# Shiakaron/Iterative-solvers-summer-2020

Hardware: AMD Instinct MI355X
Metric: Newton-steps/sec + JVP SpMV HBM GB/s (% peak), 4096^2 grid, 1/2/4/8 GPU (higher is better)
Workload: dtype f64

## Files before the change

include/nkhip.h:

```cpp
#ifndef NKHIP_H
#define NKHIP_H

#include <stdint.h>

#ifdef __cplusplus
extern "C" {
#endif

#define NK_OK 0
#define NK_NO_CONVERGENCE 1
#define NK_NONFINITE 2
#define NK_ZERO_STEP 3
#define NK_BAD_RHS 4
#define NK_EINVAL (-1)
#define NK_EHIP (-2)
#define NK_ECOMM (-3)
#define NK_ENOMEM (-4)

#define NKHIP_ABI_VERSION 3

#define NK_JVP_FD 0
#define NK_JVP_ANALYTIC 1

typedef struct nk_opts {
  double f_tol, f_rtol, x_tol, x_rtol;
  double rdiff;
  int64_t maxiter;
  int32_t inner_m;
  int32_t outer_k;
  int32_t line_search;
  int32_t jvp_mode;
  int32_t verbose;
  int32_t profile;
} nk_opts;

typedef struct nk_stats {
  int64_t nit;
  int64_t nfev;
  int64_t njvp;
  int64_t n_arnoldi;
  double fnorm_inf;
  double fnorm_2;
  int32_t status;
  int32_t pad_;
  int64_t n_backtrack;
  double step_min;
  int64_t n_device_steps;
} nk_stats;

typedef struct nk_kprof {
  char name[32];
  int64_t launches;
  double total_ms;
  double alg_bytes;
  int64_t timed;
  double timed_bytes;
} nk_kprof;

typedef struct nk_comm nk_comm;
typedef struct nk_sh nk_sh;

const char* nk_version(void);
int nk_abi_version(void);
int nk_opts_default(nk_opts* o);
const char* nk_status_string(int code);


int nk_lap5_apply(const double* v_dev, double* y_dev, int64_t ny, int64_t nx, double e, void* stream);

int nk_sh13_apply(const double* v_dev, double* y_dev, int64_t ny, int64_t nx, double h, double r,
                  void* stream);

int nk_sh_residual(const double* u_dev, const double* uo_dev, double* F_dev, int64_t ny, int64_t nx,
                   double h, double r, double k, double g, void* stream);

int nk_sh_jvp(const double* u_dev, const double* v_dev, double* y_dev, int64_t ny, int64_t nx,
              double h, double r, double k, double g, void* stream);

int nk_sh_fdjvp(const double* x0_dev, const double* G0_dev, const double* z_dev, double* y_dev,
                int64_t ny, int64_t nx, double h, double r, double k, double g, double zs,
                double sc, void* stream);

int nk_sh_arnoldi_fused(const double* const* V_dev, const double* coef, int32_t nv,
                        const double* w_dev, double tau, const double* x0_dev, const double* G0_dev,
                        const double* z_dev, int64_t ny, int64_t nx, double h, double r, double k,
                        double g, double zs, double sc, double* v_out_dev, double* w_out_dev,
                        double* dots, void* stream);

int64_t nk_edge_elems(int64_t ny, int64_t nx);
int nk_edge_gather(const double* v_dev, double* E_dev, int64_t ny, int64_t nx, void* stream);
int nk_sh_arnoldi_fused_edges(const double* const* V_dev, const double* const* E_dev,
                              const double* coef, int32_t nv, const double* w_dev, double tau,
                              const double* x0_dev, const double* G0_dev, const double* z_dev,
                              int64_t ny, int64_t nx, double h, double r, double k, double g,
                              double zs, double sc, double* v_out_dev, double* w_out_dev,
                              double* Ev_out_dev, double* Ew_out_dev, double* dots, void* stream);
int64_t nk_arnoldi_mbox_launches(void);

int nk_dot(const double* x_dev, const double* y_dev, int64_t n, double* out, void* stream);
int nk_nrm2(const double* x_dev, int64_t n, double* out, void* stream);
int nk_maxnorm(const double* x_dev, int64_t n, double* out, void* stream);
int nk_axpy(double a, const double* x_dev, double* y_dev, int64_t n, void* stream);
int nk_scal(double a, double* x_dev, int64_t n, void* stream);
int nk_mdot(const double* const* V_dev, int32_t m, const double* w_dev, int64_t n, double* out,
            void* stream);
int nk_maxpy(const double* const* V_dev, const double* coef, int32_t m, double* y_dev, int64_t n,
             void* stream);

int nk_stream_copy(const double* src_dev, double* dst_dev, int64_t n, void* stream);

int nk_debug_bounds(int64_t* violations, int32_t* first_line, int32_t reset);
int nk_debug_mailbox(int64_t* counts, int32_t reset);
int nk_debug_close(const double* const* P_dev, const double* cN, const double* cA,
                   const double* cB, int32_t m, int64_t n, double* A_dev, double* B_dev,
                   double* norm2, void* stream);
int nk_debug_ctl_step(int32_t form, int32_t t, const int32_t* ints, const double* scal,
                      const double* sig, const double* h, const double* cs, const double* sn,
                      const double* gram, const double* red, void* state_out, void* mirror_out,
                      double* prm_out, uint32_t* status_out);
typedef struct nk_stencil_pass {
  int64_t mode;
  int64_t ny, nx;
  int64_t r0, r1;
  const double* a;
  const double* a_halo;
  const double* b;
  const double* b_halo;
  const double* p0;
  double* out0;
  double* out1;
  double* out2;
  double alpha, sc, e, theta;
  double h, r, k, g;
  const double* znorm2;
  double omega;
  const double* spec;
  double spec_thr, spec_ftol, spec_rdiff, spec_zn, spec_zs;
  const double* Ea;
  const double* Eb;
  double* E0;
  double* E2;
  double* PS0[2];
  double* PS2[2];
  int64_t ps_ld;
  int64_t rev;
} nk_stencil_pass;
int nk_debug_stencil(const nk_stencil_pass* p, double* red, int64_t* nblk, void* stream);

int nk_comm_unique_id_bytes(void);
int nk_comm_get_unique_id(void* out);
int nk_comm_create_rccl(nk_comm** out, const void* unique_id, int32_t rank, int32_t nranks);
int nk_comm_create_loopback(nk_comm** out, int32_t nranks);
int nk_comm_peer_handle_bytes(void);
int nk_comm_create_peer(nk_comm** out, int32_t rank, int32_t nranks, int64_t max_nx,
                        void* handle_out);
int nk_comm_peer_connect(nk_comm* c, const void* handles);
int nk_comm_destroy(nk_comm* c);
int nk_comm_abort(nk_comm* c);
int nk_comm_selftest(nk_comm* c, int64_t nx, void* stream);
int nk_comm_selftest_push(nk_comm* c, int64_t nx, void* stream);

int nk_sh_create(nk_sh** out, int64_t ny_local, int64_t nx, int64_t ny_global, double h, double r,
                 double k, double g, const nk_opts* opts, nk_comm* comm, void* stream);
int nk_sh_destroy(nk_sh* s);
int nk_sh_step(nk_sh* s, const double* u_prev_dev, double* u_next_dev, nk_stats* stats);
int nk_sh_set_opts(nk_sh* s, const nk_opts* opts);
int nk_sh_kernel_profile(nk_sh* s, nk_kprof* out, int32_t max);
int nk_sh_reset_profile(nk_sh* s);
int nk_sh_step_log(nk_sh* s, double* steps, int32_t max);
int64_t nk_sh_workspace_bytes(nk_sh* s);

typedef int (*nk_residual_fn)(void* ctx, const double* x_dev, double* f_dev, int64_t n);
int64_t nk_solve_workspace_bytes(int64_t n, const nk_opts* opts);
int nk_solve(nk_residual_fn F, void* ctx, const double* x0_dev, double* x_dev, int64_t n,
             const nk_opts* opts, nk_stats* stats, void* stream, void* workspace,
             int64_t workspace_bytes);

typedef struct nk_drop_params {
  int32_t nx, ny;
  double endl, endr, endb, endt;
  double epsilon;
  int32_t n_exp, m_exp;
  double Bo, alpha2;
  double alpha, gamma, C;
  int32_t smoothing_iters;
  int32_t pad_;
  double a;
} nk_drop_params;
typedef struct nk_drop nk_drop;

int nk_drop_params_default(nk_drop_params* p);
int nk_drop_create(nk_drop** out, const nk_drop_params* p, const nk_opts* opts, void* stream);
int nk_drop_destroy(nk_drop* d);
int nk_drop_lds_fits(int32_t nx, int32_t ny);
int nk_drop_set_state(nk_drop* d, const double* U_dev, const double* Q_dev);
int nk_drop_get_state(nk_drop* d, double* U_dev, double* Q_dev);
int nk_drop_step(nk_drop* d, double dt, double dtmesh, int32_t pmaloops, nk_stats* stats,
                 double* dt_used, double* scale);
int nk_drop_set_scale(nk_drop* d, double scale);
int nk_drop_prepare(nk_drop* d);
int nk_drop_field(nk_drop* d, int32_t which, double* out_dev);
int nk_drop_residual(nk_drop* d, const double* u_dev, double dt, double* R_dev);
int nk_drop_solve(nk_drop* d, double dt, double* U_dev, nk_stats* stats);
int nk_drop_pma(nk_drop* d, double dtmesh, int32_t loops);
int nk_drop_init_coalescing(nk_drop* d, int32_t vsteps, const double* info, int32_t ndrops,
                            double dtmesh, int32_t loops);

typedef struct nk_shlin nk_shlin;
int nk_shlin_create(nk_shlin** out, int64_t ny, int64_t nx, double h, double r, double g, double k,
                    double rtol, int64_t maxiter, void* stream);
int nk_shlin_destroy(nk_shlin* s);
int nk_shlin_step(nk_shlin* s, const double* U_dev, const double* Uo_dev, double* Unew_dev,
                  int64_t* iters, double* relres);

typedef struct nk_mems_params {
  int32_t n;
  int32_t m;
  int32_t smoothing_iters;
  int32_t p;
  double alpha, gamma;
  double epsilon, beta, lambd;
  double endl, endr;
  double k;
} nk_mems_params;
typedef struct nk_mems nk_mems;

int nk_mems_params_default(nk_mems_params* p);
int nk_mems_create(nk_mems** out, const nk_mems_params* p, const nk_opts* opts, void* stream);
int nk_mems_destroy(nk_mems* m);
int nk_mems_set_state(nk_mems* m, const double* U_dev, const double* Q_dev);
int nk_mems_get_state(nk_mems* m, double* U_dev, double* Q_dev);
int nk_mems_step(nk_mems* m, nk_stats* stats, double* dt_used, double* time);
int nk_mems_prepare(nk_mems* m, double* dt);
int nk_mems_field(nk_mems* m, int32_t which, double* out_dev);
int nk_mems_residual(nk_mems* m, const double* u_dev, double* R_dev);

#ifdef __cplusplus
}
#endif
#endif
```

iterative-solvers-summer-2020_amd/csrc/capi.cpp:

```cpp
#include <hip/hip_runtime.h>

#include <cmath>
#include <cstdlib>
#include <cstdio>
#include <cstring>
#include <mutex>
#include <memory>
#include <new>
#include <vector>

#include "../../include/nkhip.h"
#include "comm.h"
#include "nk_kernels.h"
#include "nk_solver.h"
#include "droplet_problem.h"
#include "mems_problem.h"
#include "sh_problem.h"
#include "shlin.h"

using namespace nk;

namespace {

hipStream_t S(void* s) { return static_cast<hipStream_t>(s); }
// ... 121 lines not shown
  A.alpha = sc * zs;
  A.sc = sc;
  A.p0 = G0;
  A.out0 = y;
  A.c = sh_coef(h, r, k, g);
  return hip_rc(stencil_launch(SMode::FDJVP, A, S(stream), nullptr));
}

namespace {
int attach_mbox(ArnoldiArgs& A) {
  const int mode = arnoldi_mbox_mode();
  if (mode == 0) return NK_OK;
  static std::mutex mu;
  static double* buf = nullptr;
  static int64_t cap = 0;
  static uint64_t tag = 0;
  static std::vector<double*> retired;
  std::lock_guard<std::mutex> lk(mu);
  const int64_t need = arnoldi_mbox_elems(A.ny, A.nx);
  if (cap < need) {
    if (buf) retired.push_back(buf);
    buf = nullptr;
    cap = 0;
    if (hipMalloc(reinterpret_cast<void**>(&buf), sizeof(double) * need) != hipSuccess)
      return NK_ENOMEM;
    if (hipMemset(buf, 0, sizeof(double) * need) != hipSuccess) return NK_EHIP;
    cap = need;
  }
  A.mb = buf;
  A.mb_cap = cap;
  A.mb_tag = ++tag;
  A.mb_recompute = mode == 2;
  return NK_OK;
}

int arnoldi_fused_call(const double* const* V, const double* const* E, const double* coef,
                       int32_t nv, const double* w, double tau, const double* x0, const double* G0,
                       const double* z, int64_t ny, int64_t nx, double h, double r, double k,
                       double g, double zs, double sc, double* v_out, double* w_out,
                       double* Ev_out, double* Ew_out, double* dots, void* stream) {
  if (!V || !coef || !w || !x0 || !v_out || !w_out || !(sc != 0.0)) return NK_EINVAL;
  if (!arnoldi_supported(nv, ny, nx)) return NK_EINVAL;
  ArnoldiArgs A;
  if (E) {
    for (int i = 0; i <= nv; ++i) {
      if (!E[i]) return NK_EINVAL;
      A.E[i] = E[i];
    }
  }
  A.Eout_v = Ev_out;
  A.Eout_w = Ew_out;
  A.ny = ny;
  A.nx = nx;
  A.nv = nv;
  for (int i = 0; i < nv; ++i) {
    if (!V[i]) return NK_EINVAL;
    A.V[i] = V[i];
    A.c[i] = coef[i];
  }
  A.w = w;
  A.tau = tau;
  A.x0 = x0;
  A.g0 = G0;
  A.z = z;
  A.alpha = sc * zs;
  A.sc = sc;
  A.k = sh_coef(h, r, k, g);
  A.out_v = v_out;
  A.out_w = w_out;
  if (int rc = attach_mbox(A)) return rc;
  const int nval = 2 * nv + 3;
  if (!dots) {
    static std::mutex mu;
    std::lock_guard<std::mutex> lk(mu);
    static double* buf = nullptr;
    static int64_t cap = 0;
    const int64_t need = int64_t(nval) * 65536;
    if (cap < need) {
      if (buf) hipFree(buf);
      buf = nullptr;
      cap = 0;
      if (hipMalloc(reinterpret_cast<void**>(&buf), sizeof(double) * need) != hipSuccess)
        return NK_ENOMEM;
      cap = need;
    }
    A.partial = buf;
    A.partial_cap = cap;
    int64_t nw = 0;
    return hip_rc(arnoldi_launch(A, S(stream), &nw));
  }
  return reduce_call(int64_t(65536) * 2048, nval, nval, nval, dots, S(stream),
                     [&](double* part, int64_t* nb) {
                       A.partial = part;
                       A.partial_cap = int64_t(nval) * (65536 + 1);
                       return arnoldi_launch(A, S(stream), nb);
                     });
}
}

int64_t nk_arnoldi_mbox_launches(void) { return arnoldi_mbox_launches(); }

int nk_sh_arnoldi_fused(const double* const* V, const double* coef, int32_t nv, const double* w,
                        double tau, const double* x0, const double* G0, const double* z,
                        int64_t ny, int64_t nx, double h, double r, double k, double g, double zs,
                        double sc, double* v_out, double* w_out, double* dots, void* stream) {
  return arnoldi_fused_call(V, nullptr, coef, nv, w, tau, x0, G0, z, ny, nx, h, r, k, g, zs, sc,
                            v_out, w_out, nullptr, nullptr, dots, stream);
}

int nk_sh_arnoldi_fused_edges(const double* const* V, const double* const* E, const double* coef,
                              int32_t nv, const double* w, double tau, const double* x0,
                              const double* G0, const double* z, int64_t ny, int64_t nx, double h,
                              double r, double k, double g, double zs, double sc, double* v_out,
                              double* w_out, double* Ev_out, double* Ew_out, double* dots,
                              void* stream) {
  if (!E) return NK_EINVAL;
  return arnoldi_fused_call(V, E, coef, nv, w, tau, x0, G0, z, ny, nx, h, r, k, g, zs, sc, v_out,
                            w_out, Ev_out, Ew_out, dots, stream);
}

int64_t nk_edge_elems(int64_t ny, int64_t nx) {
  return (ny > 0 && nx > 0) ? edge_elems(ny, nx) : NK_EINVAL;
}

int nk_edge_gather(const double* v, double* E, int64_t ny, int64_t nx, void* stream) {
  if (!v || !E || ny < 1 || nx < 4 || nx % 2) return NK_EINVAL;
  return hip_rc(edge_gather_launch(v, E, ny, nx, S(stream)));
}

int nk_dot(const double* x, const double* y, int64_t n, double* out, void* stream) {
  if (!x || !y || !out || n < 0) return NK_EINVAL;
  VecList P;
  P.p[0] = y;
  return reduce_call(n, 3, 3, 1, out, S(stream), [&](double* part, int64_t* nb) {
    return mdot_launch(x, nullptr, P, 1, n, part, S(stream), nb);
  });
}

int nk_nrm2(const double* x, int64_t n, double* out, void* stream) {
  if (!x || !out || n < 0) return NK_EINVAL;
  double s2 = 0.0;
  VecList P;
  P.p[0] = x;
  const int rc = reduce_call(n, 3, 3, 1, &s2, S(stream), [&](double* part, int64_t* nb) {
    return mdot_launch(x, nullptr, P, 1, n, part, S(stream), nb);
  });
  *out = std::sqrt(s2);
  return rc;
}

int nk_maxnorm(const double* x, int64_t n, double* out, void* stream) {
  if (!x || !out || n <= 0) return NK_EINVAL;
  double* tmp = nullptr;
  hipError_t e = hipMallocAsync(reinterpret_cast<void**>(&tmp), sizeof(double) * n, S(stream));
  if (e != hipSuccess) return hip_rc(e);
  VecList none;
  double r2[2];
  const int rc = reduce_call(n, 2, 1, 2, r2, S(stream), [&](double* part, int64_t* nb) {
    return combo_launch(tmp, x, 1.0, none, 0, n, part, S(stream), nb);
  });
  hipFreeAsync(tmp, S(stream));
  hipStreamSynchronize(S(stream));
  *out = r2[1];
  return rc;
}

int nk_axpy(double a, const double* x, double* y, int64_t n, void* stream) {
  if (!x || !y || n < 0) return NK_EINVAL;
  return hip_rc(axpby_launch(a, x, 1.0, y, y, n, S(stream)));
}

int nk_scal(double a, double* x, int64_t n, void* stream) {
  if (!x || n < 0) return NK_EINVAL;
  return hip_rc(axpby_launch(a, x, 0.0, nullptr, x, n, S(stream)));
}

int nk_mdot(const double* const* V, int32_t m, const double* w, int64_t n, double* out,
            void* stream) {
  if (!V || !w || !out || m < 0 || m > kMaxVec || n < 0) return NK_EINVAL;
  if (m == 0) return NK_OK;
  VecList P;
  for (int i = 0; i < m; ++i) P.p[i] = V[i];
  const int nv = 2 * m + 1;
  double res[2 * kMaxVec + 1];
  const int rc = reduce_call(n, nv, nv, nv, res, S(stream), [&](double* part, int64_t* nb) {
    return mdot_launch(w, nullptr, P, m, n, part, S(stream), nb);
  });
  for (int i = 0; i < m; ++i) out[i] = res[i];
  return rc;
}

int nk_maxpy(const double* const* V, const double* coef, int32_t m, double* y, int64_t n,
             void* stream) {
  if (!V || !coef || !y || m < 0 || m > kMaxVec || n < 0) return NK_EINVAL;
  VecList P;
  for (int i = 0; i < m; ++i) {
    P.p[i] = V[i];
    P.c[i] = coef[i];
  }
  int64_t nb = 0;
  return hip_rc(combo_launch(y, y, 1.0, P, m, n, nullptr, S(stream), &nb));
}

int nk_stream_copy(const double* src, double* dst, int64_t n, void* stream) {
  if (!src || !dst || n < 0) return NK_EINVAL;
  return hip_rc(stream_copy_launch(src, dst, n, S(stream)));
}

int nk_debug_bounds(int64_t* violations, int32_t* first_line, int32_t reset) {
  const int rc = arnoldi_check_counters(violations, first_line, reset != 0);
  return rc == 0 ? NK_OK : (rc == -1 ? NK_EINVAL : NK_EHIP);
}

int nk_debug_mailbox(int64_t* counts, int32_t reset) {
  if (!counts) return NK_EINVAL;
  const int rc = arnoldi_mailbox_counters(counts, reset != 0);
  return rc == 0 ? NK_OK : (rc == -1 ? NK_EINVAL : NK_EHIP);
}

int nk_debug_close(const double* const* P, const double* cN, const double* cA, const double* cB,
                   int32_t m, int64_t n, double* A, double* B, double* norm2, void* stream) {
  if (!P || !cN || !cA || !cB || !A || !B || A == B || !norm2 || m < 1 || m > kMaxVec || n < 1)
    return NK_EINVAL;
  CloseList L;
  for (int i = 0; i < m; ++i) {
    for (int k = 0; k < i; ++k)
      if (P[k] == P[i]) return NK_EINVAL;
    if (!P[i]) return NK_EINVAL;
    L.p[i] = P[i];
    L.cN[i] = cN[i];
    L.cA[i] = cA[i];
    L.cB[i] = cB[i];
  }
  return reduce_call(n, 1, 1, 1, norm2, S(stream), [&](double* part, int64_t* nb) {
    return close_launch(A, B, L, m, n, part, S(stream), nb);
  });
}

int nk_debug_ctl_step(int32_t form, int32_t t, const int32_t* ints, const double* scal,
                      const double* sig, const double* h, const double* cs, const double* sn,
                      const double* gram, const double* red, void* state_out, void* mirror_out,
                      double* prm_out, uint32_t* status_out) {
  if (!state_out) return int(sizeof(ArnCtlState));
  if ((form != 0 && form != 1) || t < 1 || t + 1 > kArnMaxNV || !ints || !scal || !sig || !h ||
      !cs || !sn || !gram || !red || !mirror_out || !prm_out || !status_out)
    return NK_EINVAL;
  const int nval = 2 * (t + 1) + 1;
  ArnCtlState *hS = nullptr, *dS = nullptr;
  uint32_t* status = nullptr;
  double *prm = nullptr, *dred = nullptr;
  hipError_t e = hipHostMalloc(reinterpret_cast<void**>(&hS), sizeof(ArnCtlState), 0);
  if (e == hipSuccess)
    e = hipHostMalloc(reinterpret_cast<void**>(&status), sizeof(uint32_t) * (kMaxVec + 2), 0);
  if (e == hipSuccess) e = hipMalloc(reinterpret_cast<void**>(&dS), sizeof(ArnCtlState));
  if (e == hipSuccess) e = hipMalloc(reinterpret_cast<void**>(&prm), sizeof(double) * kCtlPrm);
  if (e == hipSuccess) e = hipMalloc(reinterpret_cast<void**>(&dred), sizeof(double) * 2 * nval);
  if (e == hipSuccess) {
    std::memset(hS, 0, sizeof(ArnCtlState));
    std::memset(status, 0, sizeof(uint32_t) * (kMaxVec + 2));
    ArnCtlState& S = *hS;
    S.j = ints[0];
    S.hn_pending = ints[1];
    S.m = ints[2];
    S.nv_max = ints[3];
    S.halt = ints[4];
    S.steps = ints[5];
    S.wnorm[t - 1] = scal[0];
    S.gv[t - 1] = scal[1];
    S.sig_est[t] = scal[2];
    S.ptol = scal[3];
    S.omega = scal[4];
    S.lag_ratio2 = scal[5];
    for (int i = 0; i <= t; ++i) S.sig[i] = sig[i];
    for (int i = 0; i < t; ++i) {
      S.h[i] = h[i];
      S.cs[i] = cs[i];
      S.sn[i] = sn[i];
      for (int k = 0; k < i; ++k) S.gram[i][k] = gram[i * t + k];
    }
    e = hipMemcpy(dS, hS, sizeof(ArnCtlState), hipMemcpyHostToDevice);
  }
  if (e == hipSuccess) e = hipMemset(prm, 0, sizeof(double) * kCtlPrm);
  if (e == hipSuccess) e = hipMemcpy(dred, red, sizeof(double) * nval, hipMemcpyHostToDevice);
  if (e == hipSuccess)
    e = form == 0 ? arn_ctl_launch(dS, hS, dred, nullptr, prm, status, t, nullptr)
                  : arn_reduce_ctl_launch(dred, 1, nval, dred + nval, nullptr, dS, hS, prm, status,
                                          t, nullptr);
  if (e == hipSuccess) e = hipDeviceSynchronize();
  if (e == hipSuccess) e = hipMemcpy(state_out, dS, sizeof(ArnCtlState), hipMemcpyDeviceToHost);
  if (e == hipSuccess)
    e = hipMemcpy(prm_out, prm, sizeof(double) * kCtlPrm, hipMemcpyDeviceToHost);
  if (e == hipSuccess) {
    std::memcpy(mirror_out, hS, sizeof(ArnCtlState));
    *status_out = status[t];
  }
  if (hS) (void)hipHostFree(hS);
  if (status) (void)hipHostFree(status);
  (void)hipFree(dS);
  (void)hipFree(prm);
  (void)hipFree(dred);
  return hip_rc(e);
}

int nk_debug_stencil(const nk_stencil_pass* p, double* red, int64_t* nblk_out, void* stream) {
  if (!p || p->mode < 0 || p->mode > 7 || p->ny <= 0 || p->nx <= 0 || !p->a || !p->out0)
    return NK_EINVAL;
  const SMode m = static_cast<SMode>(int(p->mode));
  const bool two = m == SMode::RESID || m == SMode::TRIAL || m == SMode::FDJVP || m == SMode::LINOP;
  const bool has_p0 = m == SMode::TRIAL || m == SMode::FDJVP || m == SMode::AJVP || m == SMode::LINOP;
  const bool reduces = m == SMode::TRIAL || m == SMode::LINOP;
  if ((two && !p->b) || (has_p0 && !p->p0) || (m == SMode::TRIAL && !p->out1) ||
      (m == SMode::LINOP && !p->out2) || (reduces && !red))
    return NK_EINVAL;
  if (m == SMode::FDJVP && !p->znorm2 && !p->spec && !(p->sc != 0.0)) return NK_EINVAL;
  const bool ranged = p->r1 >= 0;
  if (ranged && (p->ny < 4 || p->r0 < 0 || p->r0 >= p->r1 || p->r1 > p->ny || p->r0 == 1 ||
                 p->r1 == p->ny - 1))
    return NK_EINVAL;
  const bool push0 = p->PS0[0] || p->PS0[1], push2 = p->PS2[0] || p->PS2[1];
  if ((push0 && (!p->PS0[0] || !p->PS0[1])) || (push2 && (!p->PS2[0] || !p->PS2[1])) ||
      (push2 && !(m == SMode::TRIAL && p->out2)) ||
      ((push0 || push2) && (p->ny < 4 || p->ps_ld < p->nx || p->ps_ld % 2)))
    return NK_EINVAL;
  for (const void* q : {(const void*)p->Ea, (const void*)p->Eb, (const void*)p->E0,
                        (const void*)p->E2, (const void*)p->PS0[0], (const void*)p->PS0[1],
                        (const void*)p->PS2[0], (const void*)p->PS2[1]})
    if (reinterpret_cast<uintptr_t>(q) & 15u) return NK_EINVAL;
  if (p->E2 && m != SMode::TRIAL) return NK_EINVAL;
  if (p->rev < -1 || p->rev > 1) return NK_EINVAL;

  StencilArgs A;
  A.ny = p->ny;
  A.nx = p->nx;
  auto field = [&](const double* base, const double* halo) {
    return halo ? Field{base, halo, halo + 2 * p->nx} : periodic(base);
  };
  A.a = field(p->a, p->a_halo);
  if (p->b) A.b = (p->b == p->a && p->b_halo == p->a_halo) ? A.a : field(p->b, p->b_halo);
  A.alpha = p->alpha;
  A.p0 = p->p0;
  A.out0 = p->out0;
  A.out1 = p->out1;
  A.out2 = p->out2;
  A.e = p->e;
  A.c = sh_coef(p->h, p->r, p->k, p->g);
  A.sc = p->sc;
  A.znorm2 = p->znorm2;
  A.omega = p->omega;
  A.spec = p->spec;
  A.spec_thr = p->spec_thr;
  A.spec_ftol = p->spec_ftol;
  A.spec_rdiff = p->spec_rdiff;
  A.spec_zn = p->spec_zn;
  A.spec_zs = p->spec_zs;
  A.theta = p->theta;
  A.Ea = p->Ea;
  A.Eb = p->Eb;
  A.E0 = p->E0;
  A.E2 = p->E2;
  A.e_ny = p->ny;
  A.e_row0 = 0;
  for (int i = 0; i < 2; ++i) {
    A.PS0[i] = p->PS0[i];
    A.PS2[i] = p->PS2[i];
  }
  A.ps_ld = p->ps_ld;
  A.rev_force = int(p->rev);
  const StencilArgs L = ranged ? stencil_rows(A, p->r0, p->r1) : A;

  hipStream_t s = S(stream);
  double* buf = nullptr;
  const int64_t slots = stencil_partial_slots(p->ny, p->nx);
  hipError_t e = hipSuccess;
  StencilArgs R = L;
  if (reduces) {
    e = hipMallocAsync(reinterpret_cast<void**>(&buf), sizeof(double) * (slots + 3), s);
    if (e == hipSuccess) e = hipMemsetAsync(buf, 0xff, sizeof(double) * (slots + 3), s);
    if (e != hipSuccess) {
      if (buf) hipFreeAsync(buf, s);
      return hip_rc(e);
    }
    R.partial = buf;
  }
  int64_t nblk = 0;
  e = stencil_launch(m, R, s, &nblk);
  double host[3] = {0.0, 0.0, 0.0};
  const int nv = m == SMode::TRIAL ? 3 : 1;
  if (reduces && e == hipSuccess && 3 * nblk > slots) e = hipErrorInvalidValue;
  if (reduces && e == hipSuccess) e = reduce_final_launch(buf, nblk, 1, nv, buf + slots, nullptr, s);
  if (reduces && e == hipSuccess)
    e = hipMemcpyAsync(host, buf + slots, sizeof(double) * nv, hipMemcpyDeviceToHost, s);
  if (buf) hipFreeAsync(buf, s);
  if (e == hipSuccess) e = hipStreamSynchronize(s);
  if (e != hipSuccess) return hip_rc(e);
  for (int i = 0; reduces && i < nv; ++i) red[i] = host[i];
  if (nblk_out) *nblk_out = nblk;
  return NK_OK;
}

int nk_comm_unique_id_bytes(void) { return comm_unique_id_bytes(); }
int nk_comm_get_unique_id(void* out) { return out ? comm_get_unique_id(out) : NK_EINVAL; }
int nk_comm_create_rccl(nk_comm** out, const void* uid, int32_t rank, int32_t nranks) {
  return comm_create_rccl(out, uid, rank, nranks);
}
int nk_comm_create_loopback(nk_comm** out, int32_t nranks) {
  return comm_create_loopback(out, nranks);
}
int nk_comm_peer_handle_bytes(void) { return comm_peer_handle_bytes(); }
int nk_comm_create_peer(nk_comm** out, int32_t rank, int32_t nranks, int64_t max_nx,
                        void* handle_out) {
  return comm_create_peer(out, rank, nranks, max_nx, handle_out);
}
int nk_comm_peer_connect(nk_comm* c, const void* handles) { return comm_peer_connect(c, handles); }
int nk_comm_destroy(nk_comm* c) {
  delete c;
  return NK_OK;
}
int nk_comm_abort(nk_comm* c) {
  if (!c) return NK_EINVAL;
  c->abort();
  return NK_OK;
}

int nk_comm_selftest(nk_comm* c, int64_t nx, void* stream) {
  if (!c || nx < 1) return NK_EINVAL;
  const hipStream_t s = S(stream);
  const int P = c->size(), r = c->rank();
  constexpr int kV = 8, kSum = 5;
  const int64_t nslab = 4 * nx, nhalo = 4 * nx;
  std::vector<double> h(kV + nslab + nhalo);
  for (int i = 0; i < kV; ++i) h[i] = (i < kSum) ? r + 1.0 + i : r + double(i);
  auto code = [&](int q, int64_t row, int64_t j) { return 1e6 * q + double(row * nx + j); };
  for (int64_t row = 0; row < 4; ++row)
    for (int64_t j = 0; j < nx; ++j) h[kV + row * nx + j] = code(r, row, j);
  double* d = nullptr;
  if (hipMalloc(reinterpret_cast<void**>(&d), h.size() * sizeof(double)) != hipSuccess)
    return NK_EHIP;
  int rc = hipMemcpyAsync(d, h.data(), (kV + nslab) * sizeof(double), hipMemcpyHostToDevice, s) ==
                   hipSuccess
               ? NK_OK
               : NK_EHIP;
  if (!rc) rc = c->allreduce(d, kSum, kV, s);
  if (!rc) rc = c->halo(d + kV, d + kV + nslab, d + kV + nslab + 2 * nx, 4, nx, s);
  if (!rc && (hipMemcpyAsync(h.data(), d, h.size() * sizeof(double), hipMemcpyDeviceToHost, s) !=
                  hipSuccess ||
              hipStreamSynchronize(s) != hipSuccess))
    rc = NK_EHIP;
  (void)hipFree(d);
  if (rc) return rc;
  if (c->failed()) return NK_ECOMM;
  for (int i = 0; i < kV; ++i) {
    const double want = (i < kSum) ? P * (P + 1) / 2.0 + double(P) * i : (P - 1.0) + i;
    if (h[i] != want) return NK_ECOMM;
  }
  const int prev = (r - 1 + P) % P, next = (r + 1) % P;
  const double* lo = h.data() + kV + nslab;
  const double* hi = lo + 2 * nx;
  for (int64_t row = 0; row < 2; ++row)
    for (int64_t j = 0; j < nx; ++j)
      if (lo[row * nx + j] != code(prev, 2 + row, j) || hi[row * nx + j] != code(next, row, j))
        return NK_ECOMM;
  return NK_OK;
}

namespace {
__global__ void slot_read_kernel(const double* src, double* dst, int64_t n) {
  const int64_t i = int64_t(blockIdx.x) * blockDim.x + threadIdx.x;
  if (i < n) dst[i] = src[i];
}
}

int nk_comm_selftest_push(nk_comm* c, int64_t nx, void* stream) {
  if (!c || nx < 1) return NK_EINVAL;
  const hipStream_t s = S(stream);
  nk_halo_slots sl;
  static const char owner = 0;
  const bool claimed = c->claim_slots(&owner, &sl);
  struct Release {
    nk_comm* c;
    bool on;
    ~Release() {
      if (on) c->release_slots(&owner);
    }
  } rel{c, claimed};
  const bool have = claimed && sl.ld >= nx && sl.count >= 1;
  const int P = c->size(), r = c->rank();
  const int64_t ny = 4;
  const int64_t slots[2] = {0, sl.count - 1};
  const char* be = std::getenv("NKHIP_PEER_SELFTEST_BREAK_PUSH");
  const bool broken = be && *be && std::atoi(be) == r;
  auto code = [&](int q, int64_t slot, int64_t row, int64_t j) {
    return 1e9 * (q + 1) + 1e6 * slot + double(row * nx + j);
  };
  const int64_t nslot = have ? 4 * sl.ld : 0;
  std::vector<double> h(2 * ny * nx + 2 * nslot + 2);
  h[2 * ny * nx + 2 * nslot] = have ? 0.0 : 1.0;
  double* d = nullptr;
  if (hipMalloc(reinterpret_cast<void**>(&d), h.size() * sizeof(double)) != hipSuccess)
    return NK_EHIP;
  double* vsrc = d;
  double* rd = d + 2 * ny * nx;
  double* ar = rd + 2 * nslot;
  for (int k = 0; k < 2; ++k)
    for (int64_t row = 0; row < ny; ++row)
      for (int64_t j = 0; j < nx; ++j)
        h[(k * ny + row) * nx + j] = code(r, slots[k], row, j) + (broken ? 0.5 : 0.0);
  int rc = NK_OK;
  auto ok = [&](hipError_t e) {
    if (!rc && e != hipSuccess) rc = NK_EHIP;
  };
  for (int k = 0; k < 2 && have; ++k)
    ok(hipMemsetAsync(sl.mine + slots[k] * 4 * sl.ld, 0xff, sizeof(double) * nslot, s));
  ok(hipMemcpyAsync(d, h.data(), sizeof(double) * (2 * ny * nx + 2 * nslot + 2),
                    hipMemcpyHostToDevice, s));
  if (!rc) rc = c->allreduce(ar, 0, 2, s);
  double any_without = 1.0;
  if (!rc && (hipMemcpyAsync(&any_without, ar, sizeof(double), hipMemcpyDeviceToHost, s) !=
                  hipSuccess ||
              hipStreamSynchronize(s) != hipSuccess))
    rc = NK_EHIP;
  if (!rc && any_without != 0.0) rc = NK_EINVAL;
  for (int k = 0; k < 2 && !rc; ++k)
    ok(push_rows_launch(vsrc + k * ny * nx, sl.prev + slots[k] * 4 * sl.ld,
                        sl.next + slots[k] * 4 * sl.ld, ny, nx, sl.ld, s));
  if (!rc) rc = c->allreduce(ar, 1, 2, s);
  for (int k = 0; k < 2 && !rc; ++k) {
    hipLaunchKernelGGL(slot_read_kernel, dim3(unsigned((nslot + 255) / 256)), dim3(256), 0, s,
                       sl.mine + slots[k] * 4 * sl.ld, rd + k * nslot, nslot);
    ok(hipGetLastError());
  }
  if (!rc && (hipMemcpyAsync(h.data(), rd, sizeof(double) * 2 * nslot, hipMemcpyDeviceToHost, s) !=
                  hipSuccess ||
              hipStreamSynchronize(s) != hipSuccess))
    rc = NK_EHIP;
  (void)hipFree(d);
  if (rc) return rc;
  if (c->failed()) return NK_ECOMM;
  const int prev = (r - 1 + P) % P, next = (r + 1) % P;
  for (int k = 0; k < 2; ++k) {
    const double* m = h.data() + k * nslot;
    for (int64_t row = 0; row < 4; ++row)
      for (int64_t j = 0; j < nx; ++j) {
        const double want = row < 2 ? code(prev, slots[k], ny - 2 + row, j)
                                    : code(next, slots[k], row - 2, j);
        if (m[row * sl.ld + j] != want) return NK_ECOMM;
      }
  }
  return NK_OK;
}

int nk_sh_create(nk_sh** out, int64_t ny_local, int64_t nx, int64_t ny_global, double h, double r,
                 double k, double g, const nk_opts* opts, nk_comm* comm, void* stream) {
  if (!out || ny_local <= 0 || nx <= 0 || ny_global < ny_local || !(h > 0) || !(k != 0))
    return NK_EINVAL;
  if (comm && comm->size() > 1 && ny_local < 2) return NK_EINVAL;
  if ((!comm || comm->size() == 1) && ny_global != ny_local) return NK_EINVAL;
  std::unique_ptr<nk_sh> sh(new (std::nothrow) nk_sh());
  if (!sh) return NK_ENOMEM;
  sh->opts = opts ? *opts : default_opts();
  sh->ny = ny_local;
  sh->nx = nx;
  sh->E = std::make_unique<Engine>(ny_local * nx, comm, S(stream), sh->opts.profile > 0,
                                   stencil_partial_slots(ny_local, nx));
  sh->E->sample = sh->opts.profile > 1 ? sh->opts.profile : 1;
  sh->P = std::make_unique<SHProblem>(*sh->E, ny_local, nx, ny_global, sh_coef(h, r, k, g),
                                      sh->opts.jvp_mode);
  if (sh->P->status()) return sh->P->status();
  sh->NK = std::make_unique<NewtonKrylov>(*sh->E, *sh->P, sh->opts);
  if (sh->NK->status()) return sh->NK->status();
  const int rc = sh->E->sync();
  if (rc) return rc;
  *out = sh.release();
  return NK_OK;
}

int nk_sh_destroy(nk_sh* s) {
  delete s;
  return NK_OK;
}

int nk_sh_set_opts(nk_sh* s, const nk_opts* opts) {
  if (!s || !opts) return NK_EINVAL;
  if (opts->inner_m != s->opts.inner_m || opts->outer_k != s->opts.outer_k) return NK_EINVAL;
  s->opts = *opts;
  s->E->profile = opts->profile > 0;
  s->E->sample = opts->profile > 1 ? opts->profile : 1;
  s->P->set_jvp_mode(opts->jvp_mode);
  s->NK->set_opts(*opts);
  return NK_OK;
}

int nk_sh_step(nk_sh* s, const double* u_prev, double* u_next, nk_stats* stats) {
  if (!s || !u_prev || !u_next) return NK_EINVAL;
  int rc = s->P->prepare(u_prev);
  if (!rc) rc = s->NK->solve(u_prev, u_next, stats);
  if (rc < 0 && s->E->comm) s->E->comm->abort();
  return rc;
}

int nk_sh_kernel_profile(nk_sh* s, nk_kprof* out, int32_t max) {
  if (!s) return NK_EINVAL;
  for (int k = 0; k < K_NKINDS && k < max; ++k) {
    std::memset(out[k].name, 0, sizeof(out[k].name));
    std::strncpy(out[k].name, kind_name(k), sizeof(out[k].name) - 1);
    out[k].launches = s->E->stat(k).launches;
    out[k].total_ms = s->E->stat(k).ms;
    out[k].alg_bytes = s->E->stat(k).bytes;
    out[k].timed = s->E->stat(k).timed;
    out[k].timed_bytes = s->E->stat(k).tbytes;
  }
  return K_NKINDS;
}

int nk_sh_reset_profile(nk_sh* s) {
  if (!s) return NK_EINVAL;
  s->E->reset_stats();
  return NK_OK;
}

int nk_sh_step_log(nk_sh* s, double* steps, int32_t max) {
  if (!s || max < 0 || (max > 0 && !steps)) return NK_EINVAL;
  const std::vector<double>& log = s->NK->step_log();
  for (int32_t i = 0; i < max && size_t(i) < log.size(); ++i) steps[i] = log[i];
  return int(log.size());
}

int64_t nk_sh_workspace_bytes(nk_sh* s) { return s ? s->E->bytes_allocated() : -1; }

int64_t nk_solve_workspace_bytes(int64_t n, const nk_opts* opts) {
  if (n <= 0) return NK_EINVAL;
  const nk_opts o = opts ? *opts : default_opts();
  return int64_t(sizeof(double)) * Engine::pad(n) * (NewtonKrylov::vectors_needed(o) + 2);
}

int nk_solve(nk_residual_fn F, void* ctx, const double* x0, double* x, int64_t n,
             const nk_opts* opts, nk_stats* stats, void* stream, void* workspace,
             int64_t workspace_bytes) {
  if (!F || !x0 || !x || n <= 0) return NK_EINVAL;
  const nk_opts o = opts ? *opts : default_opts();
  if (o.jvp_mode != NK_JVP_FD) return NK_EINVAL;
  Engine E(n, nullptr, S(stream), o.profile != 0);
  const int nvec = NewtonKrylov::vectors_needed(o);
  const int64_t npad = Engine::pad(n);
  const int64_t need = nk_solve_workspace_bytes(n, &o);
  double* ws = static_cast<double*>(workspace);
  const bool own = (ws == nullptr);
  if (!own && (workspace_bytes < need || (reinterpret_cast<uintptr_t>(ws) & 255u)))
    return NK_EINVAL;
  if (own && hipMalloc(reinterpret_cast<void**>(&ws), need) != hipSuccess) return NK_ENOMEM;
  CallbackProblem P(E, F, ctx, ws + npad * nvec, ws + npad * (nvec + 1));
  int rc;
  {
    NewtonKrylov NK(E, P, o, ws, int64_t(sizeof(double)) * npad * nvec);
    rc = NK.status();
    if (!rc) rc = NK.solve(x0, x, stats);
  }
  hipStreamSynchronize(S(stream));
  if (own) hipFree(ws);
  return rc;
}

int nk_drop_params_default(nk_drop_params* p) {
  if (!p) return NK_EINVAL;
  *p = nk_drop_params{};
  p->nx = 91;
  p->ny = 61;
  p->endl = -3;
  p->endr = 6;
  p->endb = -3;
  p->endt = 3;
  p->epsilon = 1e-2;
  p->n_exp = 6;
  p->m_exp = 3;
  p->Bo = 0.01;
  p->alpha2 = 0.0;
  p->alpha = 0.01;
  p->gamma = 0.1;
  p->C = 0.15;
  p->smoothing_iters = 4;
  p->a = 100.0;
  return NK_OK;
}

int nk_drop_create(nk_drop** out, const nk_drop_params* p, const nk_opts* opts, void* stream) {
  if (!out || !p || p->nx < 7 || p->ny < 7) return NK_EINVAL;
  if (p->n_exp < 0 || p->m_exp < 0) return NK_EINVAL;
  DropParams P{};
  P.nx = p->nx;
  P.ny = p->ny;
  P.endl = p->endl;
  P.endr = p->endr;
  P.endb = p->endb;
  P.endt = p->endt;
  P.dksi = (p->endr - p->endl) / (p->nx - 1);
  P.deta = (p->endt - p->endb) / (p->ny - 1);
  P.epsilon = p->epsilon;
  P.n_exp = p->n_exp;
  P.m_exp = p->m_exp;
  P.Bo = p->Bo;
  P.alpha2 = p->alpha2;
// ... 178 lines not shown
```

iterative-solvers-summer-2020_amd/csrc/lgmres.cpp:

```cpp
#include <algorithm>
#include <atomic>
#include <cstddef>
#include <cfloat>
#include <cmath>
#include <cstdlib>
#include <cstring>

#include "nk_solver.h"
#include "peer_dev.h"

namespace nk {

namespace {
constexpr double kEps = DBL_EPSILON;
constexpr double kLagMinRatio2 = 1e-12;

bool devctl_enabled(bool multi) {
  const char* v = std::getenv("NKHIP_DEVCTL");
  if (v && v[0] == '0') return false;
  if (v && v[0] == '1') return true;
  return multi;
}

bool lag_enabled() {
  static const bool on = [] {
    const char* v = std::getenv("NKHIP_LAGNORM");
    return !(v && v[0] == '0');
  }();
  return on;
}

int close_mode_env() {
  const char* v = std::getenv("NKHIP_CLOSE");
  if (v && v[0] == '0') return 0;
  if (v && v[0] == '2') return 2;
  return 1;
}
}

int NewtonKrylov::issue_step(int j, const double* z, double zs, double znorm, bool dev_scale,
                             bool have_w) {
  const int64_t n = E_.n;
  zp_[j] = z;
  hS_->zs[j] = zs;
  double* w = V_[j + 1];
  int rc;
  if (have_w) {
    rc = NK_OK;
    st_->njvp += 1;
  } else if (dev_scale) {
    rc = P_.jvp_dev(X_, G0_, z, E_.dres(Engine::kSlotCombo), omega_, w);
    st_->njvp += 1;
  } else if (znorm == 0.0) {
    rc = E_.launch(K_COPY, 8.0 * n,
                   [&] { return hipMemsetAsync(w, 0, sizeof(double) * n, E_.s); });
    if (!rc) rc = P_.publish_edges(w);
  } else {
    rc = P_.jvp(X_, G0_, z, zs, omega_ / znorm, w);
    st_->njvp += 1;
  }
  if (rc) return rc;
  st_->n_arnoldi += 1;
  VecList P;
  for (int i = 0; i <= j; ++i) P.p[i] = V_[i];
  int64_t nblk = 0;
  const double* g = (j > 0) ? V_[j] : nullptr;
  rc = E_.launch(K_MDOT, 8.0 * n * (j + 2),
                 [&] { return mdot_launch(w, g, P, j + 1, n, E_.partial(), E_.s, &nblk); });
  if (rc) return rc;
  const int np = j + 1;
  return E_.reduce_async(nblk, 2 * np + 1, 2 * np + 1, Engine::slot_mdot(j));
}

int NewtonKrylov::lgmres(double tol, double* dnorm, double* dmax, double** dvec) {
  *dnorm = 0.0;
  *dmax = 0.0;
  *dvec = nullptr;
  const double b_norm = fx_norm_;
  if (!std::isfinite(b_norm)) return NK_BAD_RHS;
  if (b_norm == 0.0) return NK_OK;
  const double atol = std::max(0.0, tol * b_norm);
  const double r_norm = b_norm;
  if (r_norm <= std::max(atol, tol * b_norm)) return NK_OK;
  const double ptol = std::min(1.0, std::max(atol, tol * b_norm) / r_norm);

  const int n_o = ocount_;
  const int m = o_.inner_m + n_o;
  const int64_t n = E_.n;
  const int K = int(outer_.size());
  const bool lag = lag_enabled() && P_.may_speculate();
  const bool devctl = lag && devctl_enabled(E_.comm != nullptr || P_.prefers_devctl());
  V_[0] = Fx_;
  ArnCtlState& S = *hS_;
  S.m = m;
  S.halt = 0;
  S.steps = 0;
  S.ptol = ptol;
  S.omega = omega_;
  S.lag_ratio2 = kLagMinRatio2;
  double* const sig = S.sig;
  double* const rn = S.rn;
  double* const sig_est = S.sig_est;
  double* const wnorm = S.wnorm;
  double* const zs_ = S.zs;
  double* const h = S.h;
  sig[0] = 1.0 / b_norm;
  rn[0] = b_norm;
  double hcur[kMaxVec + 2];
  double red[2 * kMaxVec + 2];
  for (int i = 0; i < kMaxVec + 2; ++i) S.gv[i] = 0.0;
  S.gv[0] = 1.0;

  auto input = [&](int j, const double** z, double* zs, double* zn) {
    if (j < n_o) {
      const int slot = (ohead_ + j) % K;
      *z = outer_[slot];
      *zs = osig_[slot];
      *zn = osig_[slot] * orn_[slot];
    } else {
      *z = V_[j > n_o ? j : 0];
      const int q = j > n_o ? j : 0;
      *zs = sig[q];
      *zn = sig[q] * rn[q];
    }
  };
  auto rotated = [&](int i, double hn, double* hc) {
    for (int k = 0; k <= i; ++k) hc[k] = h[k];
    hc[i + 1] = hn;
    for (int k = 0; k < i; ++k) {
      const double t = S.cs[k] * hc[k] + S.sn[k] * hc[k + 1];
      hc[k + 1] = -S.sn[k] * hc[k] + S.cs[k] * hc[k + 1];
      hc[k] = t;
    }
  };
  auto would_stop = [&](int i, double hn) -> bool {
    double hc[kMaxVec + 2], c, s;
    rotated(i, hn, hc);
    detail::givens(hc[i], hc[i + 1], &c, &s);
    return std::fabs(-s * S.gv[i]) < ptol || !(hn > kEps * wnorm[i]);
  };
  auto finish = [&](int i, double hn) -> bool {
    rotated(i, hn, hcur);
    const double alpha = 1.0 / hn;
    sig[i + 1] = std::isfinite(alpha) ? alpha : 1.0;
    rn[i + 1] = hn;
    const bool breakdown = !(hn > kEps * wnorm[i]);
    detail::givens(hcur[i], hcur[i + 1], &S.cs[i], &S.sn[i]);
    hcur[i] = S.cs[i] * hcur[i] + S.sn[i] * hcur[i + 1];
    for (int k = 0; k <= i; ++k) S.R[k][i] = hcur[k];
    S.gv[i + 1] = -S.sn[i] * S.gv[i];
    S.gv[i] = S.cs[i] * S.gv[i];
    return std::fabs(S.gv[i + 1]) < ptol || breakdown;
  };

  int rc;
  {
    const double* z;
    double zs, zn;
    input(0, &z, &zs, &zn);
    const bool have = spec_.valid && n_o > 0 && z == spec_.z && zs == spec_.zs &&
                      zn == spec_.zn && V_[1] == spec_.w && X_ == spec_.x && G0_ == spec_.g;
    spec_.valid = false;
    rc = issue_step(0, z, zs, zn, false, have);
  }
  sig_est[0] = 0.0;
  if (!rc) rc = E_.sync();
  if (rc) return rc;
  int j = 0, last = 0;
  int close_mode = lag ? close_mode_env() : 0;
  bool closed = false;
  bool hn_pending = false;
  for (;;) {
    const int np = j + 1;
    std::memcpy(red, E_.hres(Engine::slot_mdot(j)), sizeof(double) * (2 * np + 1));
    double tau = 1.0;
    if (hn_pending) {
      hn_pending = false;
      if (finish(j - 1, std::sqrt(red[np + j]))) {
        st_->njvp -= 1;
        st_->n_arnoldi -= 1;
        last = j - 1;
        break;
      }
      if (sig_est[j] > 0.0) {
        tau = sig[j] / sig_est[j];
        zs_[j] = sig[j];
      }
    }
    const double ww = tau * tau * red[2 * np];
    if (!std::isfinite(ww)) return NK_NONFINITE;
    wnorm[j] = std::sqrt(ww);
    for (int i = 0; i < j; ++i) S.gram[j][i] = sig[j] * sig[i] * red[np + i];
    double hh = 0.0;
    for (int i = 0; i <= j; ++i) {
      double acc = tau * sig[i] * red[i];
      for (int k = 0; k < i; ++k) acc -= S.gram[i][k] * h[k];
      h[i] = acc;
      hh += acc * acc;
    }
    VecList U;
    for (int i = 0; i <= j; ++i) {
      U.p[i] = V_[i];
      U.c[i] = -h[i] * sig[i];
    }
    double* w = V_[j + 1];
    const bool more = j + 1 < m;
    const bool next_is_v = more && (j + 1 > n_o);
    const double est = ww - hh;
    int64_t nblk = 0;
    bool predicted = false;
    if (close_mode && P_.has_fused(j + 1) && j + 2 < int(V_.size())) {
      const double hn_est = std::sqrt(est);
      if (close_mode == 2) {
        predicted = true;
        close_mode = 1;
      } else if (hn_est > kEps * wnorm[j]) {
        predicted = !more || (est > kLagMinRatio2 * ww && would_stop(j, hn_est));
      }
    }
    if (predicted) {
      double hc[kMaxVec + 2], a[kMaxVec + 1], b[kMaxVec + 1];
      rotated(j, 0.0, hc);
      if (j > 0 && !detail::lstsq_upper_direct(S.R, j)) {
        close_mode = 0;
        predicted = false;
      }
      for (int i = j - 1; predicted && i >= 0; --i) {
        double accA = S.gv[i], accB = hc[i];
        for (int k = i + 1; k < j; ++k) {
          accA -= S.R[i][k] * a[k];
          accB -= S.R[i][k] * b[k];
        }
        a[i] = accA / S.R[i][i];
        b[i] = accB / S.R[i][i];
      }
      CloseList C;
      int nc = 0;
      auto entry = [&](const double* p) -> int {
        for (int q = 0; q < nc; ++q)
          if (C.p[q] == p) return q;
        if (nc == kMaxVec) return -1;
        C.p[nc] = p;
        C.cN[nc] = C.cA[nc] = C.cB[nc] = 0.0;
        return nc++;
      };
      if (predicted) {
        C.cN[entry(w)] = tau;
        for (int i = 0; i <= j; ++i) C.cN[entry(V_[i])] = U.c[i];
        for (int i = 0; i <= j; ++i) {
          const int q = entry(zp_[i]);
          if (q < 0) {
            predicted = false;
            break;
          }
          if (i < j) {
            C.cA[q] += b_norm * a[i] * zs_[i];
            C.cB[q] -= b[i] * zs_[i];
          } else {
            C.cB[q] += zs_[j];
          }
        }
      }
      if (predicted) {
        rc = E_.launch(K_COMBO, 8.0 * n * (nc + 2), [&] {
          return close_launch(Sv_, V_[j + 2], C, nc, n, E_.partial(), E_.s, &nblk);
        });
        if (rc) return rc;
        double v2 = 0.0;
        rc = E_.reduce(nblk, 1, 1, &v2);
        if (rc) return rc;
        const double hn = std::sqrt(v2);
        if (!more || would_stop(j, hn)) {
          finish(j, hn);
          last = j;
          closed = true;
          break;
        }
      }
    }
    const bool lag_step =
        more && lag && !predicted && (!next_is_v || est > kLagMinRatio2 * ww);
    if (lag_step && P_.has_fused(j + 1)) {
      const double* z = nullptr;
      double zs, zn;
      if (next_is_v) {
        const double e = std::sqrt(est);
        zs = 1.0 / e;
        zn = zs * e;
      } else {
        input(j + 1, &z, &zs, &zn);
      }
      if (zn != 0.0) {
        const double* Vp[kMaxVec];
        double cc[kMaxVec];
        for (int i = 0; i <= j; ++i) {
          Vp[i] = V_[i];
          cc[i] = U.c[i];
        }
        int64_t nw = 0;
        double* vout = Sv_;
        rc = P_.fused_step(Vp, cc, j + 1, w, tau, X_, G0_, z, zs, omega_ / zn, vout, V_[j + 2],
                           &nw, nullptr);
        if (rc) return rc;
        Sv_ = V_[j + 1];
        V_[j + 1] = vout;
        zp_[j + 1] = next_is_v ? vout : z;
        zs_[j + 1] = zs;
        sig_est[j + 1] = next_is_v ? zs : 0.0;
        st_->njvp += 1;
        st_->n_arnoldi += 1;
        const int np1 = j + 2;
        rc = E_.reduce_async(nw, 2 * np1 + 1, 2 * np1 + 1, Engine::slot_mdot(j + 1));
        if (rc) return rc;
        hn_pending = true;
        ++j;
        if (devctl && next_is_v) {
          S.j = j;
          S.hn_pending = 1;
          rc = device_steps();
          j = S.j;
          hn_pending = S.hn_pending != 0;
        } else {
          rc = E_.wait_results(Engine::slot_mdot(j), 2 * np1 + 1);
        }
        if (rc) return rc;
        continue;
      }
    }
    if (lag_step) {
      const EdgeOut eo = P_.edge_out(w);
      rc = E_.launch(K_COMBO, 8.0 * n * (j + 3), [&] {
        return combo_launch(w, w, tau, U, j + 1, n, nullptr, E_.s, &nblk, eo);
      });
      if (!rc) rc = P_.publish_edges(w, eo.E != nullptr);
      if (rc) return rc;
      const double* z;
      double zs, zn;
      if (next_is_v) {
        const double e = std::sqrt(est);
        z = w;
        zs = 1.0 / e;
        zn = zs * e;
        sig_est[j + 1] = zs;
      } else {
        input(j + 1, &z, &zs, &zn);
        sig_est[j + 1] = 0.0;
      }
      rc = issue_step(j + 1, z, zs, zn, false);
      if (rc) return rc;
      hn_pending = true;
      ++j;
      if (devctl && next_is_v && P_.has_jvp_prm() && zn != 0.0) {
        S.j = j;
        S.hn_pending = 1;
        rc = device_steps();
        j = S.j;
        hn_pending = S.hn_pending != 0;
        if (rc) return rc;
        continue;
      }
      rc = E_.sync();
      if (rc) return rc;
      continue;
    }
    const EdgeOut eo = P_.edge_out(w);
    rc = E_.launch(K_COMBO, 8.0 * n * (j + 3), [&] {
      return combo_launch(w, w, tau, U, j + 1, n, E_.partial(), E_.s, &nblk, eo);
    });
    if (!rc) rc = P_.publish_edges(w, eo.E != nullptr);
    if (!rc) rc = E_.reduce_async(nblk, 1, 1, Engine::kSlotCombo);
    if (rc) return rc;
    const bool spec = next_is_v && P_.has_dev_scale() && P_.may_speculate();
    if (spec) {
      rc = issue_step(j + 1, w, 0.0, 0.0, true);
      if (rc) return rc;
    }
    rc = E_.sync();
    if (rc) return rc;
    const bool stop = finish(j, std::sqrt(E_.hres(Engine::kSlotCombo)[0]));
    if (spec) zs_[j + 1] = sig[j + 1];
    if (stop || !more) {
      if (spec) {
        st_->njvp -= 1;
        st_->n_arnoldi -= 1;
      }
      last = j;
      break;
    }
    if (!spec) {
      const double* z;
      double zs, zn;
      input(j + 1, &z, &zs, &zn);
      rc = issue_step(j + 1, z, zs, zn, false);
      if (!rc) rc = E_.sync();
      if (rc) return rc;
    }
    sig_est[j + 1] = 0.0;
    ++j;
  }
  j = last;
  if (!std::isfinite(S.R[j][j])) return NK_OK;
  double y[kMaxVec + 1];
  detail::lstsq_upper(S.R, j + 1, S.gv, y);
  for (int i = 0; i <= j; ++i) {
    y[i] *= b_norm;
    if (!std::isfinite(y[i])) return NK_OK;
  }
  const int slot = (o_.outer_k > 0 && ocount_ < o_.outer_k) ? (ohead_ + ocount_) % K : ohead_;
  VecList Z;
  int nz = j + 1;
  if (closed && detail::lstsq_upper_direct(S.R, j + 1)) {
    nz = 2;
    Z.p[0] = Sv_;
    Z.c[0] = 1.0;
    Z.p[1] = V_[j + 2];
    Z.c[1] = y[j];
  } else {
    for (int i = 0; i <= j; ++i) {
      Z.p[i] = zp_[i];
      Z.c[i] = y[i] * zs_[i];
    }
  }
  int64_t nblk = 0;
  double* d = outer_[slot];
  const EdgeOut eo = P_.edge_out(d);
  rc = E_.launch(K_COMBO, 8.0 * n * (nz + 1), [&] {
    return combo_launch(d, nullptr, 0.0, Z, nz, n, E_.partial(), E_.s, &nblk, eo);
  });
  if (!rc) rc = P_.publish_edges(d, eo.E != nullptr);
  if (rc) return rc;
  double r2[2];
  rc = E_.reduce(nblk, 1, 2, r2);
  if (rc) return rc;
  const double nx = std::sqrt(r2[0]);
  if (nx > 0 && o_.outer_k > 0) {
    osig_[slot] = 1.0 / nx;
    orn_[slot] = nx;
    if (ocount_ < o_.outer_k)
      ++ocount_;
    else
      ohead_ = (ohead_ + 1) % K;
  }
  *dnorm = nx;
  *dmax = r2[1];
  *dvec = d;
  return NK_OK;
}

int NewtonKrylov::device_steps() {
  ArnCtlState& S = *hS_;
  const int t0 = S.j;
  int nvmax = t0;
  while (nvmax + 1 < S.m && nvmax + 1 <= kArnMaxNV &&
         (P_.has_fused(nvmax + 1) || P_.has_jvp_prm()))
    ++nvmax;
  if (nvmax < t0 + 1) return E_.wait_results(Engine::slot_mdot(t0), 2 * (t0 + 1) + 1);
  S.nv_max = nvmax;
  S.halt = 0;
  S.steps = 0;
  S.arrive = 0;
  S.done = 0;
  volatile uint32_t* st = status_;
  for (int t = t0; t < S.m && t < kMaxVec + 2; ++t) st[t] = 0;
  std::atomic_thread_fence(std::memory_order_release);

  const bool one = E_.comm == nullptr;
  struct Rot {
    double* spare;
    double* v;
    bool fused;
    bool unfused;
    bool ctl;
    bool red;
  };
  Rot rot[kMaxVec + 2];
  double cc[kMaxVec] = {};
  const uint64_t wait_ticks = device_wait_ticks();
  auto control = [&](int t, bool copy, int upload_rows = -1) {
    const int slot = Engine::slot_mdot(t);
    return E_.launch(K_CTL, 0.0, [&] {
      return arn_ctl_launch(dS_, hS_, E_.dres(slot), copy ? E_.hres_mut(slot) : nullptr, prm_,
                            status_, t, E_.s, upload_rows);
    });
  };
  auto issue = [&](int t) -> int {
    rot[t] = Rot{Sv_, V_[t + 1], false, false, true, false};
    const int nval = 2 * (t + 2) + 1;
    const int slot = Engine::slot_mdot(t + 1);
    if (!P_.has_fused(t + 1)) {
      const int64_t n = E_.n;
      double* w = V_[t + 1];
      VecList U;
      for (int i = 0; i <= t; ++i) U.p[i] = V_[i];
      int rc = E_.launch(K_COMBO, 8.0 * n * (t + 3),
                         [&] { return combo_prm_launch(w, w, prm_, U, t + 1, n, E_.s); });
      if (!rc) rc = P_.jvp_prm(X_, G0_, w, prm_, V_[t + 2]);
      if (rc) return rc;
      zp_[t + 1] = w;
      rot[t].unfused = true;
      VecList Pm;
      for (int i = 0; i <= t + 1; ++i) Pm.p[i] = V_[i];
      int64_t nb = 0;
      rc = E_.launch(K_MDOT, 8.0 * n * (t + 4), [&] {
        return mdot_launch(V_[t + 2], w, Pm, t + 2, n, E_.partial(), E_.s, &nb);
      });
      if (rc) return rc;
      if (one)
        return E_.launch(K_CTL, 8.0 * nb * nval, [&] {
          return arn_reduce_ctl_launch(E_.partial(), nb, nval, E_.dres_mut(slot),
                                       E_.hres_mut(slot), dS_, hS_, prm_, status_, t + 1, E_.s);
        });
      rot[t].red = true;
      rc = E_.reduce_async(nb, nval, nval, slot, false);
      return rc ? rc : control(t + 1, true);
    }
    const double* Vp[kMaxVec];
    for (int i = 0; i <= t; ++i) Vp[i] = V_[i];
    double* vout = Sv_;
    int64_t nw = 0;
    PeerArgs pa;
    const bool have_pa = !one && peer_fuse_enabled() && E_.comm->take_allreduce(&pa, nval);
    ArnTail tl;
    const char* te = std::getenv("NKHIP_ARN_TAIL");
    const bool tail_env = te && (te[0] == '1' || te[0] == '2');
    const bool want_tail = tail_env && (one || (have_pa && ((te && te[0] == '2') ||
                                                            !E_.comm->group_shares_device())));
    if (want_tail) {
      tl.S = dS_;
      tl.H = hS_;
      tl.result = E_.dres_mut(slot);
      tl.result_host = E_.hres_mut(slot);
      tl.prm = prm_;
      tl.status = status_;
      tl.t = t + 1;
      tl.nval = nval;
      tl.peer = !one;
      const uint64_t ticks = wait_ticks;
      tl.wait_ticks = ticks;
      if (have_pa) tl.pa = pa;
      if (const char* e = std::getenv("NKHIP_ARN_TAIL_TIMEOUT_S")) {
        const double sec = std::atof(e);
        if (sec > 0) {
          const uint64_t t = uint64_t(double(ticks) * sec / device_wait_seconds());
          tl.wait_ticks = std::min(tl.wait_ticks, t);
          if (have_pa) tl.pa.wait_ticks = std::min(tl.pa.wait_ticks, t);
        }
      }
    }
    bool tail_used = false;
    int rc = P_.fused_step(Vp, cc, t + 1, V_[t + 1], 1.0, X_, G0_, nullptr, 1.0, 1.0, vout,
                           V_[t + 2], &nw, prm_, want_tail ? &tl : nullptr, &tail_used);
    if (rc) return rc;
    Sv_ = V_[t + 1];
    V_[t + 1] = vout;
    zp_[t + 1] = vout;
    rot[t].fused = true;
    if (tail_used) {
      rot[t].ctl = false;
      return NK_OK;
    }
    if (one)
      return E_.launch(K_CTL, 8.0 * nw * nval, [&] {
        return arn_reduce_ctl_launch(E_.partial(), nw, nval, E_.dres_mut(slot),
                                     E_.hres_mut(slot), dS_, hS_, prm_, status_, t + 1, E_.s);
      });
    if (have_pa)
      return E_.launch(K_CTL, 8.0 * nw * nval, [&] {
        return arn_reduce_allreduce_ctl_launch(E_.partial(), nw, nval, E_.dres_mut(slot),
                                               E_.hres_mut(slot), pa, dS_, hS_, prm_, status_,
                                               t + 1, E_.s);
      });
    rot[t].red = true;
    rc = E_.reduce_async(nw, nval, nval, slot, false);
    return rc ? rc : control(t + 1, true);
  };
  int rc = control(t0, false, t0);
  int next = t0;
  if (!rc) rc = issue(next++);
  int t = t0;
  while (!rc) {
    const uint32_t v = E_.wait_flag(status_ + t);
    if (v != 1) {
      if (v != 2) rc = (E_.comm && E_.comm->failed()) ? NK_ECOMM : NK_EHIP;
      break;
    }
    st_->njvp += 1;
    st_->n_arnoldi += 1;
    st_->n_device_steps += 1;
    ++t;
    if (next == t && next + 1 <= nvmax) rc = issue(next++);
  }
  int voided = 0, voided_unfused = 0, voided_ctl = 0, voided_red = 0;
  for (int u = next - 1; u >= t; --u) {
    voided_ctl += rot[u].ctl ? 1 : 0;
    voided_red += rot[u].red ? 1 : 0;
    if (rot[u].unfused) {
      ++voided_unfused;
      continue;
    }
    if (!rot[u].fused) continue;
    Sv_ = rot[u].spare;
    V_[u + 1] = rot[u].v;
    ++voided;
  }
  P_.void_fused_steps(voided);
  E_.void_last(K_CTL, voided_ctl);
  E_.void_last(K_COMBO, voided_unfused);
  E_.void_last(K_USERF, voided_unfused);
  E_.void_last(K_MDOT, voided_unfused);
  E_.void_last(K_REDUCE, voided_red);
  if (rc) return rc;
  if (voided > 0 && (rc = E_.sync()) != NK_OK) return rc;
  if (S.j != t || S.halt != 1 + t) return NK_EHIP;
  S.halt = 0;
  return NK_OK;
}

}
```

iterative-solvers-summer-2020_amd/csrc/nk_kernels.h:

```cpp
#pragma once

#include <hip/hip_runtime.h>

#include <cstdint>

#include "peer_dev.h"

struct nk_comm;

namespace nk {

bool peer_fuse_enabled();
bool slab_x_enabled(const nk_comm* c);
uint64_t device_wait_ticks();
double device_wait_seconds();

struct Field {
  const double* base;
  const double* lo;
  const double* hi;
};

inline Field periodic(const double* p) { return Field{p, nullptr, nullptr}; }

struct SHCoef {
  double c0, c1, c2, c3;
  double k, g;
  double ik;
};
SHCoef sh_coef(double h, double r, double k, double g);

enum class SMode : int {
  LAP5 = 0,
  SH13 = 1,
  RESID = 2,
  BOLD = 3,
  TRIAL = 4,
  FDJVP = 5,
  AJVP = 6,
  LINOP = 7,
};

struct StencilArgs {
  int64_t ny = 0, nx = 0;
  Field a{}, b{};
  double alpha = 0.0;
  const double* p0 = nullptr;
  double* out0 = nullptr;
  double* out1 = nullptr;
  double* out2 = nullptr;
  double e = 0.0;
  SHCoef c{};
  double sc = 1.0;
  double* partial = nullptr;
  const double* znorm2 = nullptr;
  double omega = 0.0;
  const double* spec = nullptr;
  double spec_thr = 0.0, spec_ftol = 0.0, spec_rdiff = 0.0, spec_zn = 1.0, spec_zs = 1.0;
  double theta = 0.0;
  double* E0 = nullptr;
  double* E2 = nullptr;
  const double* Ea = nullptr;
  const double* Eb = nullptr;
  int64_t e_ny = 0, e_row0 = 0;
  double* PS0[2] = {};
  double* PS2[2] = {};
  int64_t ps_ld = 0;
  bool rev = false;
  int rev_force = -1;
  bool nt_p0 = false;
};

bool traversal_reverse();

StencilArgs stencil_rows(const StencilArgs& A, int64_t r0, int64_t r1);
hipError_t stencil_launch(SMode m, const StencilArgs& a, hipStream_t s, int64_t* nblk);
int64_t stencil_partial_slots(int64_t ny, int64_t nx);
double stencil_bytes_per_point(SMode m, bool has_xt);

constexpr int kMaxVec = 64;
struct VecList {
  const double* p[kMaxVec];
  double c[kMaxVec];
};

constexpr int kKrylovBlock = 256;
constexpr int kKrylovPerThread = 8;
constexpr int64_t kKrylovChunk = int64_t(kKrylovBlock) * kKrylovPerThread;

inline int64_t krylov_blocks(int64_t n) { return (n + kKrylovChunk - 1) / kKrylovChunk; }
int64_t krylov_grid(int64_t n, int* cpb, int64_t target_blocks);

hipError_t mdot_launch(const double* a, const double* g, const VecList& P, int np, int64_t n,
                       double* partial, hipStream_t s, int64_t* nblk);
struct EdgeOut {
  double* E = nullptr;
  int64_t nx = 0, ny = 0;
};
hipError_t combo_launch(double* out, const double* in, double cin, const VecList& P, int np,
                        int64_t n, double* partial, hipStream_t s, int64_t* nblk,
                        const EdgeOut& eo = EdgeOut{});
hipError_t combo_prm_launch(double* out, const double* in, const double* prm, const VecList& P,
                            int np, int64_t n, hipStream_t s);
struct CloseList {
  const double* p[kMaxVec];
  double cN[kMaxVec], cA[kMaxVec], cB[kMaxVec];
};
hipError_t close_launch(double* outA, double* outB, const CloseList& P, int np, int64_t n,
                        double* partial, hipStream_t s, int64_t* nblk);
hipError_t reduce_final_launch(const double* partial, int64_t nblk, int nsum, int nv,
                               double* result, double* result_host, hipStream_t s);
hipError_t fddiff_launch(double* w, const double* f0, double sc, int64_t n, hipStream_t s);
hipError_t cg_update_launch(double* x, double* r, const double* p, const double* q, double alpha,
                            int64_t n, double* partial, hipStream_t s, int64_t* nblk);
hipError_t shlin_diag_launch(const double* U, const double* Uo, double k, double g, double* d,
                             int64_t n, hipStream_t s);
hipError_t stream_copy_launch(const double* src, double* dst, int64_t n, hipStream_t s);
hipError_t axpby_launch(double a, const double* x, double b, const double* y, double* out,
                        int64_t n, hipStream_t s);

constexpr int kArnMaxNV = 35;
constexpr int kEdgeW = 256;
__host__ __device__ inline int64_t edge_groups(int64_t nx) { return (nx + kEdgeW - 1) / kEdgeW; }
__host__ __device__ inline int64_t edge_elems(int64_t ny, int64_t nx) { return edge_groups(nx) * ny * 4; }
hipError_t edge_gather_launch(const double* v, double* E, int64_t ny, int64_t nx, hipStream_t s);
struct SlabX {
  char* me = nullptr;
  char* prev = nullptr;
  char* next = nullptr;
  int P = 0;
  int64_t max_nx = 0;
  uint64_t tag = 0;
  int* err = nullptr;
  uint64_t wait_ticks = 0;
};
struct ArnCtlState;
struct ArnTail {
  ArnCtlState* S = nullptr;
  ArnCtlState* H = nullptr;
  double* result = nullptr;
  double* result_host = nullptr;
  double* prm = nullptr;
  uint32_t* status = nullptr;
  int t = 0;
  int nval = 0;
  bool peer = false;
  uint64_t wait_ticks = 0;
  PeerArgs pa{};
};
struct ArnoldiArgs {
  int64_t ny = 0, nx = 0;
  int nv = 0;
  int strips = 0, nbands = 0, RY = 0;
  const double* V[kArnMaxNV] = {};
  double c[kArnMaxNV] = {};
  const double* w = nullptr;
  double tau = 1.0;
  const double* x0 = nullptr;
  const double* g0 = nullptr;
  const double* z = nullptr;
  double alpha = 0.0;
  double sc = 1.0;
  SHCoef k{};
  double* out_v = nullptr;
  double* out_w = nullptr;
  const double* E[kArnMaxNV + 1] = {};
  double* Eout_v = nullptr;
  double* Eout_w = nullptr;
  const double* yh = nullptr;
  int64_t yh_ld = 0;
  SlabX x{};
  const double* HS[kArnMaxNV + 2] = {};
  int64_t hs_ld = 0;
  double* PS[4] = {};
  double* partial = nullptr;
  int64_t partial_cap = 0;
  int64_t r_begin = 0, r_end = -1;
  int64_t pstride = 0, pcol0 = 0;
  bool plan_only = false;
  int reserve_cus = 0;
  const double* ctl = nullptr;
  double* mb = nullptr;
  int64_t mb_cap = 0;
  uint64_t mb_tag = 0;
  bool mb_recompute = false;
  int alt = -1;
  ArnTail tail{};
};
inline int64_t arnoldi_mbox_elems(int64_t ny, int64_t nx) {
  return (2 * ny + 64) * (nx / 128 + 2) * 8;
}
int arnoldi_mbox_mode();
int64_t arnoldi_mbox_launches();
bool arnoldi_supported(int nv, int64_t ny, int64_t nx);
bool arnoldi_wide(int nv);
hipError_t arnoldi_launch(const ArnoldiArgs& A, hipStream_t s, int64_t* nwaves);
hipError_t arnoldi_edge_launch(const ArnoldiArgs& A, double* y4, hipStream_t s);
hipError_t arnoldi_edge_halo_launch(const ArnoldiArgs& A, const PeerArgs& pa, double* yh,
                                    hipStream_t s);
int arnoldi_check_counters(int64_t* violations, int32_t* first_line, bool reset);
int arnoldi_mailbox_counters(int64_t out[4], bool reset);
hipError_t push_rows_launch(const double* v, double* prev_slot, double* next_slot, int64_t ny,
                            int64_t nx, int64_t ld, hipStream_t s);

struct ArnCtlState {
  int32_t j;
  int32_t hn_pending;
  int32_t m;
  int32_t nv_max;
  int32_t halt;
  int32_t steps;
  uint32_t arrive;
  uint32_t done;
  double ptol, omega, lag_ratio2, pad2_;
  double sig[kMaxVec + 2];
  double rn[kMaxVec + 2];
  double sig_est[kMaxVec + 2];
  double wnorm[kMaxVec + 2];
  double zs[kMaxVec + 2];
  double cs[kMaxVec + 1], sn[kMaxVec + 1];
  double gv[kMaxVec + 2];
  double h[kMaxVec + 2];
  double R[kMaxVec + 1][kMaxVec + 1];
  double gram[kMaxVec + 1][kMaxVec + 1];
};
constexpr int kCtlPrm = kArnMaxNV + 4;
hipError_t arn_ctl_launch(ArnCtlState* S, ArnCtlState* H, const double* red, double* red_host,
                          double* prm, uint32_t* status, int t, hipStream_t s,
                          int upload_rows = -1);
hipError_t arn_reduce_ctl_launch(const double* partial, int64_t nblk, int nval, double* result,
                                 double* result_host, ArnCtlState* S, ArnCtlState* H, double* prm,
                                 uint32_t* status, int t, hipStream_t s);
hipError_t arn_reduce_allreduce_ctl_launch(const double* partial, int64_t nblk, int nval,
                                           double* result, double* result_host, const PeerArgs& pa,
                                           ArnCtlState* S, ArnCtlState* H, double* prm,
                                           uint32_t* status, int t, hipStream_t s);

}
```

iterative-solvers-summer-2020_amd/csrc/nk_solver.cpp:

```cpp
#include "nk_solver.h"

#include <algorithm>
#include <atomic>
#include <cfloat>
#include <cmath>
#include <cstdio>
#include <cstdlib>
#include <cstring>
#include <mutex>

namespace nk {

namespace {
constexpr double kEps = DBL_EPSILON;
constexpr int kReduceSlots = Engine::kSlots;
}

const char* kind_name(int kind) {
  static const char* names[K_NKINDS] = {"sh_fdjvp", "sh_ajvp", "sh_trial", "sh_bold",
                                         "krylov_mdot", "krylov_combo", "reduce_final", "copy",
                                         "halo", "user_F", "axpby", "arnoldi_fused",
                                         "arnoldi_edge", "edge_gather", "arnoldi_slab_edges",
                                         "arnoldi_ctl", "halo_push"};
  return (kind >= 0 && kind < K_NKINDS) ? names[kind] : "?";
// ... 171 lines not shown
}

int64_t Engine::pool_index(const double* v) const {
  if (!pool_ || !v || v < pool_) return -1;
  const int64_t off = v - pool_;
  if (off % npad != 0 || off / npad >= pool_count_) return -1;
  return off / npad;
}

void Engine::mark_edges(const double* v) {
  const int64_t q = pool_index(v);
  if (q < 0 || !epool_) return;
  if (ekept_.size() < size_t(pool_count_)) ekept_.assign(pool_count_, 0);
  ekept_[q] = 1;
}

bool Engine::edges_kept(const double* v) const {
  const int64_t q = pool_index(v);
  return q >= 0 && size_t(q) < ekept_.size() && ekept_[q] != 0;
}

double* Engine::edges(const double* v) const {
  if (!epool_ || !v || v < pool_) return nullptr;
  const int64_t off = v - pool_;
  if (off % npad != 0 || off / npad >= pool_count_) return nullptr;
  return epool_ + edge_n_ * (off / npad);
}

int Engine::gather_edges(const double* v) {
  double* e = edges(v);
  if (!e) return NK_OK;
  mark_edges(v);
  return launch(K_EDGE, 8.0 * edge_n_ * 2,
                [&] { return edge_gather_launch(v, e, edge_ny_, edge_nx_, s); });
}

EdgeOut Engine::edge_out(const double* v) {
  EdgeOut eo;
  eo.E = edges(v);
  if (!eo.E) return eo;
  mark_edges(v);
  eo.nx = edge_nx_;
  eo.ny = edge_ny_;
  return eo;
}

hipEvent_t Engine::ev() {
  if (!free_ev_.empty()) {
    hipEvent_t e = free_ev_.back();
    free_ev_.pop_back();
    return e;
  }
  hipEvent_t e = nullptr;
  hipEventCreate(&e);
  return e;
}

void Engine::harvest() {
  for (auto& p : pend_) {
    float ms = 0.f;
    hipEventElapsedTime(&ms, p.a, p.b);
    stats_[p.kind].timed += 1;
    stats_[p.kind].ms += ms;
    stats_[p.kind].tbytes += p.bytes;
    free_ev_.push_back(p.a);
    free_ev_.push_back(p.b);
  }
  pend_.clear();
}

void Engine::void_last(int kind, int count) {
  if (kind < 0 || kind >= K_NKINDS) return;
  for (int c = 0; c < count && c < kRecent && stats_[kind].launches > 0; ++c) {
    const int64_t idx = stats_[kind].launches - 1;
    stats_[kind].launches = idx;
    stats_[kind].bytes -= recent_bytes_[kind][idx % kRecent];
    for (size_t i = 0; i < pend_.size(); ++i) {
      if (pend_[i].kind == kind && pend_[i].idx == idx) {
        free_ev_.push_back(pend_[i].a);
        free_ev_.push_back(pend_[i].b);
        pend_.erase(pend_.begin() + i);
        break;
      }
    }
  }
}

void Engine::reset_stats() {
  for (auto& k : stats_) k = KStat{};
  for (auto& t : tick_) t = 0;
}

int Engine::sync() {
  if (hipStreamSynchronize(s) != hipSuccess) return NK_EHIP;
  harvest();
  return (comm && comm->failed()) ? NK_ECOMM : NK_OK;
}

int Engine::copy(double* dst, const double* src, int64_t cnt) {
  if (dst == src) return NK_OK;
  return launch(K_COPY, 16.0 * cnt, [&] {
    if (cnt >= (int64_t(1) << 16)) return axpby_launch(1.0, src, 0.0, nullptr, dst, cnt, s);
    return hipMemcpyAsync(dst, src, sizeof(double) * cnt, hipMemcpyDeviceToDevice, s);
  });
}

namespace {
constexpr uint64_t kUnset = 0x7FF0DEADBEEF0001ull;
bool poll_enabled() {
  static const bool on = [] {
    const char* e = std::getenv("NKHIP_POLL");
    return !(e && e[0] == '0');
  }();
  return on;
}
}

int Engine::wait_results(int slot, int nv) {
  if ((comm && !comm->allreduce_writes_host()) || !poll_enabled()) return sync();
  volatile uint64_t* h = reinterpret_cast<volatile uint64_t*>(hres_ + slot);
  for (int k = 0; k < nv; ++k) {
    for (int64_t spins = 0; h[k] == kUnset; ++spins) {
      if (spins > (int64_t(1) << 26)) return sync();
      __builtin_ia32_pause();
    }
  }
  std::atomic_thread_fence(std::memory_order_acquire);
  return NK_OK;
}

uint32_t Engine::wait_flag(const uint32_t* flag) {
  const volatile uint32_t* f = flag;
  for (int64_t spins = 0; *f == 0; ++spins) {
    if (spins > (int64_t(1) << 26)) {
      if (sync() != NK_OK) return 0;
      break;
    }
    __builtin_ia32_pause();
  }
  const uint32_t v = *f;
  std::atomic_thread_fence(std::memory_order_acquire);
  return v;
}

int Engine::reduce_async(int64_t nblk, int nsum, int nv, int slot, bool host_copy) {
  if (slot < 0 || slot + nv > kReduceSlots) return NK_EINVAL;
  const bool multi = comm != nullptr;
  if (!multi || (host_copy && comm->allreduce_writes_host())) {
    uint64_t* h = reinterpret_cast<uint64_t*>(hres_ + slot);
    for (int k = 0; k < nv; ++k) h[k] = kUnset;
    std::atomic_thread_fence(std::memory_order_release);
  }
  int rc = launch(K_REDUCE, 8.0 * nblk * nv, [&] {
    return reduce_final_launch(partial_, nblk, nsum, nv, dres_ + slot,
                               multi ? nullptr : hres_ + slot, s);
  });
  if (rc || !multi) return rc;
  if (!host_copy) return comm->allreduce(dres_ + slot, nsum, nv, s);
  return comm->allreduce_host(dres_ + slot, hres_ + slot, nsum, nv, s);
}

int Engine::reduce(int64_t nblk, int nsum, int nv, double* out) {
  int rc = reduce_async(nblk, nsum, nv, kSlotSync);
  if (!rc) rc = sync();
  if (rc) return rc;
  std::memcpy(out, hres_ + kSlotSync, sizeof(double) * nv);
  return NK_OK;
}

namespace detail {

void givens(double a, double b, double* c, double* s) {
  if (b == 0.0) {
    *c = 1.0;
    *s = 0.0;
    return;
  }
  const double r = std::hypot(a, b);
  *c = a / r;
  *s = b / r;
}

bool lstsq_upper_direct(const double (*R)[kMaxVec + 1], int n) {
  double dmax = 0.0, dmin = INFINITY;
  for (int i = 0; i < n; ++i) {
    dmax = std::max(dmax, std::fabs(R[i][i]));
    dmin = std::min(dmin, std::fabs(R[i][i]));
  }
  return n > 0 && dmin > kEps * n * dmax;
}

void lstsq_upper(const double (*R)[kMaxVec + 1], int n, const double* g, double* y) {
  if (lstsq_upper_direct(R, n)) {
    for (int i = n - 1; i >= 0; --i) {
      double acc = g[i];
      for (int k = i + 1; k < n; ++k) acc -= R[i][k] * y[k];
      y[i] = acc / R[i][i];
    }
    return;
  }
  std::vector<double> A(n * n), Vm(n * n, 0.0);
  for (int i = 0; i < n; ++i)
    for (int k = 0; k < n; ++k) A[i * n + k] = (k >= i) ? R[i][k] : 0.0;
  for (int i = 0; i < n; ++i) Vm[i * n + i] = 1.0;
  for (int sweep = 0; sweep < 60; ++sweep) {
    double off = 0.0;
    for (int p = 0; p < n - 1; ++p)
      for (int q = p + 1; q < n; ++q) {
        double a = 0, b = 0, c = 0;
        for (int i = 0; i < n; ++i) {
          a += A[i * n + p] * A[i * n + p];
          b += A[i * n + q] * A[i * n + q];
          c += A[i * n + p] * A[i * n + q];
        }
        if (c == 0.0) continue;
        off = std::max(off, std::fabs(c) / std::sqrt(a * b + 1e-300));
        const double zeta = (b - a) / (2.0 * c);
        const double t = std::copysign(1.0, zeta) / (std::fabs(zeta) + std::sqrt(1.0 + zeta * zeta));
        const double cs = 1.0 / std::sqrt(1.0 + t * t), sn = cs * t;
        for (int i = 0; i < n; ++i) {
          const double ap = A[i * n + p], aq = A[i * n + q];
          A[i * n + p] = cs * ap - sn * aq;
          A[i * n + q] = sn * ap + cs * aq;
          const double vp = Vm[i * n + p], vq = Vm[i * n + q];
          Vm[i * n + p] = cs * vp - sn * vq;
          Vm[i * n + q] = sn * vp + cs * vq;
        }
      }
    if (off < 1e-15) break;
  }
  std::vector<double> sig(n);
  double smax = 0.0;
  for (int k = 0; k < n; ++k) {
    double acc = 0;
    for (int i = 0; i < n; ++i) acc += A[i * n + k] * A[i * n + k];
    sig[k] = std::sqrt(acc);
    smax = std::max(smax, sig[k]);
  }
  const double cut = kEps * n * smax;
  for (int i = 0; i < n; ++i) y[i] = 0.0;
  for (int k = 0; k < n; ++k) {
    if (!(sig[k] > cut)) continue;
    double ug = 0.0;
    for (int i = 0; i < n; ++i) ug += A[i * n + k] * g[i];
    ug /= sig[k] * sig[k];
    for (int i = 0; i < n; ++i) y[i] += Vm[i * n + k] * ug;
  }
}

}

NewtonKrylov::NewtonKrylov(Engine& E, Problem& P, const nk_opts& o, void* external,
                           int64_t external_bytes)
    : E_(E), P_(P), o_(o) {
  if (o.inner_m < 1 || o.outer_k < 0 || o.inner_m + o.outer_k + 1 > kMaxVec) {
    init_status_ = NK_EINVAL;
    return;
  }
  std::vector<double*> v;
  init_status_ = E_.alloc(vectors_needed(o), &v, external, external_bytes);
  if (init_status_) return;
  int q = 0;
  X_ = v[q++];
  Xt_ = v[q++];
  Fx_ = v[q++];
  Ft_ = v[q++];
  G0_ = v[q++];
  Gt_ = v[q++];
  Sv_ = v[q++];
  const int nv = o.inner_m + o.outer_k + 1;
  V_.assign(nv, nullptr);
  for (int i = 1; i < nv; ++i) V_[i] = v[q++];
  outer_.assign(std::max(o.outer_k, 1), nullptr);
  for (int i = 0; i < std::max(o.outer_k, 1); ++i) outer_[i] = v[q++];
  osig_.assign(outer_.size(), 0.0);
  orn_.assign(outer_.size(), 0.0);
  if (hipHostMalloc(reinterpret_cast<void**>(&hS_), sizeof(ArnCtlState), 0) != hipSuccess ||
      hipHostMalloc(reinterpret_cast<void**>(&status_), sizeof(uint32_t) * (kMaxVec + 2), 0) !=
          hipSuccess ||
      hipMalloc(reinterpret_cast<void**>(&dS_), sizeof(ArnCtlState)) != hipSuccess ||
      hipMalloc(reinterpret_cast<void**>(&prm_), sizeof(double) * kCtlPrm) != hipSuccess) {
    init_status_ = NK_ENOMEM;
    return;
  }
  std::memset(hS_, 0, sizeof(ArnCtlState));
}

NewtonKrylov::~NewtonKrylov() {
  if (E_.s) hipStreamSynchronize(E_.s);
  if (hS_) hipHostFree(hS_);
  if (status_) hipHostFree(status_);
  if (dS_) hipFree(dS_);
  if (prm_) hipFree(prm_);
}


int NewtonKrylov::line_search(double* s_out, double* fnorm_new, double* fmax, double* xmax) {
  double tmp_s = 0.0, tmp_phi = fx_norm_ * fx_norm_;
  double tmp_fmax = 0.0, tmp_xmax = 0.0, tmp_sum = tmp_phi;
  int rc = NK_OK;
  auto phi = [&](double s) -> double {
    if (s == tmp_s) return tmp_phi;
    double red[3];
    rc = P_.eval(X_, d_, -s, Xt_, Ft_, Gt_, red);
    st_->nfev += 1;
    const double p = std::isfinite(red[0]) ? red[0] : INFINITY;
    tmp_s = s;
    tmp_phi = p;
    tmp_sum = red[0];
    tmp_fmax = std::isfinite(red[0]) ? red[1] : NAN;
    tmp_xmax = red[2];
    return p;
  };
  double s = 1.0;
  bool found = true;
  if (o_.line_search) {
    const double phi0 = tmp_phi, derphi0 = -tmp_phi, c1 = 1e-4, amin = 1e-2;
    double alpha0 = 1.0;
    const double thr = phi0 + c1 * alpha0 * derphi0;
    const int K = int(outer_.size());
    spec_.valid = false;
    Problem::SpecJvp sp{};
    const bool arm = P_.can_spec_jvp() && ocount_ > 0 && K > 0 && V_.size() > 1;
    if (arm) {
      const int slot = ohead_ % K;
      sp = Problem::SpecJvp{outer_[slot], osig_[slot], osig_[slot] * orn_[slot], thr, f_tol_,
                            rdiff_, V_[1]};
      if (sp.zn != 0.0) P_.arm_spec(&sp);
    }
    double phi_a0 = phi(alpha0);
    P_.arm_spec(nullptr);
    if (rc) return rc;
    if (arm && sp.zn != 0.0) {
      const bool ran = std::isfinite(tmp_sum) && tmp_sum <= thr && !(tmp_fmax <= f_tol_);
      if (ran) {
        spec_.valid = true;
        spec_.z = sp.z;
        spec_.zs = sp.zs;
        spec_.zn = sp.zn;
        spec_.w = sp.w;
        spec_.x = Xt_;
        spec_.g = Gt_;
      } else {
        E_.void_last(K_FDJVP, 1);
      }
    }
    if (phi_a0 <= phi0 + c1 * alpha0 * derphi0) {
      s = alpha0;
    } else {
      double alpha1 = -(derphi0)*alpha0 * alpha0 / 2.0 / (phi_a0 - phi0 - derphi0 * alpha0);
      double phi_a1 = phi(alpha1);
      if (rc) return rc;
      if (phi_a1 <= phi0 + c1 * alpha1 * derphi0) {
        s = alpha1;
      } else {
        found = false;
        while (alpha1 > amin) {
          const double factor = alpha0 * alpha0 * alpha1 * alpha1 * (alpha1 - alpha0);
          double a = alpha0 * alpha0 * (phi_a1 - phi0 - derphi0 * alpha1) -
                     alpha1 * alpha1 * (phi_a0 - phi0 - derphi0 * alpha0);
          a = a / factor;
          double b = -alpha0 * alpha0 * alpha0 * (phi_a1 - phi0 - derphi0 * alpha1) +
                     alpha1 * alpha1 * alpha1 * (phi_a0 - phi0 - derphi0 * alpha0);
          b = b / factor;
          double alpha2 = (-b + std::sqrt(std::fabs(b * b - 3 * a * derphi0))) / (3.0 * a);
          const double phi_a2 = phi(alpha2);
          if (rc) return rc;
          if (phi_a2 <= phi0 + c1 * alpha2 * derphi0) {
            s = alpha2;
            found = true;
            break;
          }
          if ((alpha1 - alpha2) > alpha1 / 2.0 || (1 - alpha2 / alpha1) < 0.96) alpha2 = alpha1 / 2.0;
          alpha0 = alpha1;
          alpha1 = alpha2;
          phi_a0 = phi_a1;
          phi_a1 = phi_a2;
        }
        if (!found) s = 1.0;
      }
    }
    if (s != tmp_s) phi(s);
    if (rc) return rc;
  } else {
    phi(1.0);
    if (rc) return rc;
  }
  *s_out = s;
  *fnorm_new = std::sqrt(tmp_sum);
  *fmax = tmp_fmax;
  *xmax = tmp_xmax;
  return NK_OK;
}

int NewtonKrylov::solve(const double* x_in, double* x_out, nk_stats* st) {
  if (init_status_) return init_status_;
  nk_stats dummy;
  st_ = st ? st : &dummy;
  std::memset(st_, 0, sizeof(nk_stats));
  st_->step_min = 1.0;
  steps_.clear();
  ocount_ = 0;
  ohead_ = 0;
  const int64_t n = E_.n;
  const double f_tol = std::isnan(o_.f_tol) ? std::pow(kEps, 1.0 / 3.0) : o_.f_tol;
  f_tol_ = f_tol;
  spec_.valid = false;
  const double f_rtol = std::isnan(o_.f_rtol) ? INFINITY : o_.f_rtol;
  const double x_tol = std::isnan(o_.x_tol) ? INFINITY : o_.x_tol;
  const double x_rtol = std::isnan(o_.x_rtol) ? INFINITY : o_.x_rtol;
  rdiff_ = (o_.rdiff > 0) ? o_.rdiff : std::pow(kEps, 0.5);
  const int64_t maxiter = (o_.maxiter > 0) ? o_.maxiter : 100 * (P_.n_global() + 1);
  const bool talk = o_.verbose && (!E_.comm || E_.comm->rank() == 0);

  int rc = P_.set_x0(x_in);
  double red[3];
  if (!rc) rc = P_.eval(x_in, x_in, 0.0, X_, Fx_, G0_, red);
  if (rc) return rc;
  st_->nfev = 1;
  fx_norm_ = std::sqrt(red[0]);
  double fmax = std::isfinite(red[0]) ? red[1] : NAN;
  double xmax = red[2];
  omega_ = rdiff_ * std::max(1.0, xmax) / std::max(1.0, fmax);
  const double gamma = 0.9, eta_max = 0.9999, eta_treshold = 0.1;
  double eta = 1e-3;
  double dxmax = INFINITY;
  double f0_norm = NAN;
  bool converged = false;
  int64_t it = 0;
  for (it = 0; it < maxiter; ++it) {
    const double f_norm = fmax;
    if (std::isnan(f0_norm)) f0_norm = f_norm;
    if (f_norm == 0.0 || ((f_norm <= f_tol && f_norm / f_rtol <= f0_norm) &&
                          (dxmax <= x_tol && dxmax / x_rtol <= xmax))) {
      converged = true;
      break;
    }
    const double tol = std::min(eta, eta * fx_norm_);
    double dnorm = 0.0, dmx = 0.0;
    rc = lgmres(tol, &dnorm, &dmx, &d_);
    if (rc) break;
    if (!(dnorm != 0.0) || d_ == nullptr) {
      rc = NK_ZERO_STEP;
      break;
    }
    dxmax = dmx;
    rc = P_.set_dir(d_);
    if (rc) break;
    double s = 1.0, fnorm_new = 0.0;
    rc = line_search(&s, &fnorm_new, &fmax, &xmax);
    if (rc) break;
    if (s != 1.0) st_->n_backtrack += 1;
    st_->step_min = std::min(st_->step_min, s);
    steps_.push_back(s);
    std::swap(X_, Xt_);
    std::swap(Fx_, Ft_);
    std::swap(G0_, Gt_);
    rc = P_.set_x0(X_);
    if (rc) break;
    omega_ = rdiff_ * std::max(1.0, xmax) / std::max(1.0, fmax);
    const double eta_A = gamma * fnorm_new * fnorm_new / (fx_norm_ * fx_norm_);
    if (gamma * eta * eta < eta_treshold)
      eta = std::min(eta_max, eta_A);
    else
      eta = std::min(eta_max, std::max(eta_A, gamma * eta * eta));
    fx_norm_ = fnorm_new;
    if (talk) {
      std::printf("%lld:  |F(x)| = %g; step %g\n", static_cast<long long>(it), fmax, s);
      std::fflush(stdout);
    }
  }
  st_->nit = it;
  st_->fnorm_inf = fmax;
  st_->fnorm_2 = fx_norm_;
  if (rc) {
    st_->status = rc;
    return rc;
  }
  rc = E_.copy(x_out, X_, n);
  if (!rc) rc = E_.sync();
  if (rc) return rc;
  st_->status = converged ? NK_OK : NK_NO_CONVERGENCE;
  return st_->status;
}

}
```

iterative-solvers-summer-2020_amd/csrc/nk_solver.h:

```cpp
#pragma once

#include <hip/hip_runtime.h>

#include <cstdint>
#include <string>
#include <vector>

#include "../../include/nkhip.h"
#include "comm.h"
#include "nk_kernels.h"

namespace nk {

enum Kind : int {
  K_FDJVP = 0,
  K_AJVP,
  K_TRIAL,
  K_BOLD,
  K_MDOT,
  K_COMBO,
  K_REDUCE,
  K_COPY,
  K_HALO,
  K_USERF,
  K_AXPBY,
  K_ARNOLDI,
  K_ARN_EDGE,
  K_EDGE,
  K_ARN_SLAB,
  K_CTL,
  K_PUSH,
  K_NKINDS
};

const char* kind_name(int kind);
void log_launch(int kind, double bytes);

struct KStat {
  int64_t launches = 0;
  double bytes = 0.0;
  int64_t timed = 0;
  double ms = 0.0;
  double tbytes = 0.0;
};

class Engine {
 public:
  Engine(int64_t n, nk_comm* comm, hipStream_t s, bool profile, int64_t min_partial = 0);
  ~Engine();
  Engine(const Engine&) = delete;
  Engine& operator=(const Engine&) = delete;

  int alloc(int count, std::vector<double*>* out, void* external = nullptr,
            int64_t external_bytes = 0);
  bool pool_chunk_mapped() const { return vmm_base_ != nullptr; }
  void enable_edges(int64_t ny, int64_t nx) {
    edge_ny_ = ny;
    edge_nx_ = nx;
  }
  double* edges(const double* v) const;
  int64_t pool_index(const double* v) const;
  int pool_count() const { return pool_count_; }
  void mark_edges(const double* v);
  bool edges_kept(const double* v) const;
  int gather_edges(const double* v);
  EdgeOut edge_out(const double* v);
  static int64_t pad(int64_t n) {
    const int64_t p = (n + 255) / 256 * 256;
    if (p < (int64_t(1) << 16)) return p;
    return (p + 32767) / 32768 * 32768 + 16384;
  }

  template <class L>
  int launch(int kind, double bytes, L&& fn) {
    return launch_on(kind, bytes, s, static_cast<L&&>(fn));
  }
  template <class L>
  int launch_on(int kind, double bytes, hipStream_t st, L&& fn);
  int reduce(int64_t nblk, int nsum, int nv, double* out);
  int reduce_async(int64_t nblk, int nsum, int nv, int slot, bool host_copy = true);
  const double* dres(int slot) const { return dres_ + slot; }
  const double* hres(int slot) const { return hres_ + slot; }
  double* dres_mut(int slot) const { return dres_ + slot; }
  double* hres_mut(int slot) const { return hres_ + slot; }
  static constexpr int kSlots = 1024;
  static int slot_mdot(int j) { return (j & 3) * 136; }
  static constexpr int kSlotCombo = 560;
  static constexpr int kSlotSync = 600;
  int sync();
  int wait_results(int slot, int nv);
  uint32_t wait_flag(const uint32_t* flag);
  int copy(double* dst, const double* src, int64_t n);
  void void_last(int kind, int count);

  double* partial() const { return partial_; }
  int64_t partial_cap() const { return partial_cap_; }
  const KStat& stat(int k) const { return stats_[k]; }
  void reset_stats();
  int64_t bytes_allocated() const { return bytes_; }

  int64_t n;
  int64_t npad;
  nk_comm* comm;
  hipStream_t s;
  bool profile;
  int sample = 1;

 private:
  void harvest();
  hipEvent_t ev();
  double* pool_ = nullptr;
  bool own_pool_ = false;
  int pool_count_ = 0;
  std::vector<uint8_t> ekept_;
  double* epool_ = nullptr;
  int64_t edge_ny_ = 0, edge_nx_ = 0, edge_n_ = 0;
  double* partial_ = nullptr;
  int64_t partial_cap_ = 0;
  double* dres_ = nullptr;
  double* hres_ = nullptr;
  int64_t bytes_ = 0;
  void* vmm_base_ = nullptr;
  size_t vmm_size_ = 0, vmm_chunk_ = 0;
  std::vector<hipMemGenericAllocationHandle_t> vmm_h_;
  int vmm_alloc(size_t bytes, size_t chunk);
  void vmm_free();
  struct Pending {
    int kind;
    hipEvent_t a, b;
    double bytes;
    int64_t idx;
  };
  static constexpr int kRecent = 8;
  double recent_bytes_[K_NKINDS][kRecent] = {};
  std::vector<Pending> pend_;
  std::vector<hipEvent_t> free_ev_;
  KStat stats_[K_NKINDS];
  int64_t tick_[K_NKINDS] = {};
};

template <class L>
int Engine::launch_on(int kind, double bytes, hipStream_t st, L&& fn) {
  hipEvent_t a = nullptr, b = nullptr;
  const bool timed = profile && (tick_[kind]++ % sample == 0);
  if (timed) {
    a = ev();
    hipEventRecord(a, st);
  }
  const hipError_t e = fn();
  if (timed) {
    b = ev();
    hipEventRecord(b, st);
    pend_.push_back(Pending{kind, a, b, bytes, stats_[kind].launches});
  }
  recent_bytes_[kind][stats_[kind].launches % kRecent] = bytes;
  stats_[kind].launches += 1;
  stats_[kind].bytes += bytes;
  log_launch(kind, bytes);
  return e == hipSuccess ? NK_OK : NK_EHIP;
}

struct Problem {
  virtual ~Problem() = default;
  virtual int64_t n_global() const = 0;
  virtual int eval(const double* x, const double* p, double alpha, double* xt, double* F,
                   double* G, double red[3]) = 0;
  virtual int jvp(const double* x0, const double* G0, const double* z, double zs, double sc,
                  double* w) = 0;
  virtual bool has_dev_scale() const { return false; }
  virtual int jvp_dev(const double* , const double* , const double* ,
                      const double* , double , double* ) {
    return NK_EINVAL;
  }
  virtual bool may_speculate() const { return true; }
  virtual bool has_jvp_prm() const { return false; }
  virtual int jvp_prm(const double* , const double* , const double* ,
                      const double* , double* ) {
    return NK_EINVAL;
  }
  virtual bool prefers_devctl() const { return false; }
  virtual bool has_fused(int ) const { return false; }
  virtual int fused_step(const double* const* , const double* , int ,
                         const double* , double , const double* ,
                         const double* , const double* , double , double ,
                         double* , double* , int64_t* ,
                         const double* , const ArnTail*  = nullptr,
                         bool*  = nullptr) {
    return NK_EINVAL;
  }
  virtual int publish_edges(const double* , bool  = false) { return NK_OK; }
  virtual EdgeOut edge_out(const double* ) { return EdgeOut{}; }
  virtual void void_fused_steps(int ) {}
  virtual int set_x0(const double* ) { return NK_OK; }
  virtual int set_dir(const double* ) { return NK_OK; }
  struct SpecJvp {
    const double* z;
    double zs, zn;
    double thr, ftol, rdiff;
    double* w;
  };
  virtual bool can_spec_jvp() const { return false; }
  virtual void arm_spec(const SpecJvp* ) {}
};

class NewtonKrylov {
 public:
  NewtonKrylov(Engine& E, Problem& P, const nk_opts& o, void* external = nullptr,
               int64_t external_bytes = 0);
  ~NewtonKrylov();
  NewtonKrylov(const NewtonKrylov&) = delete;
  NewtonKrylov& operator=(const NewtonKrylov&) = delete;
  int status() const { return init_status_; }
  void set_opts(const nk_opts& o) { o_ = o; }
  int solve(const double* x_in, double* x_out, nk_stats* st);
  static int vectors_needed(const nk_opts& o) { return o.inner_m + 2 * o.outer_k + 8; }
  const std::vector<double>& step_log() const { return steps_; }

 private:
  int lgmres(double tol, double* dnorm, double* dmax, double** dvec);
  int issue_step(int j, const double* z, double zs, double znorm, bool dev_scale,
                 bool have_w = false);
  int device_steps();
  const double* zp_[kMaxVec + 1];
  ArnCtlState* hS_ = nullptr;
  ArnCtlState* dS_ = nullptr;
  double* prm_ = nullptr;
  uint32_t* status_ = nullptr;
  int line_search(double* s_out, double* fnorm_new, double* fmax, double* xmax);

  Engine& E_;
  Problem& P_;
  nk_opts o_;
  int init_status_ = NK_OK;
  double *X_ = nullptr, *Xt_ = nullptr, *Fx_ = nullptr, *Ft_ = nullptr, *G0_ = nullptr,
         *Gt_ = nullptr;
  double* Sv_ = nullptr;
  std::vector<double*> V_;
  std::vector<double*> outer_;
  std::vector<double> osig_, orn_;
  int ocount_ = 0, ohead_ = 0;
  double omega_ = 0.0;
  double* d_ = nullptr;
  nk_stats* st_ = nullptr;
  std::vector<double> steps_;
  double fx_norm_ = 0.0;
  double rdiff_ = 0.0;
  double f_tol_ = 0.0;
  struct {
    bool valid = false;
    const double* z = nullptr;
    double zs = 0.0, zn = 0.0;
    double* w = nullptr;
    const double* x = nullptr;
    const double* g = nullptr;
  } spec_;
};

nk_opts default_opts();

namespace detail {
void givens(double a, double b, double* c, double* s);
void lstsq_upper(const double (*R)[kMaxVec + 1], int n, const double* g, double* y);
bool lstsq_upper_direct(const double (*R)[kMaxVec + 1], int n);
}

}
```

iterative-solvers-summer-2020_amd/csrc/sh_problem.cpp:

```cpp
#include "sh_problem.h"

#include <algorithm>
#include <cmath>
#include <cstdlib>
#include <cstring>

#include "peer_dev.h"

namespace nk {

SHProblem::SHProblem(Engine& E, int64_t ny, int64_t nx, int64_t ny_global, SHCoef c, int jvp_mode)
    : E_(E), ny_(ny), nx_(nx), ny_g_(ny_global), c_(c), jvp_mode_(jvp_mode) {
  if (arnoldi_supported(1, ny, nx)) E_.enable_edges(ny, nx);
  if (arnoldi_supported(1, ny, nx) && !(E_.comm && E_.comm->shares_device())) {
    const int64_t n = arnoldi_mbox_elems(ny, nx);
    if (hipMalloc(reinterpret_cast<void**>(&mb_), sizeof(double) * n) == hipSuccess &&
        hipMemset(mb_, 0, sizeof(double) * n) == hipSuccess) {
      mb_cap_ = n;
    } else {
      if (mb_) hipFree(mb_);
      mb_ = nullptr;
      (void)hipGetLastError();
    }
  }
  if (hipMalloc(reinterpret_cast<void**>(&B_), sizeof(double) * Engine::pad(ny * nx)) !=
      hipSuccess) {
    B_ = nullptr;
    status_ = NK_ENOMEM;
    return;
  }
  if (dist()) {
    if (ny < 2) {
      status_ = NK_EINVAL;
      return;
    }
    double* h = nullptr;
    if (hipMalloc(reinterpret_cast<void**>(&h), sizeof(double) * 24 * nx) != hipSuccess) {
      status_ = NK_ENOMEM;
      return;
    }
    hx_ = h;
    hz_ = h + 4 * nx;
    hd_ = h + 8 * nx;
    hu_ = h + 12 * nx;
    y4_ = h + 16 * nx;
    yh_ = h + 20 * nx;
    if (!E_.comm->claim_slots(this, &slots_) || slots_.ld < nx) {
      if (slots_.mine) E_.comm->release_slots(this);
      slots_ = nk_halo_slots{};
    }
    double mm[3] = {-double(ny), double(ny), slots_.mine ? 0.0 : 1.0};
    if (hipMemcpyAsync(y4_, mm, sizeof(mm), hipMemcpyHostToDevice, E_.s) != hipSuccess ||
        E_.comm->allreduce(y4_, 0, 3, E_.s) != NK_OK ||
        hipMemcpyAsync(mm, y4_, sizeof(mm), hipMemcpyDeviceToHost, E_.s) != hipSuccess ||
        hipStreamSynchronize(E_.s) != hipSuccess) {
      status_ = NK_ECOMM;
      return;
    }
    ny_min_ = int64_t(-mm[0]);
    ny_max_ = int64_t(mm[1]);
    if (mm[2] > 0.0 && slots_.mine) {
      E_.comm->release_slots(this);
      slots_ = nk_halo_slots{};
    }
    if (hipStreamCreateWithFlags(&side_, hipStreamNonBlocking) != hipSuccess ||
        hipEventCreateWithFlags(&ev_in_, hipEventDisableTiming) != hipSuccess ||
        hipEventCreateWithFlags(&ev_out_, hipEventDisableTiming) != hipSuccess) {
      status_ = NK_EHIP;
      return;
    }
  }
}

SHProblem::~SHProblem() {
  if (slots_.mine) E_.comm->release_slots(this);
  if (side_) hipStreamSynchronize(side_);
  if (B_) hipFree(B_);
  if (hx_) hipFree(hx_);
  if (mb_) hipFree(mb_);
  if (ev_in_) hipEventDestroy(ev_in_);
  if (ev_out_) hipEventDestroy(ev_out_);
  if (side_) hipStreamDestroy(side_);
}

namespace {
Field sub_field(const Field& f, int64_t r0, int64_t r1, int64_t ny, int64_t nx) {
  if (!f.base) return f;
  Field s;
  s.base = f.base + r0 * nx;
  s.lo = (r0 >= 2) ? f.base + (r0 - 2) * nx : (f.lo ? f.lo : f.base + (ny - 2) * nx);
  s.hi = (r1 + 2 <= ny) ? f.base + r1 * nx : (f.lo ? f.hi : f.base);
  return s;
}
}

StencilArgs stencil_rows(const StencilArgs& A, int64_t r0, int64_t r1) {
  StencilArgs B = A;
  B.ny = r1 - r0;
  B.a = sub_field(A.a, r0, r1, A.ny, A.nx);
  B.b = sub_field(A.b, r0, r1, A.ny, A.nx);
  const int64_t off = r0 * A.nx;
  B.e_row0 = A.e_row0 + r0;
  if (A.p0) B.p0 = A.p0 + off;
  if (A.out0) B.out0 = A.out0 + off;
  if (A.out1) B.out1 = A.out1 + off;
  if (A.out2) B.out2 = A.out2 + off;
  return B;
}

int SHProblem::halo_stencil(int kind, SMode m, const StencilArgs& A, const double* z, double* zh) {
  const double bytes = stencil_bytes_per_point(m, false);
  if (!z)
    return E_.launch(kind, bytes * ny_ * nx_, [&] { return stencil_launch(m, A, E_.s, nullptr); });
  if (!dist() || ny_ < 8 || !side_) {
    int rc = halo(z, zh);
    if (rc) return rc;
    return E_.launch(kind, bytes * ny_ * nx_,
                     [&] { return stencil_launch(m, A, E_.s, nullptr); });
  }
  if (hipEventRecord(ev_in_, E_.s) != hipSuccess ||
      hipStreamWaitEvent(side_, ev_in_, 0) != hipSuccess)
    return NK_EHIP;
  const StencilArgs I = stencil_rows(A, 2, ny_ - 2);
  if (stencil_launch(m, I, side_, nullptr) != hipSuccess) return NK_EHIP;
  if (hipEventRecord(ev_out_, side_) != hipSuccess) return NK_EHIP;
  int rc = halo(z, zh);
  if (rc) return rc;
  const StencilArgs T = stencil_rows(A, 0, 2), Bm = stencil_rows(A, ny_ - 2, ny_);
  rc = E_.launch(kind, bytes * ny_ * nx_, [&] {
    hipError_t e = stencil_launch(m, T, E_.s, nullptr);
    if (e == hipSuccess) e = stencil_launch(m, Bm, E_.s, nullptr);
    if (e == hipSuccess) e = hipStreamWaitEvent(E_.s, ev_out_, 0);
    return e;
  });
  return rc;
}

Field SHProblem::field(const double* p, const double* halo) const {
  if (!dist()) return periodic(p);
  return Field{p, halo, halo + 2 * nx_};
}

int SHProblem::halo(const double* v, double* h) {
  if (!dist()) return NK_OK;
  return E_.launch(K_HALO, 2.0 * 4 * 8 * nx_,
                   [&] {
                     return E_.comm->halo(v, h, h + 2 * nx_, ny_, nx_, E_.s) == NK_OK
                                ? hipSuccess
                                : hipErrorUnknown;
                   }) == NK_OK
             ? NK_OK
             : NK_ECOMM;
}

int SHProblem::prepare(const double* u_prev) {
  int rc = halo(u_prev, hu_);
  if (rc) return rc;
  StencilArgs A;
  A.ny = ny_;
  A.nx = nx_;
  A.a = field(u_prev, hu_);
  A.c = c_;
  A.out0 = B_;
  return E_.launch(K_BOLD, stencil_bytes_per_point(SMode::BOLD, false) * ny_ * nx_,
                   [&] { return stencil_launch(SMode::BOLD, A, E_.s, nullptr); });
}

int SHProblem::set_x0(const double* x0) {
  hxp_ = slot_halo(x0);
  if (hxp_) return NK_OK;
  hxp_ = hx_;
  return halo(x0, hx_);
}
int SHProblem::set_dir(const double* d) {
  hdp_ = slot_halo(d);
  if (hdp_) return NK_OK;
  hdp_ = hd_;
  return halo(d, hd_);
}

void SHProblem::set_push(StencilArgs* A, const double* out0, const double* out2) {
  if (!push_mode() || !A->E0) return;
  double* p0 = slot(slots_.prev, out0);
  double* n0 = slot(slots_.next, out0);
  if (!p0 || !n0) return;
  A->PS0[0] = p0;
  A->PS0[1] = n0;
  A->ps_ld = slots_.ld;
  pushed(out0);
  if (out2) {
    double* p2 = slot(slots_.prev, out2);
    double* n2 = slot(slots_.next, out2);
    if (p2 && n2) {
      A->PS2[0] = p2;
      A->PS2[1] = n2;
      pushed(out2);
    }
  }
}

void SHProblem::pushed(const double* v) {
  const int64_t q = E_.pool_index(v);
  if (q < 0) return;
  if (push_ep_.size() < size_t(E_.pool_count())) push_ep_.assign(E_.pool_count(), ~uint64_t(0));
  push_ep_[q] = E_.comm->epoch();
}

const double* SHProblem::slot_halo(const double* v) const {
  if (!push_mode() || slots_.ld != nx_ || !has_fused(1)) return nullptr;
  const int64_t q = E_.pool_index(v);
  if (q < 0 || size_t(q) >= push_ep_.size() || push_ep_[q] == ~uint64_t(0) ||
      !(E_.comm->epoch() > push_ep_[q]))
    return nullptr;
  return slots_.mine + q * 4 * slots_.ld;
}

bool SHProblem::push_mode() const {
  if (!slots_.mine || E_.pool_count() > slots_.count || slab_x_enabled(E_.comm)) return false;
  const char* e = std::getenv("NKHIP_SLAB_PUSH");
  return !(e && e[0] == '0');
}

double* SHProblem::slot(double* base, const double* v) const {
  const int64_t q = E_.pool_index(v);
  return q < 0 ? nullptr : base + q * 4 * slots_.ld;
}

int SHProblem::push(const double* v) {
  if (!push_mode() || !has_fused(1)) return NK_OK;
  double* pp = slot(slots_.prev, v);
  double* pn = slot(slots_.next, v);
  if (!pp || !pn) return NK_OK;
  const int rc = E_.launch(K_PUSH, 2.0 * 4 * 8 * nx_, [&] {
    return push_rows_launch(v, pp, pn, ny_, nx_, slots_.ld, E_.s);
  });
  if (!rc) pushed(v);
  return rc;
}

int SHProblem::eval(const double* x, const double* p, double alpha, double* xt, double* F,
                    double* G, double red[3]) {
  StencilArgs A;
  A.ny = ny_;
  A.nx = nx_;
  A.a = field(x, hxp_ ? hxp_ : hx_);
  A.b = (p == x) ? A.a : field(p, hdp_ ? hdp_ : hd_);
  A.alpha = alpha;
  A.p0 = B_;
  A.out0 = F;
  A.out1 = G;
  A.out2 = xt;
  A.c = c_;
  A.partial = E_.partial();
  set_edges(&A, F);
  if (A.E0 && xt && (A.E2 = E_.edges(xt)) != nullptr) E_.mark_edges(xt);
  set_push(&A, F, xt);
  int64_t nblk = 0;
  int rc = E_.launch(K_TRIAL, stencil_bytes_per_point(SMode::TRIAL, xt != nullptr) * ny_ * nx_,
                     [&] { return stencil_launch(SMode::TRIAL, A, E_.s, &nblk); });
  if (rc) return rc;
  const SpecJvp sp = spec_;
  spec_ = SpecJvp{};
  if (!sp.z || !xt || dist()) return E_.reduce(nblk, 1, 3, red);
  rc = E_.reduce_async(nblk, 1, 3, Engine::kSlotSync);
  if (!rc) {
    StencilArgs J;
    J.ny = ny_;
    J.nx = nx_;
    J.c = c_;
    J.out0 = sp.w;
    set_edges(&J, sp.w);
    J.a = field(xt, hx_);
    J.b = field(sp.z, hz_);
    J.p0 = G;
    J.spec = E_.dres(Engine::kSlotSync);
    J.spec_thr = sp.thr;
    J.spec_ftol = sp.ftol;
    J.spec_rdiff = sp.rdiff;
    J.spec_zn = sp.zn;
    J.spec_zs = sp.zs;
    side_edges(&J, xt, sp.z);
    rc = halo_stencil(K_FDJVP, SMode::FDJVP, J, nullptr, hz_);
  }
  if (!rc) rc = E_.wait_results(Engine::kSlotSync, 3);
  if (rc) return rc;
  std::memcpy(red, E_.hres(Engine::kSlotSync), sizeof(double) * 3);
  return NK_OK;
}

bool SHProblem::can_spec_jvp() const {
  const char* e = std::getenv("NKHIP_SPEC_JVP");
  return !dist() && jvp_mode_ == NK_JVP_FD && !(e && e[0] == '0');
}

int SHProblem::jvp(const double* x0, const double* G0, const double* z, double zs, double sc,
                   double* w) {
  StencilArgs A;
  A.ny = ny_;
  A.nx = nx_;
  A.c = c_;
  A.out0 = w;
  set_edges(&A, w);
  set_push(&A, w, nullptr);
  const double* zsh = slot_halo(z);
  if (jvp_mode_ == NK_JVP_ANALYTIC) {
    A.a = field(z, zsh ? zsh : hz_);
    A.alpha = zs;
    A.p0 = x0;
    const int rc = halo_stencil(K_AJVP, SMode::AJVP, A, zsh ? nullptr : z, hz_);
    return rc;
  }
  A.a = field(x0, hxp_ ? hxp_ : hx_);
  A.b = field(z, zsh ? zsh : hz_);
  A.alpha = sc * zs;
  A.p0 = G0;
  A.sc = sc;
  side_edges(&A, x0, z);
  const int rc = halo_stencil(K_FDJVP, SMode::FDJVP, A, zsh ? nullptr : z, hz_);
  return rc;
}

int SHProblem::jvp_dev(const double* x0, const double* G0, const double* z, const double* znorm2,
                       double omega, double* w) {
  StencilArgs A;
  A.ny = ny_;
  A.nx = nx_;
  A.c = c_;
  A.out0 = w;
  set_edges(&A, w);
  set_push(&A, w, nullptr);
  A.znorm2 = znorm2;
  A.omega = omega;
  const double* zsh = slot_halo(z);
  if (jvp_mode_ == NK_JVP_ANALYTIC) {
    A.a = field(z, zsh ? zsh : hz_);
    A.p0 = x0;
    const int rc = halo_stencil(K_AJVP, SMode::AJVP, A, zsh ? nullptr : z, hz_);
    return rc;
  }
  A.a = field(x0, hxp_ ? hxp_ : hx_);
  A.b = field(z, zsh ? zsh : hz_);
  A.p0 = G0;
  side_edges(&A, x0, z);
  const int rc = halo_stencil(K_FDJVP, SMode::FDJVP, A, zsh ? nullptr : z, hz_);
  return rc;
}

bool SHProblem::has_fused(int nv) const {
  const char* e = std::getenv("NKHIP_FUSED");
  if (e && e[0] == '0') return false;
  if (jvp_mode_ != NK_JVP_FD) return false;
  if (!dist()) return arnoldi_supported(nv, ny_, nx_);
  return arnoldi_supported(nv, ny_min_, nx_) && arnoldi_supported(nv, ny_max_, nx_);
}

int SHProblem::fused_step(const double* const* V, const double* c, int nv, const double* w,
                          double tau, const double* x0, const double* G0, const double* z,
                          double zs, double sc, double* out_v, double* out_w, int64_t* nwaves,
                          const double* ctl, const ArnTail* tail, bool* tail_used) {
  ArnoldiArgs A;
  A.ctl = ctl;
  if (tail_used) *tail_used = false;
  auto with_tail = [&] {
    if (!tail) return;
    A.tail = *tail;
    if (tail_used) *tail_used = true;
  };
  A.ny = ny_;
  A.nx = nx_;
  A.nv = nv;
  for (int i = 0; i < nv; ++i) {
    A.V[i] = V[i];
    A.c[i] = c[i];
  }
  A.w = w;
  A.tau = tau;
  A.x0 = x0;
  A.g0 = G0;
  A.z = z;
  A.alpha = sc * zs;
  A.sc = sc;
  A.k = c_;
  A.out_v = out_v;
  A.out_w = out_w;
  A.partial = E_.partial();
  A.partial_cap = E_.partial_cap();
  bool all = true;
  for (int i = 0; i < nv; ++i) all = all && (A.E[i] = E_.edges(V[i])) != nullptr;
  all = all && (A.E[nv] = E_.edges(w)) != nullptr;
  const char* eoff = std::getenv("NKHIP_EDGES");
  if (!all || (eoff && eoff[0] == '0'))
    for (int i = 0; i <= nv; ++i) A.E[i] = nullptr;
  A.Eout_v = E_.edges(out_v);
  A.Eout_w = E_.edges(out_w);
  if (A.Eout_v) E_.mark_edges(out_v);
  if (A.Eout_w) E_.mark_edges(out_w);
  if (mb_) {
    const int mode = arnoldi_mbox_mode();
    if (mode != 0) {
      A.mb = mb_;
      A.mb_cap = mb_cap_;
      A.mb_tag = ++mb_tag_;
      A.mb_recompute = mode == 2;
    }
  }
  const double rowb = 8.0 * double(nx_) * (nv + 4 + (z ? 1 : 0));
  if (!dist()) {
    with_tail();
    return E_.launch(K_ARNOLDI, rowb * ny_, [&] { return arnoldi_launch(A, E_.s, nwaves); });
  }

  if (push_mode()) {
    bool ok = true;
    for (int i = 0; i < nv; ++i) ok = ok && (A.HS[i] = slot(slots_.mine, V[i])) != nullptr;
    ok = ok && (A.HS[nv] = slot(slots_.mine, w)) != nullptr;
    if (z) ok = ok && (A.HS[nv + 1] = slot(slots_.mine, z)) != nullptr;
    ok = ok && (A.PS[0] = slot(slots_.prev, out_v)) != nullptr &&
         (A.PS[1] = slot(slots_.next, out_v)) != nullptr &&
         (A.PS[2] = slot(slots_.prev, out_w)) != nullptr &&
         (A.PS[3] = slot(slots_.next, out_w)) != nullptr;
    if (ok) {
      A.hs_ld = slots_.ld;
      pushed(out_v);
      pushed(out_w);
      A.yh = y4_;
      A.yh_ld = nx_;
      last_split_ = false;
      edge_launched_ = false;
      with_tail();
      return E_.launch(K_ARNOLDI, rowb * ny_, [&] { return arnoldi_launch(A, E_.s, nwaves); });
    }
    for (int i = 0; i <= nv + 1; ++i) A.HS[i] = nullptr;
    for (auto& p : A.PS) p = nullptr;
  }
  const char* ov = std::getenv("NKHIP_SLAB_OVERLAP");
  const bool split = ny_ >= 12 && side_ && (ov && ov[0] == '1');
  last_split_ = split;
  ArnoldiArgs I = A, T = A, Bm = A;
  int64_t nwI = 0, nwT = 0, nwB = 0;
  if (split) {
    I.r_begin = 2;
    I.r_end = ny_ - 2;
    static const int reserve = [] {
      const char* e = std::getenv("NKHIP_SLAB_RESERVE_CUS");
      return (e && *e) ? std::atoi(e) : 8;
    }();
    I.reserve_cus = reserve;
    T.r_begin = 0;
    T.r_end = 2;
    Bm.r_begin = ny_ - 2;
    Bm.r_end = ny_;
    I.plan_only = T.plan_only = Bm.plan_only = true;
    if (arnoldi_launch(I, E_.s, &nwI) != hipSuccess || arnoldi_launch(T, E_.s, &nwT) != hipSuccess ||
        arnoldi_launch(Bm, E_.s, &nwB) != hipSuccess)
      return NK_EHIP;
    I.plan_only = T.plan_only = Bm.plan_only = false;
    I.pstride = T.pstride = Bm.pstride = nwI + nwT + nwB;
    I.pcol0 = 0;
    T.pcol0 = nwI;
    Bm.pcol0 = nwI + nwT;
    if (hipEventRecord(ev_in_, E_.s) != hipSuccess || hipStreamWaitEvent(side_, ev_in_, 0) != hipSuccess)
      return NK_EHIP;
    int64_t nw = 0;
    int rc = E_.launch_on(K_ARNOLDI, rowb * (ny_ - 4), side_,
                          [&] { return arnoldi_launch(I, side_, &nw); });
    if (rc) return rc;
    if (hipEventRecord(ev_out_, side_) != hipSuccess) return NK_EHIP;
  }
  const double eb = 8.0 * 4 * nx_ * (z ? 2 : nv + 2);
  int rc = NK_OK;
  PeerArgs pa;
  edge_launched_ = true;
  if (!split && slab_x_enabled(E_.comm) && E_.comm->take_halo(&pa, nx_)) {
    const int par = int(pa.tag & 1);
    A.x.me = pa.base[pa.rank];
    A.x.prev = pa.base[(pa.rank - 1 + pa.P) % pa.P];
    A.x.next = pa.base[(pa.rank + 1) % pa.P];
    A.x.P = pa.P;
    A.x.max_nx = pa.max_nx;
    A.x.tag = pa.tag;
    A.x.err = pa.err;
    A.x.wait_ticks = pa.wait_ticks;
    A.yh = stage(A.x.me, pa.P, pa.max_nx, par, 0, 0);
    A.yh_ld = pa.max_nx;
    edge_launched_ = false;
    with_tail();
    return E_.launch(K_ARNOLDI, rowb * ny_, [&] { return arnoldi_launch(A, E_.s, nwaves); });
  }
  if (!split && peer_fuse_enabled() && E_.comm->take_halo(&pa, nx_)) {
    rc = E_.launch(K_ARN_EDGE, eb + 2.0 * 4 * 8 * nx_,
                   [&] { return arnoldi_edge_halo_launch(A, pa, yh_, E_.s); });
    if (rc) return rc;
  } else {
    rc = E_.launch(K_ARN_EDGE, eb, [&] { return arnoldi_edge_launch(A, y4_, E_.s); });
    if (rc) return rc;
    rc = E_.launch(K_HALO, 2.0 * 4 * 8 * nx_, [&] {
      return E_.comm->halo(y4_, yh_, yh_ + 2 * nx_, 4, nx_, E_.s) == NK_OK ? hipSuccess
                                                                         : hipErrorUnknown;
    });
    if (rc) return NK_ECOMM;
  }
  if (!split) {
    A.yh = yh_;
    with_tail();
    return E_.launch(K_ARNOLDI, rowb * ny_, [&] { return arnoldi_launch(A, E_.s, nwaves); });
  }
  T.yh = Bm.yh = yh_;
  int64_t nw = 0;
  rc = E_.launch(K_ARN_SLAB, rowb * 4, [&] {
    hipError_t e = arnoldi_launch(T, E_.s, &nw);
    if (e == hipSuccess) e = arnoldi_launch(Bm, E_.s, &nw);
    if (e == hipSuccess) e = hipStreamWaitEvent(E_.s, ev_out_, 0);
    return e;
  });
  *nwaves = nwI + nwT + nwB;
  return rc;
}

void SHProblem::void_fused_steps(int count) {
  E_.void_last(K_ARNOLDI, count);
  if (dist() && edge_launched_) E_.void_last(K_ARN_EDGE, count);
  if (last_split_) E_.void_last(K_ARN_SLAB, count);
}

void SHProblem::set_edges(StencilArgs* A, const double* out) {
  if (!has_fused(1)) return;
  A->E0 = E_.edges(out);
  A->e_ny = ny_;
  A->e_row0 = 0;
  if (A->E0) E_.mark_edges(out);
}

void SHProblem::side_edges(StencilArgs* A, const double* a, const double* b) const {
  const char* e = std::getenv("NKHIP_EDGES");
  if (!has_fused(1) || (e && e[0] == '0')) return;
  A->e_ny = ny_;
  A->e_row0 = 0;
  if (a && E_.edges_kept(a)) A->Ea = E_.edges(a);
  if (b && E_.edges_kept(b)) A->Eb = E_.edges(b);
}

int SHProblem::publish_edges(const double* v, bool written) {
  if (!has_fused(1)) return NK_OK;
  const int rc = written ? NK_OK : E_.gather_edges(v);
  return rc ? rc : push(v);
}

EdgeOut SHProblem::edge_out(const double* v) {
  const char* e = std::getenv("NKHIP_COMBO_EDGES");
  if (!has_fused(1) || (e && e[0] == '0')) return EdgeOut{};
  return E_.edge_out(v);
}

CallbackProblem::CallbackProblem(Engine& E, nk_residual_fn F, void* ctx, double* tmp, double* tmp2)
    : E_(E), F_(F), ctx_(ctx), tmp_(tmp), tmp2_(tmp2) {}

int CallbackProblem::norms(double* v, double* sum2, double* vmax) {
  VecList none;
  int64_t nblk = 0;
  int rc = E_.launch(K_COMBO, 16.0 * E_.n, [&] {
    return combo_launch(tmp2_, v, 1.0, none, 0, E_.n, E_.partial(), E_.s, &nblk);
  });
  if (rc) return rc;
  double red[2];
  rc = E_.reduce(nblk, 1, 2, red);
  *sum2 = red[0];
  *vmax = red[1];
  return rc;
}

int CallbackProblem::eval(const double* x, const double* p, double alpha, double* xt, double* F,
                          double* G, double red[3]) {
  const int64_t n = E_.n;
  const double* xe = x;
  if (xt || alpha != 0.0) {
    double* dst = xt ? xt : tmp_;
    int rc = E_.launch(K_AXPBY, 24.0 * n,
                       [&] { return axpby_launch(1.0, x, alpha, p, dst, n, E_.s); });
    if (rc) return rc;
    xe = dst;
  }
  int rc = E_.launch(K_USERF, 0.0, [&] {
    return F_(ctx_, xe, F, n) == 0 ? hipSuccess : hipErrorUnknown;
  });
  if (rc) return rc;
  double s2 = 0, fm = 0, xs = 0, xm = 0;
  rc = norms(F, &s2, &fm);
  if (!rc) rc = norms(const_cast<double*>(xe), &xs, &xm);
  if (rc) return rc;
  red[0] = s2;
// ... 21 lines not shown
```

iterative-solvers-summer-2020_amd/csrc/sh_problem.h:

```cpp
#pragma once

#include "nk_solver.h"

namespace nk {

class SHProblem final : public Problem {
 public:
  SHProblem(Engine& E, int64_t ny, int64_t nx, int64_t ny_global, SHCoef c, int jvp_mode);
  ~SHProblem() override;
  int status() const { return status_; }
  void set_jvp_mode(int m) { jvp_mode_ = m; }
  int64_t n_global() const override { return ny_g_ * nx_; }
  int prepare(const double* u_prev);
  int eval(const double* x, const double* p, double alpha, double* xt, double* F, double* G,
           double red[3]) override;
  int jvp(const double* x0, const double* G0, const double* z, double zs, double sc,
          double* w) override;
  bool has_dev_scale() const override { return true; }
  bool can_spec_jvp() const override;
  void arm_spec(const SpecJvp* sp) override { spec_ = sp ? *sp : SpecJvp{}; }
  int jvp_dev(const double* x0, const double* G0, const double* z, const double* znorm2,
              double omega, double* w) override;
  bool has_fused(int nv) const override;
  int fused_step(const double* const* V, const double* c, int nv, const double* w, double tau,
                 const double* x0, const double* G0, const double* z, double zs, double sc,
                 double* out_v, double* out_w, int64_t* nwaves, const double* ctl,
                 const ArnTail* tail = nullptr, bool* tail_used = nullptr) override;
  int set_x0(const double* x0) override;
  int set_dir(const double* d) override;
  int publish_edges(const double* v, bool written = false) override;
  EdgeOut edge_out(const double* v) override;
  void set_edges(StencilArgs* A, const double* out);
  void side_edges(StencilArgs* A, const double* a, const double* b) const;
  void void_fused_steps(int count) override;

 private:
  bool dist() const { return E_.comm != nullptr; }
  Field field(const double* p, const double* halo) const;
  int halo(const double* v, double* h);
  int halo_stencil(int kind, SMode m, const StencilArgs& A, const double* z, double* zh);
  bool push_mode() const;
  double* slot(double* base, const double* v) const;
  int push(const double* v);
  void pushed(const double* v);
  void set_push(StencilArgs* A, const double* out0, const double* out2);
  const double* slot_halo(const double* v) const;
  Engine& E_;
  int64_t ny_, nx_, ny_g_;
  SHCoef c_;
  int jvp_mode_;
  int status_ = NK_OK;
  double* B_ = nullptr;
  SpecJvp spec_{};
  double* hx_ = nullptr;
  double* hz_ = nullptr;
  double* hd_ = nullptr;
  double* hu_ = nullptr;
  double* y4_ = nullptr;
  double* yh_ = nullptr;
  int64_t ny_min_ = 0, ny_max_ = 0;
  hipStream_t side_ = nullptr;
  hipEvent_t ev_in_ = nullptr, ev_out_ = nullptr;
  double* mb_ = nullptr;
  int64_t mb_cap_ = 0;
  uint64_t mb_tag_ = 0;
  bool last_split_ = false;
  bool edge_launched_ = false;
  nk_halo_slots slots_{};
  std::vector<uint64_t> push_ep_;
  const double* hxp_ = nullptr;
  const double* hdp_ = nullptr;
};

class CallbackProblem final : public Problem {
 public:
  CallbackProblem(Engine& E, nk_residual_fn F, void* ctx, double* tmp, double* tmp2);
  int64_t n_global() const override { return E_.n; }
  int eval(const double* x, const double* p, double alpha, double* xt, double* F, double* G,
           double red[3]) override;
  int jvp(const double* x0, const double* G0, const double* z, double zs, double sc,
          double* w) override;
  bool may_speculate() const override { return false; }

 private:
  int norms(double* v, double* sum2, double* vmax);
  Engine& E_;
  nk_residual_fn F_;
  void* ctx_;
  double* tmp_;
  double* tmp2_;
};

}
```

iterative-solvers-summer-2020_amd/csrc/stencil.hip:

```cpp
#include <cmath>
#include <cstdlib>

#include "nk_device.h"
#include "nk_kernels.h"
#include "peer_dev.h"

namespace nk {

SHCoef sh_coef(double h, double r, double k, double g) {
  const double e = 1.0 / (h * h);
  SHCoef c;
  c.c0 = -20.0 * e * e + 8.0 * e + r - 1.0;
  c.c1 = 8.0 * e * e - 2.0 * e;
  c.c2 = -2.0 * e * e;
  c.c3 = -e * e;
  c.k = k;
  c.ik = 1.0 / k;
  c.g = g;
  return c;
}

namespace {

struct Nb {
  double c, a1, dg, a2;
};

struct Res {
  double o0, o1, o2;
};

__device__ __forceinline__ const double* rowp(const Field& f, int64_t r, int64_t ny, int64_t nx) {
  if (r >= 0 && r < ny) return f.base + r * nx;
  if (f.lo == nullptr) {
    r %= ny;
    if (r < 0) r += ny;
    return f.base + r * nx;
  }
  return (r < 0) ? f.lo + (r + 2) * nx : f.hi + (r - ny) * nx;
}

__device__ __forceinline__ const double* rowp_fast(const Field& f, int64_t r, int64_t ny,
                                                   int64_t nx) {
  const double* b = (r < 0) ? f.lo : ((r >= ny) ? f.hi : f.base);
  const int64_t rr = (r < 0) ? r + 2 : ((r >= ny) ? r - ny : r);
  return b + rr * nx;
}

__device__ __forceinline__ double applyL(const SHCoef& k, const Nb& n) {
  return k.c0 * n.c + k.c1 * n.a1 + k.c2 * n.dg + k.c3 * n.a2;
}

__device__ __forceinline__ double Gfun(const SHCoef& k, double w, double Lw) {
  const double ww = w * w;
  return w * k.ik - (Lw + k.g * ww - w * ww) / 2;
}

template <SMode M>
__device__ __forceinline__ Res finish(const StencilArgs& A, const Nb& na, const Nb& nb, double pv,
                                      double alpha, double sc) {
  Res r{0.0, 0.0, 0.0};
  const SHCoef& k = A.c;
  if constexpr (M == SMode::LAP5) {
    r.o0 = A.e * (na.a1 - 4.0 * na.c);
  } else if constexpr (M == SMode::SH13) {
    r.o0 = applyL(k, na);
  } else if constexpr (M == SMode::RESID) {
    const double u = na.c, uo = nb.c;
    const double uu = u * u, uouo = uo * uo;
    r.o0 = (u - uo) / k.k -
           (applyL(k, na) + k.g * uu - u * uu + applyL(k, nb) + k.g * uouo - uo * uouo) / 2;
  } else if constexpr (M == SMode::BOLD) {
    const double uo = na.c;
    const double uouo = uo * uo;
    r.o0 = -uo * k.ik - (applyL(k, na) + k.g * uouo - uo * uouo) / 2;
  } else if constexpr (M == SMode::TRIAL) {
    const double G = Gfun(k, na.c, applyL(k, na));
    r.o0 = G + pv;
    r.o1 = G;
    r.o2 = na.c;
  } else if constexpr (M == SMode::FDJVP) {
    r.o0 = (Gfun(k, na.c, applyL(k, na)) - pv) * sc;
  } else if constexpr (M == SMode::LINOP) {
    r.o0 = (1.0 + pv) * na.c - A.theta * applyL(k, na);
    r.o2 = na.c;
  } else {
    const double z = na.c, u = pv;
    r.o0 = alpha * (z * k.ik - (applyL(k, na) + (2.0 * k.g * u - 3.0 * u * u) * z) / 2);
  }
  return r;
}

template <SMode M>
constexpr bool kComb = (M == SMode::TRIAL || M == SMode::FDJVP || M == SMode::LINOP);
template <SMode M>
constexpr bool kRed = (M == SMode::TRIAL || M == SMode::LINOP);
template <SMode M>
constexpr bool kTwo = (M == SMode::RESID);
template <SMode M>
constexpr bool kHasP0 =
    (M == SMode::TRIAL || M == SMode::FDJVP || M == SMode::AJVP || M == SMode::LINOP);
template <SMode M>
constexpr int kRad = (M == SMode::LAP5) ? 1 : 2;

template <SMode M>
__device__ __forceinline__ bool jvp_scale(const StencilArgs& A, double* alpha, double* sc) {
  *alpha = A.alpha;
  *sc = A.sc;
  bool go = true;
  if constexpr (M == SMode::FDJVP || M == SMode::AJVP) {
    if (A.znorm2) {
      const double hn = sqrt(*A.znorm2);
      double sig = 1.0 / hn;
      if (!isfinite(sig)) sig = 1.0;
      if constexpr (M == SMode::FDJVP) {
        *sc = A.omega / (sig * hn);
        *alpha = *sc * sig;
      } else {
        *alpha = sig;
      }
    }
  }
  if constexpr (M == SMode::FDJVP) {
    if (A.spec) {
      const double red0 = A.spec[0], fm = A.spec[1], xm = A.spec[2];
      go = isfinite(red0) && red0 <= A.spec_thr && !(fm <= A.spec_ftol);
      const double omega = A.spec_rdiff * fmax(1.0, xm) / fmax(1.0, fm);
      *sc = omega / A.spec_zn;
      *alpha = *sc * A.spec_zs;
    }
    *sc = 1.0 / *sc;
  }
  return go;
}

typedef double dv2 __attribute__((ext_vector_type(2)));
__device__ __forceinline__ double2 ld_p0(const StencilArgs& A, const double* p) {
  if (A.nt_p0) {
    const dv2 v = __builtin_nontemporal_load(reinterpret_cast<const dv2*>(p));
    return make_double2(v.x, v.y);
  }
  return *reinterpret_cast<const double2*>(p);
}

template <SMode M>
constexpr int kFields = (kComb<M> || kTwo<M>) ? 2 : 1;

template <SMode M, int BX, int PF>
__global__ void __launch_bounds__(BX) march_kernel(StencilArgs A, int RY, int gx, int gy) {
  constexpr int R = kRad<M>;
  constexpr int NR = 2 * R + 1;
  constexpr int RING = NR + PF;
  constexpr int NF = kFields<M>;
  const int64_t nx = A.nx, ny = A.ny;
  const int64_t lb = (int64_t(blockIdx.x) % 8) * (int64_t(gridDim.x) / 8) + blockIdx.x / 8;
  if (lb >= int64_t(gx) * gy) return;
  const int64_t bx = lb % gx, by = lb / gx;
  const int64_t c0 = 2 * (bx * BX + threadIdx.x);
  const bool active = c0 < nx;
  const int64_t cc = active ? c0 : 0;
  const int64_t cm = (cc >= 2) ? cc - 2 : cc - 2 + nx;
  const int64_t cp = (cc + 2 < nx) ? cc + 2 : cc + 2 - nx;
  double alpha, sc;
  if (!jvp_scale<M>(A, &alpha, &sc)) return;

  static_assert(2 * BX == kEdgeW, "a march block is one edge group wide");
  const int64_t nbE = edge_groups(nx);
  const int64_t eL = (cc / kEdgeW) * A.e_ny * 4, eR = (((cc + 2) / kEdgeW) % nbE) * A.e_ny * 4 + 2;
  const bool sideL = threadIdx.x == 0, sideR = threadIdx.x == BX - 1;
  auto ld = [&](const Field& f, const double* E, int64_t r, double (&v)[6]) {
    const double* p = rowp_fast(f, r, ny, nx);
    const double* pl = p + cm;
    const double* pr = p + cp;
    if (E && r >= 0 && r < ny) {
      const int64_t er = (A.e_row0 + r) * 4;
      pl = sideL ? E + eL + er : pl;
      pr = sideR ? E + eR + er : pr;
    }
    const double2 x0 = *reinterpret_cast<const double2*>(pl);
    const double2 x1 = *reinterpret_cast<const double2*>(p + cc);
    const double2 x2 = *reinterpret_cast<const double2*>(pr);
    v[0] = x0.x; v[1] = x0.y; v[2] = x1.x; v[3] = x1.y; v[4] = x2.x; v[5] = x2.y;
  };
  double ring[NF][RING][6];
  auto load_row = [&](int slot, int64_t r) {
    r = (r > ny + 1) ? ny + 1 : ((r < -2) ? -2 : r);
    ld(A.a, A.Ea, r, ring[0][slot]);
    if constexpr (NF == 2) ld(A.b, A.Eb, r, ring[1][slot]);
  };
  auto combine = [&](int slot) {
    if constexpr (kComb<M>) {
#pragma unroll
      for (int q = 0; q < 6; ++q) ring[0][slot][q] = ring[0][slot][q] + alpha * ring[1][slot][q];
    }
  };
  auto ldp = [&](int64_t r) {
    r = (r >= ny) ? ny - 1 : ((r < 0) ? 0 : r);
    return ld_p0(A, A.p0 + r * nx + cc);
  };

  const int64_t band = A.rev ? int64_t(gy) - 1 - by : by;
  const int64_t r0 = band * RY;
  const int64_t r1 = (r0 + RY < ny) ? r0 + RY : ny;
  const bool up = (band & 1) != 0;
  const int64_t dir = up ? -1 : 1;
  const int64_t rs = up ? r1 - 1 : r0;
  const int64_t nrows = r1 - r0;

#pragma unroll
  for (int k = 0; k < RING - 1; ++k) load_row(k, rs + dir * (k - R));
  double2 pq[RING];
#pragma unroll
  for (int d = 0; d < RING; ++d) pq[d] = make_double2(0.0, 0.0);
  if constexpr (kHasP0<M>) {
#pragma unroll
    for (int d = 0; d < PF; ++d) pq[d] = ldp(rs + dir * d);
  }
#pragma unroll
  for (int k = 0; k < NR - 1; ++k) combine(k);

  double red[3] = {0.0, 0.0, 0.0};
  bool pushed = false;
  auto push_row = [&](double* const* ps, int64_t g, double2 v) {
    const bool top = g < 2, bot = g >= A.e_ny - 2;
    if (!(top || bot)) return;
    double* d = top ? ps[0] + (2 + g) * A.ps_ld : ps[1] + (g - (A.e_ny - 2)) * A.ps_ld;
    store_sys16(d + cc, v.x, v.y);
    pushed = true;
  };
  for (int64_t base = 0; base < nrows; base += RING) {
#pragma unroll
    for (int u = 0; u < RING; ++u) {
      const int64_t it = base + u;
      const int64_t r = rs + dir * it;
      load_row((u + RING - 1) % RING, r + dir * (R + PF));
      if constexpr (kHasP0<M>) pq[(u + PF) % RING] = ldp(r + dir * PF);
      combine((u + NR - 1) % RING);
      const double2 pv = pq[u % RING];
      auto W = [&](int m, int q) -> double { return ring[0][(u + m) % RING][q]; };
      auto Wb = [&](int m, int q) -> double { return ring[NF - 1][(u + m) % RING][q]; };
      Res res[2];
#pragma unroll
      for (int q = 0; q < 2; ++q) {
        Nb na, nb{0.0, 0.0, 0.0, 0.0};
        if constexpr (R == 2) {
          na.c = W(2, 2 + q);
          na.a1 = (W(2, 1 + q) + W(2, 3 + q)) + (W(1, 2 + q) + W(3, 2 + q));
          na.dg = (W(1, 1 + q) + W(1, 3 + q)) + (W(3, 1 + q) + W(3, 3 + q));
          na.a2 = (W(2, q) + W(2, 4 + q)) + (W(0, 2 + q) + W(4, 2 + q));
          if constexpr (kTwo<M>) {
            nb.c = Wb(2, 2 + q);
            nb.a1 = (Wb(2, 1 + q) + Wb(2, 3 + q)) + (Wb(1, 2 + q) + Wb(3, 2 + q));
            nb.dg = (Wb(1, 1 + q) + Wb(1, 3 + q)) + (Wb(3, 1 + q) + Wb(3, 3 + q));
            nb.a2 = (Wb(2, q) + Wb(2, 4 + q)) + (Wb(0, 2 + q) + Wb(4, 2 + q));
          }
        } else {
          na.c = W(1, 2 + q);
          na.a1 = (W(1, 1 + q) + W(1, 3 + q)) + (W(0, 2 + q) + W(2, 2 + q));
          na.dg = 0.0;
          na.a2 = 0.0;
        }
        res[q] = finish<M>(A, na, nb, q == 0 ? pv.x : pv.y, alpha, sc);
      }
      if (active && it < nrows) {
        const int64_t o = r * nx + cc;
        *reinterpret_cast<double2*>(A.out0 + o) = make_double2(res[0].o0, res[1].o0);
        if (A.PS0[0]) push_row(A.PS0, A.e_row0 + r, make_double2(res[0].o0, res[1].o0));
        if (A.E0) {
          const int64_t er = A.e_row0 + r;
          const double2 ev = make_double2(res[0].o0, res[1].o0);
          if (cc % kEdgeW == 0)
            *reinterpret_cast<double2*>(A.E0 + ((cc / kEdgeW) * A.e_ny + er) * 4 + 2) = ev;
          if ((cc + 2) % kEdgeW == 0 || cc + 2 == nx) {
            const int64_t b = (cc + 2 == nx) ? 0 : (cc + 2) / kEdgeW;
            *reinterpret_cast<double2*>(A.E0 + (b * A.e_ny + er) * 4) = ev;
          }
        }
        if constexpr (M == SMode::TRIAL) {
          *reinterpret_cast<double2*>(A.out1 + o) = make_double2(res[0].o1, res[1].o1);
          if (A.out2) *reinterpret_cast<double2*>(A.out2 + o) = make_double2(res[0].o2, res[1].o2);
          if (A.PS2[0]) push_row(A.PS2, A.e_row0 + r, make_double2(res[0].o2, res[1].o2));
          if (A.E2) {
            const int64_t er = A.e_row0 + r;
            const double2 ev = make_double2(res[0].o2, res[1].o2);
            if (cc % kEdgeW == 0)
              *reinterpret_cast<double2*>(A.E2 + ((cc / kEdgeW) * A.e_ny + er) * 4 + 2) = ev;
            if ((cc + 2) % kEdgeW == 0 || cc + 2 == nx) {
              const int64_t b = (cc + 2 == nx) ? 0 : (cc + 2) / kEdgeW;
              *reinterpret_cast<double2*>(A.E2 + (b * A.e_ny + er) * 4) = ev;
            }
          }
#pragma unroll
          for (int q = 0; q < 2; ++q) {
            red[0] += res[q].o0 * res[q].o0;
            red[1] = nmax(red[1], fabs(res[q].o0));
            red[2] = nmax(red[2], fabs(res[q].o2));
          }
        } else if constexpr (M == SMode::LINOP) {
          *reinterpret_cast<double2*>(A.out2 + o) = make_double2(res[0].o2, res[1].o2);
#pragma unroll
          for (int q = 0; q < 2; ++q) red[0] += res[q].o2 * res[q].o0;
        }
      }
    }
  }
  if (pushed) drain_stores();
  if constexpr (kRed<M>) {
    const double v = block_reduce<3, 1, BX>(red);
    const int64_t nblk = int64_t(gx) * gy;
    const int64_t bid = band * gx + bx;
    if (threadIdx.x < 3) A.partial[threadIdx.x * nblk + bid] = v;
  }
}

template <SMode M>
__global__ void __launch_bounds__(256) point_kernel(StencilArgs A) {
  constexpr int R = kRad<M>;
  const int64_t nx = A.nx, ny = A.ny;
  const int64_t idx = int64_t(blockIdx.x) * 256 + threadIdx.x;
  const bool active = idx < nx * ny;
  double alpha, sc;
  if (!jvp_scale<M>(A, &alpha, &sc)) return;
  double red[3] = {0.0, 0.0, 0.0};
  if (active) {
    const int64_t i = idx / nx, j = idx % nx;
    auto col = [&](int64_t dj) {
      int64_t c = (j + dj) % nx;
      if (c < 0) c += nx;
      return c;
    };
    auto val = [&](const Field& f, int64_t di, int64_t dj) {
      return rowp(f, i + di, ny, nx)[col(dj)];
    };
    auto wv = [&](int64_t di, int64_t dj) {
      double v = val(A.a, di, dj);
      if constexpr (kComb<M>) v = v + alpha * val(A.b, di, dj);
      return v;
    };
    Nb a, b{0.0, 0.0, 0.0, 0.0};
    a.c = wv(0, 0);
    a.a1 = (wv(0, -1) + wv(0, 1)) + (wv(-1, 0) + wv(1, 0));
    if constexpr (R == 2) {
      a.dg = (wv(-1, -1) + wv(-1, 1)) + (wv(1, -1) + wv(1, 1));
      a.a2 = (wv(0, -2) + wv(0, 2)) + (wv(-2, 0) + wv(2, 0));
    } else {
      a.dg = 0.0;
      a.a2 = 0.0;
    }
    if constexpr (kTwo<M>) {
      b.c = val(A.b, 0, 0);
      b.a1 = (val(A.b, 0, -1) + val(A.b, 0, 1)) + (val(A.b, -1, 0) + val(A.b, 1, 0));
      b.dg = (val(A.b, -1, -1) + val(A.b, -1, 1)) + (val(A.b, 1, -1) + val(A.b, 1, 1));
      b.a2 = (val(A.b, 0, -2) + val(A.b, 0, 2)) + (val(A.b, -2, 0) + val(A.b, 2, 0));
    }
    double pv = 0.0;
    if constexpr (kHasP0<M>) pv = A.p0[idx];
    const Res res = finish<M>(A, a, b, pv, alpha, sc);
    A.out0[idx] = res.o0;
    if constexpr (M == SMode::TRIAL) {
      A.out1[idx] = res.o1;
      if (A.out2) A.out2[idx] = res.o2;
      red[0] = res.o0 * res.o0;
      red[1] = fabs(res.o0);
      red[2] = fabs(res.o2);
    } else if constexpr (M == SMode::LINOP) {
      A.out2[idx] = res.o2;
      red[0] = res.o2 * res.o0;
    }
  }
  if constexpr (kRed<M>) {
    const double v = block_reduce<3, 1, 256>(red);
    if (threadIdx.x < 3) A.partial[threadIdx.x * int64_t(gridDim.x) + blockIdx.x] = v;
  }
}

template <SMode M, int ROWS, bool NTS>
__global__ void __launch_bounds__(256) tile_kernel(StencilArgs A, int gxt) {
  constexpr int R = kRad<M>;
  constexpr int NR = 2 * R + ROWS;
  const int64_t nx = A.nx, ny = A.ny;
  const int64_t lb = (int64_t(blockIdx.x) % 8) * (int64_t(gridDim.x) / 8) + blockIdx.x / 8;
  const int64_t nrb = (ny + ROWS - 1) / ROWS;
  if (lb >= int64_t(gxt) * nrb) return;
  const int64_t r0 = (lb / gxt) * ROWS;
  const int64_t c0 = 2 * ((lb % gxt) * 256 + threadIdx.x);
  if (c0 >= nx) return;
  const int64_t cm = (c0 >= 2) ? c0 - 2 : c0 - 2 + nx;
  const int64_t cp = (c0 + 2 < nx) ? c0 + 2 : c0 + 2 - nx;
  double w[NR][6];
#pragma unroll
  for (int m = 0; m < NR; ++m) {
    int64_t rr = r0 + m - R;
    rr = (rr > ny + 1) ? ny + 1 : rr;
    const double* p = rowp_fast(A.a, rr, ny, nx);
    const double2 x0 = *reinterpret_cast<const double2*>(p + cm);
    const double2 x1 = *reinterpret_cast<const double2*>(p + c0);
    const double2 x2 = *reinterpret_cast<const double2*>(p + cp);
    w[m][0] = x0.x; w[m][1] = x0.y; w[m][2] = x1.x; w[m][3] = x1.y; w[m][4] = x2.x; w[m][5] = x2.y;
  }
#pragma unroll
  for (int t = 0; t < ROWS; ++t) {
    Res res[2];
#pragma unroll
    for (int q = 0; q < 2; ++q) {
      Nb na, nb{0.0, 0.0, 0.0, 0.0};
      if constexpr (R == 2) {
        na.c = w[t + 2][2 + q];
        na.a1 = (w[t + 2][1 + q] + w[t + 2][3 + q]) + (w[t + 1][2 + q] + w[t + 3][2 + q]);
        na.dg = (w[t + 1][1 + q] + w[t + 1][3 + q]) + (w[t + 3][1 + q] + w[t + 3][3 + q]);
        na.a2 = (w[t + 2][q] + w[t + 2][4 + q]) + (w[t][2 + q] + w[t + 4][2 + q]);
      } else {
        na.c = w[t + 1][2 + q];
        na.a1 = (w[t + 1][1 + q] + w[t + 1][3 + q]) + (w[t][2 + q] + w[t + 2][2 + q]);
        na.dg = 0.0;
        na.a2 = 0.0;
      }
      res[q] = finish<M>(A, na, nb, 0.0, 0.0, 1.0);
    }
    if (r0 + t < ny) {
      dv2* o = reinterpret_cast<dv2*>(A.out0 + (r0 + t) * nx + c0);
      const dv2 v{res[0].o0, res[1].o0};
      if constexpr (NTS)
        __builtin_nontemporal_store(v, o);
      else
        *o = v;
    }
  }
}

bool aligned16(const void* p) { return (reinterpret_cast<uintptr_t>(p) & 15u) == 0; }

int env_int(const char* name, int dflt) {
  const char* v = std::getenv(name);
  return (v && *v) ? std::atoi(v) : dflt;
}

bool field_ok(const Field& f) {
  return f.base == nullptr ||
         (aligned16(f.base) && (f.lo == nullptr || (aligned16(f.lo) && aligned16(f.hi))));
}

template <SMode M>
hipError_t launch_mode(const StencilArgs& A, hipStream_t s, int64_t* nblk) {
  const bool fast = (A.nx % 2 == 0) && A.nx >= 2 && A.ny >= 2 && field_ok(A.a) && field_ok(A.b) &&
                    aligned16(A.p0) && aligned16(A.out0) && aligned16(A.out1) && aligned16(A.out2);
  if (fast) {
    StencilArgs B = A;
    for (Field* f : {&B.a, &B.b}) {
      if (f->base && !f->lo) {
        f->lo = f->base + (A.ny - 2) * A.nx;
        f->hi = f->base;
      }
    }
    if constexpr (M == SMode::LAP5 || M == SMode::SH13) {
      static const int64_t tile_max = env_int("NKHIP_TILE_MAX", 1 << 21);
      if (A.nx * A.ny <= tile_max && !A.E0 && !A.PS0[0]) {
        static const int rows = env_int("NKHIP_TILE_ROWS", 2);
        static const bool nts = env_int("NKHIP_TILE_NT", 1) != 0;
        const int rt = (rows == 4 || rows == 2) ? rows : 1;
        const int gxt = int((A.nx / 2 + 255) / 256);
        const int64_t nb = int64_t(gxt) * ((A.ny + rt - 1) / rt);
        if (nblk) *nblk = nb;
        const dim3 grid{unsigned((nb + 7) / 8 * 8), 1u, 1u};
        auto go = [&](auto kern) { hipLaunchKernelGGL(kern, grid, dim3(256), 0, s, B, gxt); };
        if (rt == 4)
          nts ? go(tile_kernel<M, 4, true>) : go(tile_kernel<M, 4, false>);
        else if (rt == 2)
          nts ? go(tile_kernel<M, 2, true>) : go(tile_kernel<M, 2, false>);
        else
          nts ? go(tile_kernel<M, 1, true>) : go(tile_kernel<M, 1, false>);
        return hipGetLastError();
      }
    }
    static const int blocks = env_int("NKHIP_BLOCKS", 4096);
    static const int pf = env_int("NKHIP_PF", 1);
    constexpr int BX = 128;
    constexpr int R = kRad<M>;
    const int ring = 2 * R + 1 + (pf == 2 ? 2 : 1);
    const int64_t gx = (A.nx / 2 + BX - 1) / BX;
    const int64_t want = (A.ny * gx) / blocks;
    int64_t k = (want + ring / 2) / ring;
    if (k < 1) k = 1;
    if (k > 6) k = 6;
    const int RY = int(k * ring);
    const int64_t gy = (A.ny + RY - 1) / RY;
    if (gx * gy > (int64_t(1) << 31) - 8) return hipErrorInvalidValue;
    if (nblk) *nblk = gx * gy;
    B.rev = (A.rev_force >= 0) ? A.rev_force != 0 : traversal_reverse();
    static const bool nt_p0 = env_int("NKHIP_NT_P0", 1) != 0;
    B.nt_p0 = nt_p0;
    const dim3 grid{unsigned((gx * gy + 7) / 8 * 8), 1u, 1u};
    if (pf == 2)
      hipLaunchKernelGGL((march_kernel<M, BX, 2>), grid, dim3(BX), 0, s, B, RY, int(gx), int(gy));
    else
      hipLaunchKernelGGL((march_kernel<M, BX, 1>), grid, dim3(BX), 0, s, B, RY, int(gx), int(gy));
  } else {
    if (A.E0 || A.E2 || A.Ea || A.Eb || A.PS0[0] || A.PS2[0])
      return hipErrorInvalidValue;
    const int64_t n = A.nx * A.ny;
    const int64_t g = (n + 255) / 256;
    if (nblk) *nblk = g;
    hipLaunchKernelGGL((point_kernel<M>), dim3(unsigned(g)), dim3(256), 0, s, A);
  }
  return hipGetLastError();
}

}

hipError_t stencil_launch(SMode m, const StencilArgs& a, hipStream_t s, int64_t* nblk) {
  if (a.nx <= 0 || a.ny <= 0) return hipSuccess;
  switch (m) {
    case SMode::LAP5: return launch_mode<SMode::LAP5>(a, s, nblk);
    case SMode::SH13: return launch_mode<SMode::SH13>(a, s, nblk);
    case SMode::RESID: return launch_mode<SMode::RESID>(a, s, nblk);
    case SMode::BOLD: return launch_mode<SMode::BOLD>(a, s, nblk);
    case SMode::TRIAL: return launch_mode<SMode::TRIAL>(a, s, nblk);
    case SMode::FDJVP: return launch_mode<SMode::FDJVP>(a, s, nblk);
    case SMode::AJVP: return launch_mode<SMode::AJVP>(a, s, nblk);
    case SMode::LINOP: return launch_mode<SMode::LINOP>(a, s, nblk);
  }
  return hipErrorInvalidValue;
}

int64_t stencil_partial_slots(int64_t ny, int64_t nx) {
  const int64_t march = ((nx / 2 + 127) / 128) * ((ny + 3) / 4);
  const int64_t point = (nx * ny + 255) / 256;
  return 3 * (march > point ? march : point) + 3;
}

double stencil_bytes_per_point(SMode m, bool has_xt) {
  switch (m) {
    case SMode::LAP5: return 16.0;
    case SMode::SH13: return 16.0;
    case SMode::RESID: return 24.0;
    case SMode::BOLD: return 16.0;
    case SMode::TRIAL: return has_xt ? 48.0 : 40.0;
    case SMode::FDJVP: return 32.0;
    case SMode::AJVP: return 24.0;
    case SMode::LINOP: return 40.0;
  }
  return 0.0;
}

}
```

iterative-solvers-summer-2020_amd/nkhip/_lib.py:

```python
from __future__ import annotations

import ctypes as C
import os

import torch

LIB_PATH = os.path.join(os.path.dirname(os.path.abspath(__file__)), "libnkhip.so")
LIB_PATH = os.environ.get("NKHIP_LIB") or LIB_PATH

NK_OK = 0
NK_NO_CONVERGENCE = 1
NK_NONFINITE = 2
NK_ZERO_STEP = 3
NK_BAD_RHS = 4
NK_EINVAL = -1
NK_EHIP = -2
NK_ECOMM = -3
NK_ENOMEM = -4
ABI_VERSION = 3
NK_JVP_FD = 0
NK_JVP_ANALYTIC = 1


class nk_opts(C.Structure):
    _fields_ = [("f_tol", C.c_double), ("f_rtol", C.c_double), ("x_tol", C.c_double),
                ("x_rtol", C.c_double), ("rdiff", C.c_double), ("maxiter", C.c_int64),
                ("inner_m", C.c_int32), ("outer_k", C.c_int32), ("line_search", C.c_int32),
                ("jvp_mode", C.c_int32), ("verbose", C.c_int32), ("profile", C.c_int32)]


class nk_stats(C.Structure):
    _fields_ = [("nit", C.c_int64), ("nfev", C.c_int64), ("njvp", C.c_int64),
                ("n_arnoldi", C.c_int64), ("fnorm_inf", C.c_double), ("fnorm_2", C.c_double),
                ("status", C.c_int32), ("pad_", C.c_int32), ("n_backtrack", C.c_int64),
                ("step_min", C.c_double), ("n_device_steps", C.c_int64)]

    def as_dict(self):
        return {k: getattr(self, k) for k, _ in self._fields_ if k != "pad_"}


class nk_kprof(C.Structure):
    _fields_ = [("name", C.c_char * 32), ("launches", C.c_int64), ("total_ms", C.c_double),
                ("alg_bytes", C.c_double), ("timed", C.c_int64), ("timed_bytes", C.c_double)]


class nk_drop_params(C.Structure):
    _fields_ = [("nx", C.c_int32), ("ny", C.c_int32), ("endl", C.c_double), ("endr", C.c_double),
                ("endb", C.c_double), ("endt", C.c_double), ("epsilon", C.c_double),
                ("n_exp", C.c_int32), ("m_exp", C.c_int32), ("Bo", C.c_double),
                ("alpha2", C.c_double), ("alpha", C.c_double), ("gamma", C.c_double),
                ("C", C.c_double), ("smoothing_iters", C.c_int32), ("pad_", C.c_int32),
                ("a", C.c_double)]


class nk_mems_params(C.Structure):
    _fields_ = [("n", C.c_int32), ("m", C.c_int32), ("smoothing_iters", C.c_int32),
                ("p", C.c_int32), ("alpha", C.c_double), ("gamma", C.c_double),
                ("epsilon", C.c_double), ("beta", C.c_double), ("lambd", C.c_double),
                ("endl", C.c_double), ("endr", C.c_double), ("k", C.c_double)]


class nk_stencil_pass(C.Structure):
    _fields_ = ([(n, C.c_int64) for n in ("mode", "ny", "nx", "r0", "r1")]
                + [(n, C.c_void_p) for n in ("a", "a_halo", "b", "b_halo", "p0", "out0", "out1",
                                             "out2")]
                + [(n, C.c_double) for n in ("alpha", "sc", "e", "theta", "h", "r", "k", "g")]
                + [("znorm2", C.c_void_p), ("omega", C.c_double), ("spec", C.c_void_p)]
                + [(n, C.c_double) for n in ("spec_thr", "spec_ftol", "spec_rdiff", "spec_zn",
                                             "spec_zs")]
                + [(n, C.c_void_p) for n in ("Ea", "Eb", "E0", "E2")]
                + [("PS0", C.c_void_p * 2), ("PS2", C.c_void_p * 2), ("ps_ld", C.c_int64),
                   ("rev", C.c_int64)])


RESIDUAL_FN = C.CFUNCTYPE(C.c_int, C.c_void_p, C.c_void_p, C.c_void_p, C.c_int64)

_P = C.c_void_p
_D = C.c_double
_I64 = C.c_int64
_I32 = C.c_int32

SIGNATURES = [
    ("nk_version", C.c_char_p, []),
    ("nk_abi_version", C.c_int, []),
    ("nk_opts_default", C.c_int, [C.POINTER(nk_opts)]),
    ("nk_status_string", C.c_char_p, [C.c_int]),
    ("nk_lap5_apply", C.c_int, [_P, _P, _I64, _I64, _D, _P]),
    ("nk_sh13_apply", C.c_int, [_P, _P, _I64, _I64, _D, _D, _P]),
    ("nk_sh_residual", C.c_int, [_P, _P, _P, _I64, _I64, _D, _D, _D, _D, _P]),
    ("nk_sh_jvp", C.c_int, [_P, _P, _P, _I64, _I64, _D, _D, _D, _D, _P]),
    ("nk_sh_fdjvp", C.c_int, [_P, _P, _P, _P, _I64, _I64, _D, _D, _D, _D, _D, _D, _P]),
    ("nk_sh_arnoldi_fused", C.c_int, [C.POINTER(_P), C.POINTER(_D), _I32, _P, _D, _P, _P, _P,
                                      _I64, _I64, _D, _D, _D, _D, _D, _D, _P, _P,
                                      C.POINTER(_D), _P]),
    ("nk_edge_elems", C.c_int64, [_I64, _I64]),
    ("nk_arnoldi_mbox_launches", C.c_int64, []),
    ("nk_edge_gather", C.c_int, [_P, _P, _I64, _I64, _P]),
    ("nk_sh_arnoldi_fused_edges", C.c_int, [C.POINTER(_P), C.POINTER(_P), C.POINTER(_D), _I32,
                                            _P, _D, _P, _P, _P, _I64, _I64, _D, _D, _D, _D, _D,
                                            _D, _P, _P, _P, _P, C.POINTER(_D), _P]),
    ("nk_dot", C.c_int, [_P, _P, _I64, C.POINTER(_D), _P]),
    ("nk_nrm2", C.c_int, [_P, _I64, C.POINTER(_D), _P]),
    ("nk_maxnorm", C.c_int, [_P, _I64, C.POINTER(_D), _P]),
    ("nk_axpy", C.c_int, [_D, _P, _P, _I64, _P]),
    ("nk_scal", C.c_int, [_D, _P, _I64, _P]),
    ("nk_mdot", C.c_int, [C.POINTER(_P), _I32, _P, _I64, C.POINTER(_D), _P]),
    ("nk_maxpy", C.c_int, [C.POINTER(_P), C.POINTER(_D), _I32, _P, _I64, _P]),
    ("nk_stream_copy", C.c_int, [_P, _P, _I64, _P]),
    ("nk_debug_bounds", C.c_int, [C.POINTER(_I64), C.POINTER(_I32), _I32]),
    ("nk_debug_mailbox", C.c_int, [C.POINTER(_I64), _I32]),
    ("nk_debug_close", C.c_int, [C.POINTER(_P), C.POINTER(_D), C.POINTER(_D), C.POINTER(_D), _I32,
                                 _I64, _P, _P, C.POINTER(_D), _P]),
    ("nk_debug_ctl_step", C.c_int, [_I32, _I32, _P, _P, _P, _P, _P, _P, _P, _P, _P, _P, _P, _P]),
    ("nk_debug_stencil", C.c_int, [C.POINTER(nk_stencil_pass), C.POINTER(_D), C.POINTER(_I64),
                                   _P]),
    ("nk_comm_unique_id_bytes", C.c_int, []),
    ("nk_comm_get_unique_id", C.c_int, [_P]),
    ("nk_comm_create_rccl", C.c_int, [C.POINTER(_P), _P, _I32, _I32]),
    ("nk_comm_create_loopback", C.c_int, [C.POINTER(_P), _I32]),
    ("nk_comm_peer_handle_bytes", C.c_int, []),
    ("nk_comm_create_peer", C.c_int, [C.POINTER(_P), _I32, _I32, _I64, _P]),
    ("nk_comm_peer_connect", C.c_int, [_P, _P]),
    ("nk_comm_destroy", C.c_int, [_P]),
    ("nk_comm_abort", C.c_int, [_P]),
    ("nk_comm_selftest", C.c_int, [_P, _I64, _P]),
    ("nk_comm_selftest_push", C.c_int, [_P, _I64, _P]),
    ("nk_sh_create", C.c_int, [C.POINTER(_P), _I64, _I64, _I64, _D, _D, _D, _D,
                               C.POINTER(nk_opts), _P, _P]),
    ("nk_sh_destroy", C.c_int, [_P]),
    ("nk_sh_step", C.c_int, [_P, _P, _P, C.POINTER(nk_stats)]),
    ("nk_sh_set_opts", C.c_int, [_P, C.POINTER(nk_opts)]),
    ("nk_sh_kernel_profile", C.c_int, [_P, C.POINTER(nk_kprof), _I32]),
    ("nk_sh_reset_profile", C.c_int, [_P]),
    ("nk_sh_step_log", C.c_int, [_P, C.POINTER(_D), _I32]),
    ("nk_sh_workspace_bytes", C.c_int64, [_P]),
    ("nk_solve_workspace_bytes", C.c_int64, [_I64, C.POINTER(nk_opts)]),
    ("nk_solve", C.c_int, [RESIDUAL_FN, _P, _P, _P, _I64, C.POINTER(nk_opts),
                           C.POINTER(nk_stats), _P, _P, _I64]),
    ("nk_drop_params_default", C.c_int, [C.POINTER(nk_drop_params)]),
    ("nk_drop_create", C.c_int, [C.POINTER(_P), C.POINTER(nk_drop_params), C.POINTER(nk_opts),
                                 _P]),
    ("nk_drop_destroy", C.c_int, [_P]),
    ("nk_drop_lds_fits", C.c_int, [_I32, _I32]),
    ("nk_drop_set_state", C.c_int, [_P, _P, _P]),
    ("nk_drop_get_state", C.c_int, [_P, _P, _P]),
    ("nk_drop_step", C.c_int, [_P, _D, _D, _I32, C.POINTER(nk_stats), C.POINTER(_D),
                               C.POINTER(_D)]),
    ("nk_drop_set_scale", C.c_int, [_P, _D]),
    ("nk_drop_prepare", C.c_int, [_P]),
    ("nk_drop_field", C.c_int, [_P, _I32, _P]),
    ("nk_drop_residual", C.c_int, [_P, _P, _D, _P]),
    ("nk_drop_solve", C.c_int, [_P, _D, _P, C.POINTER(nk_stats)]),
    ("nk_drop_pma", C.c_int, [_P, _D, _I32]),
    ("nk_drop_init_coalescing", C.c_int, [_P, _I32, C.POINTER(_D), _I32, _D, _I32]),
    ("nk_shlin_create", C.c_int, [C.POINTER(_P), _I64, _I64, _D, _D, _D, _D, _D, _I64, _P]),
    ("nk_shlin_destroy", C.c_int, [_P]),
    ("nk_shlin_step", C.c_int, [_P, _P, _P, _P, C.POINTER(_I64), C.POINTER(_D)]),
    ("nk_mems_params_default", C.c_int, [C.POINTER(nk_mems_params)]),
    ("nk_mems_create", C.c_int, [C.POINTER(_P), C.POINTER(nk_mems_params), C.POINTER(nk_opts),
                                 _P]),
    ("nk_mems_destroy", C.c_int, [_P]),
    ("nk_mems_set_state", C.c_int, [_P, _P, _P]),
    ("nk_mems_get_state", C.c_int, [_P, _P, _P]),
    ("nk_mems_step", C.c_int, [_P, C.POINTER(nk_stats), C.POINTER(_D), C.POINTER(_D)]),
    ("nk_mems_prepare", C.c_int, [_P, C.POINTER(_D)]),
    ("nk_mems_field", C.c_int, [_P, _I32, _P]),
    ("nk_mems_residual", C.c_int, [_P, _P, _P]),
]


def load(path: str = LIB_PATH) -> C.CDLL:
    if not os.path.exists(path):
        raise ImportError(
            f"nkhip: {path} is missing -- build it with `make -C iterative-solvers-summer-2020_amd` "
            "(or __graft_entry__.build()); there is no CPU fallback")
    lib = C.CDLL(path)
    for name, res, args in SIGNATURES:
        fn = getattr(lib, name)
        fn.restype = res
        fn.argtypes = args
    got = lib.nk_abi_version()
    if got != ABI_VERSION:
        raise ImportError(f"nkhip: {path} has C-ABI version {got}, this binding expects "
                          f"{ABI_VERSION} (rebuild the library)")
    return lib


lib = load()


def status_string(code: int) -> str:
    return lib.nk_status_string(int(code)).decode()


def default_opts() -> nk_opts:
    o = nk_opts()
    lib.nk_opts_default(C.byref(o))
    return o


class NKError(RuntimeError):
    """A HIP / RCCL / argument failure inside libnkhip."""


def check(rc: int, what: str) -> int:
    if rc < 0:
        raise NKError(f"{what}: {status_string(rc)} ({rc})")
    return rc
```

iterative-solvers-summer-2020_amd/nkhip/ops.py:

```python
from __future__ import annotations

import ctypes as C

import torch

from ._lib import check, lib


def _stream():
    return C.c_void_p(torch.cuda.current_stream().cuda_stream)


def _dev(t: torch.Tensor, name: str) -> torch.Tensor:
    if not isinstance(t, torch.Tensor) or not t.is_cuda:
        raise TypeError(f"{name} must be a CUDA (HIP) tensor")
    if t.dtype != torch.float64:
        raise TypeError(f"{name} must be float64 (the reference computes in fp64)")
    if not t.is_contiguous():
        raise ValueError(f"{name} must be contiguous")
    return t


def _ptr(t: torch.Tensor):
    return C.c_void_p(t.data_ptr())


def _grid(v: torch.Tensor, ny, nx):
    if ny is None or nx is None:
        if v.dim() != 2:
            raise ValueError("pass a 2-D (ny, nx) grid or ny/nx explicitly")
        ny, nx = v.shape
    if v.numel() != ny * nx:
        raise ValueError(f"grid {ny}x{nx} does not match {v.numel()} values")
    return int(ny), int(nx)


def lap5_apply(v, e, ny=None, nx=None, out=None):
    _dev(v, "v")
    ny, nx = _grid(v, ny, nx)
    out = torch.empty_like(v) if out is None else _dev(out, "out")
    check(lib.nk_lap5_apply(_ptr(v), _ptr(out), ny, nx, float(e), _stream()), "nk_lap5_apply")
    return out


def sh13_apply(v, h, r, ny=None, nx=None, out=None):
    _dev(v, "v")
    ny, nx = _grid(v, ny, nx)
    out = torch.empty_like(v) if out is None else _dev(out, "out")
    check(lib.nk_sh13_apply(_ptr(v), _ptr(out), ny, nx, float(h), float(r), _stream()),
          "nk_sh13_apply")
    return out


def sh_residual(u, uo, h, r, k, g, ny=None, nx=None, out=None):
    _dev(u, "u")
    _dev(uo, "uo")
    ny, nx = _grid(u, ny, nx)
    out = torch.empty_like(u) if out is None else _dev(out, "out")
    check(lib.nk_sh_residual(_ptr(u), _ptr(uo), _ptr(out), ny, nx, float(h), float(r), float(k),
                             float(g), _stream()), "nk_sh_residual")
    return out


def sh_jvp(u, v, h, r, k, g, ny=None, nx=None, out=None):
    _dev(u, "u")
    _dev(v, "v")
    ny, nx = _grid(u, ny, nx)
    out = torch.empty_like(u) if out is None else _dev(out, "out")
    check(lib.nk_sh_jvp(_ptr(u), _ptr(v), _ptr(out), ny, nx, float(h), float(r), float(k),
                        float(g), _stream()), "nk_sh_jvp")
    return out


def sh_fdjvp(x0, G0, z, h, r, k, g, zs, sc, ny=None, nx=None, out=None):
    for t, nm in ((x0, "x0"), (G0, "G0"), (z, "z")):
        _dev(t, nm)
    ny, nx = _grid(x0, ny, nx)
    out = torch.empty_like(x0) if out is None else _dev(out, "out")
    check(lib.nk_sh_fdjvp(_ptr(x0), _ptr(G0), _ptr(z), _ptr(out), ny, nx, float(h), float(r),
                          float(k), float(g), float(zs), float(sc), _stream()), "nk_sh_fdjvp")
    return out


def sh_arnoldi_fused(V, coef, w, tau, x0, G0, h, r, k, g, zs, sc, z=None, ny=None, nx=None,
                     v_out=None, w_out=None, reduce=True, E=None, Ev_out=None, Ew_out=None):
    for t, nm in ((w, "w"), (x0, "x0")):
        _dev(t, nm)
    ny, nx = _grid(x0, ny, nx)
    nv = len(V)
    ptrs = (C.c_void_p * max(nv, 1))(*[_dev(v, "V[i]").data_ptr() for v in V])
    cf = (C.c_double * max(nv, 1))(*[float(c) for c in coef])
    v_out = torch.empty_like(x0) if v_out is None else _dev(v_out, "v_out")
    w_out = torch.empty_like(x0) if w_out is None else _dev(w_out, "w_out")
    dots = (C.c_double * (2 * nv + 3))() if reduce else None
    zp = _ptr(_dev(z, "z")) if z is not None else None
    common = (cf, nv, _ptr(w), float(tau), _ptr(x0), _ptr(G0) if G0 is not None else None, zp,
              ny, nx, float(h), float(r), float(k), float(g), float(zs), float(sc), _ptr(v_out),
              _ptr(w_out))
    if E is None:
        check(lib.nk_sh_arnoldi_fused(ptrs, *common, dots, _stream()), "nk_sh_arnoldi_fused")
    else:
        if len(E) != nv + 1:
            raise ValueError("E holds the edge arrays of V[0..nv-1] and w")
        eptrs = (C.c_void_p * (nv + 1))(*[_dev(e, "E[i]").data_ptr() for e in E])
        check(lib.nk_sh_arnoldi_fused_edges(
            ptrs, eptrs, *common, _ptr(Ev_out) if Ev_out is not None else None,
            _ptr(Ew_out) if Ew_out is not None else None, dots, _stream()),
            "nk_sh_arnoldi_fused_edges")
    return v_out, w_out, (list(dots) if reduce else None)


def arnoldi_mbox_launches() -> int:
    return int(lib.nk_arnoldi_mbox_launches())


def edge_gather(v, ny=None, nx=None, out=None):
    _dev(v, "v")
    ny, nx = _grid(v, ny, nx)
    n = int(lib.nk_edge_elems(ny, nx))
    out = torch.empty(n, dtype=torch.float64, device=v.device) if out is None else out
    check(lib.nk_edge_gather(_ptr(v), _ptr(out), ny, nx, _stream()), "nk_edge_gather")
    return out


def dot(x, y) -> float:
    _dev(x, "x")
    _dev(y, "y")
    r = C.c_double()
    check(lib.nk_dot(_ptr(x), _ptr(y), x.numel(), C.byref(r), _stream()), "nk_dot")
    return r.value


def nrm2(x) -> float:
    _dev(x, "x")
    r = C.c_double()
    check(lib.nk_nrm2(_ptr(x), x.numel(), C.byref(r), _stream()), "nk_nrm2")
    return r.value


def maxnorm(x) -> float:
    _dev(x, "x")
    r = C.c_double()
    check(lib.nk_maxnorm(_ptr(x), x.numel(), C.byref(r), _stream()), "nk_maxnorm")
    return r.value


def axpy(a, x, y):
    _dev(x, "x")
    _dev(y, "y")
    check(lib.nk_axpy(float(a), _ptr(x), _ptr(y), x.numel(), _stream()), "nk_axpy")
    return y


def scal(a, x):
    _dev(x, "x")
    check(lib.nk_scal(float(a), _ptr(x), x.numel(), _stream()), "nk_scal")
    return x


def mdot(V, w):
    _dev(w, "w")
    m = len(V)
    ptrs = (C.c_void_p * max(m, 1))(*[_dev(v, "V[i]").data_ptr() for v in V])
    out = (C.c_double * max(m, 1))()
    check(lib.nk_mdot(ptrs, m, _ptr(w), w.numel(), out, _stream()), "nk_mdot")
    return [out[i] for i in range(m)]


def maxpy(V, coef, y):
    _dev(y, "y")
    m = len(V)
    ptrs = (C.c_void_p * max(m, 1))(*[_dev(v, "V[i]").data_ptr() for v in V])
    cs = (C.c_double * max(m, 1))(*[float(c) for c in coef])
    check(lib.nk_maxpy(ptrs, cs, m, _ptr(y), y.numel(), _stream()), "nk_maxpy")
    return y


def lgmres_close(P, cN, cA, cB, A=None, B=None):
    m = len(P)
    if m < 1 or not (len(cN) == len(cA) == len(cB) == m):
        raise ValueError("lgmres_close: one (cN, cA, cB) triple per vector, at least one vector")
    for i, p in enumerate(P):
        _dev(p, "P[i]")
        if p.numel() != P[0].numel():
            raise ValueError("lgmres_close: size mismatch")
    if len({p.data_ptr() for p in P}) != m:
        raise ValueError("lgmres_close: the vectors must be distinct (one list entry per tensor)")
    A = torch.empty_like(P[0]) if A is None else _dev(A, "A")
    B = torch.empty_like(P[0]) if B is None else _dev(B, "B")
    if A.numel() != P[0].numel() or B.numel() != P[0].numel():
        raise ValueError("lgmres_close: size mismatch")
    ptrs = (C.c_void_p * m)(*[p.data_ptr() for p in P])
    arr = [(C.c_double * m)(*[float(c) for c in cs]) for cs in (cN, cA, cB)]
    r = C.c_double()
    check(lib.nk_debug_close(ptrs, *arr, m, P[0].numel(), _ptr(A), _ptr(B), C.byref(r),
                             _stream()), "nk_debug_close")
    return A, B, r.value


STENCIL_MODES = ("LAP5", "SH13", "RESID", "BOLD", "TRIAL", "FDJVP", "AJVP", "LINOP")


def stencil_pass(mode, ny, nx, a, out0, *, b=None, p0=None, out1=None, out2=None, a_halo=None,
                 b_halo=None, rows=None, alpha=0.0, sc=1.0, e=0.0, theta=0.0, h=1.0, r=0.0, k=1.0,
                 g=0.0, znorm2=None, omega=0.0, spec=None, spec_thr=0.0, spec_ftol=0.0,
                 spec_rdiff=0.0, spec_zn=1.0, spec_zs=1.0, Ea=None, Eb=None, E0=None, E2=None,
                 PS0=None, PS2=None, ps_ld=0, rev=-1):
    from ._lib import nk_stencil_pass

    m = STENCIL_MODES.index(mode) if isinstance(mode, str) else int(mode)
    ny, nx = int(ny), int(nx)
    P = nk_stencil_pass()
    P.mode, P.ny, P.nx = m, ny, nx
    P.r0, P.r1 = (0, -1) if rows is None else (int(rows[0]), int(rows[1]))

    def dev(t, name, n):
        if t is None:
            return None
        _dev(t, name)
        if t.numel() < n:
            raise ValueError(f"stencil_pass: {name} holds {t.numel()} values, needs {n}")
        return t.data_ptr()

    n = ny * nx
    for name, t in (("a", a), ("b", b), ("p0", p0), ("out0", out0), ("out1", out1),
                    ("out2", out2)):
        setattr(P, name, dev(t, name, n))
    P.a_halo = dev(a_halo, "a_halo", 4 * nx)
    P.b_halo = dev(b_halo, "b_halo", 4 * nx)
    P.alpha, P.sc, P.e, P.theta = float(alpha), float(sc), float(e), float(theta)
    P.h, P.r, P.k, P.g = float(h), float(r), float(k), float(g)
    P.znorm2, P.omega = dev(znorm2, "znorm2", 1), float(omega)
    P.spec = dev(spec, "spec", 3)
    P.spec_thr, P.spec_ftol, P.spec_rdiff = float(spec_thr), float(spec_ftol), float(spec_rdiff)
    P.spec_zn, P.spec_zs = float(spec_zn), float(spec_zs)
    ne = int(lib.nk_edge_elems(ny, nx))
    for name, t in (("Ea", Ea), ("Eb", Eb), ("E0", E0), ("E2", E2)):
        setattr(P, name, dev(t, name, ne))
    P.ps_ld = int(ps_ld)
    for name, pair in (("PS0", PS0), ("PS2", PS2)):
        if pair is not None:
            if len(pair) != 2 or P.ps_ld < nx:
                raise ValueError(f"stencil_pass: {name} is a (prev, next) pair of slots, ps_ld >= nx")
            arr = getattr(P, name)
            for i, t in enumerate(pair):
                arr[i] = dev(t, name, 4 * P.ps_ld)
    P.rev = int(rev)
    red = (C.c_double * 3)()
    nblk = C.c_int64(0)
    check(lib.nk_debug_stencil(C.byref(P), red, C.byref(nblk), _stream()), "nk_debug_stencil")
    nred = {4: 3, 7: 1}.get(m, 0)
    return [red[i] for i in range(nred)], nblk.value


def stream_copy(src, out=None):
    src = _dev(src, "src")
    out = torch.empty_like(src) if out is None else _dev(out, "out")
    if out.numel() != src.numel():
        raise ValueError("stream_copy: size mismatch")
    check(lib.nk_stream_copy(_ptr(src), _ptr(out), src.numel(), _stream()), "nk_stream_copy")
    return out
```

Before: 32.25.

## Fuse Arnoldi dots into FD JVP stencil and drop stored G buffer

```diff
diff --git a/include/nkhip.h b/include/nkhip.h
--- a/include/nkhip.h
+++ b/include/nkhip.h
@@ -146,6 +146,8 @@
   int64_t rev;
 } nk_stencil_pass;
 int nk_debug_stencil(const nk_stencil_pass* p, double* red, int64_t* nblk, void* stream);
+int nk_debug_stencil_callpass(const nk_stencil_pass* p, const double* q, double* red,
+                              int64_t* nblk, void* stream);
 
 int nk_comm_unique_id_bytes(void);
 int nk_comm_get_unique_id(void* out);
diff --git a/iterative-solvers-summer-2020_amd/csrc/capi.cpp b/iterative-solvers-summer-2020_amd/csrc/capi.cpp
--- a/iterative-solvers-summer-2020_amd/csrc/capi.cpp
+++ b/iterative-solvers-summer-2020_amd/csrc/capi.cpp
@@ -447,15 +447,24 @@
   return hip_rc(e);
 }
 
-int nk_debug_stencil(const nk_stencil_pass* p, double* red, int64_t* nblk_out, void* stream) {
+namespace {
+int debug_stencil(const nk_stencil_pass* p, const double* q, bool callpass, double* red,
+                  int64_t* nblk_out, void* stream) {
   if (!p || p->mode < 0 || p->mode > 7 || p->ny <= 0 || p->nx <= 0 || !p->a || !p->out0)
     return NK_EINVAL;
   const SMode m = static_cast<SMode>(int(p->mode));
   const bool two = m == SMode::RESID || m == SMode::TRIAL || m == SMode::FDJVP || m == SMode::LINOP;
-  const bool has_p0 = m == SMode::TRIAL || m == SMode::FDJVP || m == SMode::AJVP || m == SMode::LINOP;
-  const bool reduces = m == SMode::TRIAL || m == SMode::LINOP;
-  if ((two && !p->b) || (has_p0 && !p->p0) || (m == SMode::TRIAL && !p->out1) ||
-      (m == SMode::LINOP && !p->out2) || (reduces && !red))
+  const bool cp = callpass && (m == SMode::TRIAL || m == SMode::FDJVP);
+  const bool has_p0 = !cp && (m == SMode::TRIAL || m == SMode::FDJVP || m == SMode::AJVP ||
+                              m == SMode::LINOP);
+  const bool dots = cp && m == SMode::FDJVP && !p->p0 && q;
+  const bool reduces = m == SMode::TRIAL || m == SMode::LINOP || dots;
+  if ((two && !p->b) || (has_p0 && !p->p0) || (m == SMode::TRIAL && !cp && !p->out1) ||
+      (m == SMode::LINOP && !p->out2) || (reduces && !red) || (q && !dots) ||
+      (reinterpret_cast<uintptr_t>(q) & 15u))
+    return NK_EINVAL;
+  if (cp && m == SMode::TRIAL && !p->p0 &&
+      !(p->out1 && p->alpha == 0.0 && p->b == p->a && p->b_halo == p->a_halo))
     return NK_EINVAL;
   if (m == SMode::FDJVP && !p->znorm2 && !p->spec && !(p->sc != 0.0)) return NK_EINVAL;
   const bool ranged = p->r1 >= 0;
@@ -484,6 +493,7 @@
   if (p->b) A.b = (p->b == p->a && p->b_halo == p->a_halo) ? A.a : field(p->b, p->b_halo);
   A.alpha = p->alpha;
   A.p0 = p->p0;
+  A.q = q;
   A.out0 = p->out0;
   A.out1 = p->out1;
   A.out2 = p->out2;
@@ -530,9 +540,10 @@
   int64_t nblk = 0;
   e = stencil_launch(m, R, s, &nblk);
   double host[3] = {0.0, 0.0, 0.0};
-  const int nv = m == SMode::TRIAL ? 3 : 1;
+  const int nv = (m == SMode::TRIAL || dots) ? 3 : 1;
   if (reduces && e == hipSuccess && 3 * nblk > slots) e = hipErrorInvalidValue;
-  if (reduces && e == hipSuccess) e = reduce_final_launch(buf, nblk, 1, nv, buf + slots, nullptr, s);
+  if (reduces && e == hipSuccess)
+    e = reduce_final_launch(buf, nblk, dots ? 3 : 1, nv, buf + slots, nullptr, s);
   if (reduces && e == hipSuccess)
     e = hipMemcpyAsync(host, buf + slots, sizeof(double) * nv, hipMemcpyDeviceToHost, s);
   if (buf) hipFreeAsync(buf, s);
@@ -541,6 +552,16 @@
   for (int i = 0; reduces && i < nv; ++i) red[i] = host[i];
   if (nblk_out) *nblk_out = nblk;
   return NK_OK;
+}
+}
+
+int nk_debug_stencil(const nk_stencil_pass* p, double* red, int64_t* nblk_out, void* stream) {
+  return debug_stencil(p, nullptr, false, red, nblk_out, stream);
+}
+
+int nk_debug_stencil_callpass(const nk_stencil_pass* p, const double* q, double* red,
+                              int64_t* nblk_out, void* stream) {
+  return debug_stencil(p, q, true, red, nblk_out, stream);
 }
 
 int nk_comm_unique_id_bytes(void) { return comm_unique_id_bytes(); }
diff --git a/iterative-solvers-summer-2020_amd/csrc/lgmres.cpp b/iterative-solvers-summer-2020_amd/csrc/lgmres.cpp
--- a/iterative-solvers-summer-2020_amd/csrc/lgmres.cpp
+++ b/iterative-solvers-summer-2020_amd/csrc/lgmres.cpp
@@ -39,28 +39,37 @@
 }
 
 int NewtonKrylov::issue_step(int j, const double* z, double zs, double znorm, bool dev_scale,
-                             bool have_w) {
+                             bool have_w, bool have_dots) {
   const int64_t n = E_.n;
   zp_[j] = z;
   hS_->zs[j] = zs;
   double* w = V_[j + 1];
   int rc;
+  if (j == 0 && !have_w && !dev_scale && znorm != 0.0 && P_.has_step0()) {
+    int64_t nb = 0;
+    rc = P_.jvp_dots(X_, z, zs, omega_ / znorm, V_[0], w, &nb);
+    if (rc) return rc;
+    st_->njvp += 1;
+    st_->n_arnoldi += 1;
+    return E_.reduce_async(nb, 3, 3, Engine::slot_mdot(0));
+  }
   if (have_w) {
     rc = NK_OK;
     st_->njvp += 1;
   } else if (dev_scale) {
-    rc = P_.jvp_dev(X_, G0_, z, E_.dres(Engine::kSlotCombo), omega_, w);
+    rc = P_.jvp_dev(X_, gbuf(G0_), z, E_.dres(Engine::kSlotCombo), omega_, w);
     st_->njvp += 1;
   } else if (znorm == 0.0) {
     rc = E_.launch(K_COPY, 8.0 * n,
                    [&] { return hipMemsetAsync(w, 0, sizeof(double) * n, E_.s); });
     if (!rc) rc = P_.publish_edges(w);
   } else {
-    rc = P_.jvp(X_, G0_, z, zs, omega_ / znorm, w);
+    rc = P_.jvp(X_, gbuf(G0_), z, zs, omega_ / znorm, w);
     st_->njvp += 1;
   }
   if (rc) return rc;
   st_->n_arnoldi += 1;
+  if (have_w && have_dots) return NK_OK;
   VecList P;
   for (int i = 0; i <= j; ++i) P.p[i] = V_[i];
   int64_t nblk = 0;
@@ -161,7 +170,7 @@
     const bool have = spec_.valid && n_o > 0 && z == spec_.z && zs == spec_.zs &&
                       zn == spec_.zn && V_[1] == spec_.w && X_ == spec_.x && G0_ == spec_.g;
     spec_.valid = false;
-    rc = issue_step(0, z, zs, zn, false, have);
+    rc = issue_step(0, z, zs, zn, false, have, have && spec_.dots);
   }
   sig_est[0] = 0.0;
   if (!rc) rc = E_.sync();
@@ -494,7 +503,7 @@
       for (int i = 0; i <= t; ++i) U.p[i] = V_[i];
       int rc = E_.launch(K_COMBO, 8.0 * n * (t + 3),
                          [&] { return combo_prm_launch(w, w, prm_, U, t + 1, n, E_.s); });
-      if (!rc) rc = P_.jvp_prm(X_, G0_, w, prm_, V_[t + 2]);
+      if (!rc) rc = P_.jvp_prm(X_, gbuf(G0_), w, prm_, V_[t + 2]);
       if (rc) return rc;
       zp_[t + 1] = w;
       rot[t].unfused = true;
diff --git a/iterative-solvers-summer-2020_amd/csrc/nk_kernels.h b/iterative-solvers-summer-2020_amd/csrc/nk_kernels.h
--- a/iterative-solvers-summer-2020_amd/csrc/nk_kernels.h
+++ b/iterative-solvers-summer-2020_amd/csrc/nk_kernels.h
@@ -46,6 +46,7 @@
   Field a{}, b{};
   double alpha = 0.0;
   const double* p0 = nullptr;
+  const double* q = nullptr;
   double* out0 = nullptr;
   double* out1 = nullptr;
   double* out2 = nullptr;
@@ -74,9 +75,10 @@
 bool traversal_reverse();
 
 StencilArgs stencil_rows(const StencilArgs& A, int64_t r0, int64_t r1);
+int stencil_variant(SMode m, const StencilArgs& A);
 hipError_t stencil_launch(SMode m, const StencilArgs& a, hipStream_t s, int64_t* nblk);
 int64_t stencil_partial_slots(int64_t ny, int64_t nx);
-double stencil_bytes_per_point(SMode m, bool has_xt);
+double stencil_bytes_per_point(SMode m, bool has_xt, int variant = 0);
 
 constexpr int kMaxVec = 64;
 struct VecList {
diff --git a/iterative-solvers-summer-2020_amd/csrc/nk_solver.cpp b/iterative-solvers-summer-2020_amd/csrc/nk_solver.cpp
--- a/iterative-solvers-summer-2020_amd/csrc/nk_solver.cpp
+++ b/iterative-solvers-summer-2020_amd/csrc/nk_solver.cpp
@@ -497,7 +497,7 @@
   auto phi = [&](double s) -> double {
     if (s == tmp_s) return tmp_phi;
     double red[3];
-    rc = P_.eval(X_, d_, -s, Xt_, Ft_, Gt_, red);
+    rc = P_.eval(X_, d_, -s, Xt_, Ft_, gbuf(Gt_), red);
     st_->nfev += 1;
     const double p = std::isfinite(red[0]) ? red[0] : INFINITY;
     tmp_s = s;
@@ -536,6 +536,7 @@
         spec_.w = sp.w;
         spec_.x = Xt_;
         spec_.g = Gt_;
+        spec_.dots = P_.spec_dots();
       } else {
         E_.void_last(K_FDJVP, 1);
       }
@@ -610,7 +611,7 @@
 
   int rc = P_.set_x0(x_in);
   double red[3];
-  if (!rc) rc = P_.eval(x_in, x_in, 0.0, X_, Fx_, G0_, red);
+  if (!rc) rc = P_.eval(x_in, x_in, 0.0, X_, Fx_, gbuf(G0_), red);
   if (rc) return rc;
   st_->nfev = 1;
   fx_norm_ = std::sqrt(red[0]);
diff --git a/iterative-solvers-summer-2020_amd/csrc/nk_solver.h b/iterative-solvers-summer-2020_amd/csrc/nk_solver.h
--- a/iterative-solvers-summer-2020_amd/csrc/nk_solver.h
+++ b/iterative-solvers-summer-2020_amd/csrc/nk_solver.h
@@ -200,6 +200,13 @@
     double* w;
   };
   virtual bool can_spec_jvp() const { return false; }
+  virtual bool needs_g() const { return true; }
+  virtual bool has_step0() const { return false; }
+  virtual int jvp_dots(const double* , const double* , double , double ,
+                       const double* , double* , int64_t* ) {
+    return NK_EINVAL;
+  }
+  virtual bool spec_dots() const { return false; }
   virtual void arm_spec(const SpecJvp* ) {}
 };
 
@@ -219,7 +226,7 @@
  private:
   int lgmres(double tol, double* dnorm, double* dmax, double** dvec);
   int issue_step(int j, const double* z, double zs, double znorm, bool dev_scale,
-                 bool have_w = false);
+                 bool have_w = false, bool have_dots = false);
   int device_steps();
   const double* zp_[kMaxVec + 1];
   ArnCtlState* hS_ = nullptr;
@@ -253,7 +260,9 @@
     double* w = nullptr;
     const double* x = nullptr;
     const double* g = nullptr;
+    bool dots = false;
   } spec_;
+  double* gbuf(double* g) const { return P_.needs_g() ? g : nullptr; }
 };
 
 nk_opts default_opts();
diff --git a/iterative-solvers-summer-2020_amd/csrc/sh_problem.cpp b/iterative-solvers-summer-2020_amd/csrc/sh_problem.cpp
--- a/iterative-solvers-summer-2020_amd/csrc/sh_problem.cpp
+++ b/iterative-solvers-summer-2020_amd/csrc/sh_problem.cpp
@@ -102,6 +102,7 @@
   const int64_t off = r0 * A.nx;
   B.e_row0 = A.e_row0 + r0;
   if (A.p0) B.p0 = A.p0 + off;
+  if (A.q) B.q = A.q + off;
   if (A.out0) B.out0 = A.out0 + off;
   if (A.out1) B.out1 = A.out1 + off;
   if (A.out2) B.out2 = A.out2 + off;
@@ -109,7 +110,7 @@
 }
 
 int SHProblem::halo_stencil(int kind, SMode m, const StencilArgs& A, const double* z, double* zh) {
-  const double bytes = stencil_bytes_per_point(m, false);
+  const double bytes = stencil_bytes_per_point(m, false, stencil_variant(m, A));
   if (!z)
     return E_.launch(kind, bytes * ny_ * nx_, [&] { return stencil_launch(m, A, E_.s, nullptr); });
   if (!dist() || ny_ < 8 || !side_) {
@@ -153,7 +154,30 @@
              : NK_ECOMM;
 }
 
+bool SHProblem::callpass(int part) const {
+  const char* e = std::getenv("NKHIP_CALLPASS");
+  if (!e || !*e) return true;
+  if (e[0] == 'p') return std::strchr(e + 1, '0' + part) != nullptr;
+  return e[0] != '0';
+}
+
+bool SHProblem::needs_g() const { return !march_path() || !callpass(2); }
+
+bool SHProblem::has_step0() const {
+  return callpass(1) && !dist() && jvp_mode_ == NK_JVP_FD && march_path();
+}
+
 int SHProblem::prepare(const double* u_prev) {
+  b_pending_ = nullptr;
+  if (callpass(3) && !needs_g() && !dist() &&
+      (reinterpret_cast<uintptr_t>(u_prev) & 15u) == 0) {
+    b_pending_ = u_prev;
+    return NK_OK;
+  }
+  return form_b(u_prev);
+}
+
+int SHProblem::form_b(const double* u_prev) {
   int rc = halo(u_prev, hu_);
   if (rc) return rc;
   StencilArgs A;
@@ -240,15 +264,26 @@
 
 int SHProblem::eval(const double* x, const double* p, double alpha, double* xt, double* F,
                     double* G, double red[3]) {
+  bool init = false;
+  if (b_pending_) {
+    init = x == b_pending_ && p == x && alpha == 0.0 && !G;
+    const double* u = b_pending_;
+    b_pending_ = nullptr;
+    if (!init) {
+      const int rb = form_b(u);
+      if (rb) return rb;
+    }
+  }
+  spec_dots_ = false;
   StencilArgs A;
   A.ny = ny_;
   A.nx = nx_;
   A.a = field(x, hxp_ ? hxp_ : hx_);
   A.b = (p == x) ? A.a : field(p, hdp_ ? hdp_ : hd_);
   A.alpha = alpha;
-  A.p0 = B_;
+  A.p0 = init ? nullptr : B_;
   A.out0 = F;
-  A.out1 = G;
+  A.out1 = init ? B_ : G;
   A.out2 = xt;
   A.c = c_;
   A.partial = E_.partial();
@@ -256,7 +291,10 @@
   if (A.E0 && xt && (A.E2 = E_.edges(xt)) != nullptr) E_.mark_edges(xt);
   set_push(&A, F, xt);
   int64_t nblk = 0;
-  int rc = E_.launch(K_TRIAL, stencil_bytes_per_point(SMode::TRIAL, xt != nullptr) * ny_ * nx_,
+  int rc = E_.launch(K_TRIAL,
+                     stencil_bytes_per_point(SMode::TRIAL, xt != nullptr,
+                                             stencil_variant(SMode::TRIAL, A)) *
+                         ny_ * nx_,
                      [&] { return stencil_launch(SMode::TRIAL, A, E_.s, &nblk); });
   if (rc) return rc;
   const SpecJvp sp = spec_;
@@ -280,12 +318,43 @@
     J.spec_zn = sp.zn;
     J.spec_zs = sp.zs;
     side_edges(&J, xt, sp.z);
-    rc = halo_stencil(K_FDJVP, SMode::FDJVP, J, nullptr, hz_);
+    if (has_step0()) {
+      J.p0 = nullptr;
+      J.q = F;
+      J.partial = E_.partial();
+      int64_t nb = 0;
+      rc = E_.launch(K_FDJVP, stencil_bytes_per_point(SMode::FDJVP, false, 2) * ny_ * nx_,
+                     [&] { return stencil_launch(SMode::FDJVP, J, E_.s, &nb); });
+      if (!rc) rc = E_.reduce_async(nb, 3, 3, Engine::slot_mdot(0));
+      spec_dots_ = !rc;
+    } else {
+      rc = halo_stencil(K_FDJVP, SMode::FDJVP, J, nullptr, hz_);
+    }
   }
   if (!rc) rc = E_.wait_results(Engine::kSlotSync, 3);
   if (rc) return rc;
   std::memcpy(red, E_.hres(Engine::kSlotSync), sizeof(double) * 3);
   return NK_OK;
+}
+
+int SHProblem::jvp_dots(const double* x0, const double* z, double zs, double sc, const double* q,
+                        double* w, int64_t* nblk) {
+  StencilArgs A;
+  A.ny = ny_;
+  A.nx = nx_;
+  A.c = c_;
+  A.out0 = w;
+  set_edges(&A, w);
+  A.a = field(x0, hxp_ ? hxp_ : hx_);
+  A.b = field(z, hz_);
+  A.alpha = sc * zs;
+  A.sc = sc;
+  A.q = q;
+  A.partial = E_.partial();
+  side_edges(&A, x0, z);
+  const double bytes = stencil_bytes_per_point(SMode::FDJVP, false, q == z ? 1 : 2);
+  return E_.launch(K_FDJVP, bytes * ny_ * nx_,
+                   [&] { return stencil_launch(SMode::FDJVP, A, E_.s, nblk); });
 }
 
 bool SHProblem::can_spec_jvp() const {
diff --git a/iterative-solvers-summer-2020_amd/csrc/sh_problem.h b/iterative-solvers-summer-2020_amd/csrc/sh_problem.h
--- a/iterative-solvers-summer-2020_amd/csrc/sh_problem.h
+++ b/iterative-solvers-summer-2020_amd/csrc/sh_problem.h
@@ -17,6 +17,11 @@
   int jvp(const double* x0, const double* G0, const double* z, double zs, double sc,
           double* w) override;
   bool has_dev_scale() const override { return true; }
+  bool needs_g() const override;
+  bool has_step0() const override;
+  int jvp_dots(const double* x0, const double* z, double zs, double sc, const double* q, double* w,
+               int64_t* nblk) override;
+  bool spec_dots() const override { return spec_dots_; }
   bool can_spec_jvp() const override;
   void arm_spec(const SpecJvp* sp) override { spec_ = sp ? *sp : SpecJvp{}; }
   int jvp_dev(const double* x0, const double* G0, const double* z, const double* znorm2,
@@ -36,6 +41,9 @@
 
  private:
   bool dist() const { return E_.comm != nullptr; }
+  bool callpass(int part) const;
+  bool march_path() const { return nx_ % 2 == 0 && nx_ >= 2 && ny_ >= 2; }
+  int form_b(const double* u_prev);
   Field field(const double* p, const double* halo) const;
   int halo(const double* v, double* h);
   int halo_stencil(int kind, SMode m, const StencilArgs& A, const double* z, double* zh);
@@ -51,6 +59,8 @@
   int jvp_mode_;
   int status_ = NK_OK;
   double* B_ = nullptr;
+  const double* b_pending_ = nullptr;
+  bool spec_dots_ = false;
   SpecJvp spec_{};
   double* hx_ = nullptr;
   double* hz_ = nullptr;
diff --git a/iterative-solvers-summer-2020_amd/csrc/stencil.hip b/iterative-solvers-summer-2020_amd/csrc/stencil.hip
--- a/iterative-solvers-summer-2020_amd/csrc/stencil.hip
+++ b/iterative-solvers-summer-2020_amd/csrc/stencil.hip
@@ -56,7 +56,7 @@
   return w * k.ik - (Lw + k.g * ww - w * ww) / 2;
 }
 
-template <SMode M>
+template <SMode M, int X = 0>
 __device__ __forceinline__ Res finish(const StencilArgs& A, const Nb& na, const Nb& nb, double pv,
                                       double alpha, double sc) {
   Res r{0.0, 0.0, 0.0};
@@ -74,11 +74,28 @@
     const double uo = na.c;
     const double uouo = uo * uo;
     r.o0 = -uo * k.ik - (applyL(k, na) + k.g * uouo - uo * uouo) / 2;
+  } else if constexpr (M == SMode::TRIAL && X == 2) {
+    const double Lw = applyL(k, na);
+    const double G = Gfun(k, na.c, Lw);
+    const double uo = na.c;
+    const double uouo = uo * uo;
+    const double B = -uo * k.ik - (Lw + k.g * uouo - uo * uouo) / 2;
+    r.o0 = G + B;
+    r.o1 = B;
+    r.o2 = na.c;
   } else if constexpr (M == SMode::TRIAL) {
     const double G = Gfun(k, na.c, applyL(k, na));
     r.o0 = G + pv;
     r.o1 = G;
     r.o2 = na.c;
+  } else if constexpr (M == SMode::FDJVP && X >= 1) {
+    const double zs = alpha * sc;
+    const double uc = na.c;
+    const double Lu = applyL(k, na);
+    const double x = pv;
+    const double t = alpha * uc;
+    const double D = k.g * (2.0 * x + t) - (3.0 * x * (x + t) + t * t);
+    r.o0 = zs * (uc * k.ik - (Lu + uc * D) / 2);
   } else if constexpr (M == SMode::FDJVP) {
     r.o0 = (Gfun(k, na.c, applyL(k, na)) - pv) * sc;
   } else if constexpr (M == SMode::LINOP) {
@@ -102,6 +119,14 @@
     (M == SMode::TRIAL || M == SMode::FDJVP || M == SMode::AJVP || M == SMode::LINOP);
 template <SMode M>
 constexpr int kRad = (M == SMode::LAP5) ? 1 : 2;
+template <SMode M, int X>
+constexpr bool kClosed = (M == SMode::FDJVP && X >= 1);
+template <SMode M, int X>
+constexpr bool kDots = (M == SMode::FDJVP && X == 2);
+template <SMode M, int X>
+constexpr bool kNoG = (M == SMode::TRIAL && X == 1);
+template <SMode M, int X>
+constexpr bool kInit = (M == SMode::TRIAL && X == 2);
 
 template <SMode M>
 __device__ __forceinline__ bool jvp_scale(const StencilArgs& A, double* alpha, double* sc) {
@@ -143,15 +168,19 @@
   return *reinterpret_cast<const double2*>(p);
 }
 
-template <SMode M>
-constexpr int kFields = (kComb<M> || kTwo<M>) ? 2 : 1;
-
-template <SMode M, int BX, int PF>
+template <SMode M, int X = 0>
+constexpr int kFields = ((kComb<M> || kTwo<M>) && !kClosed<M, X> && !kInit<M, X>) ? 2 : 1;
+
+template <SMode M, int BX, int PF, int X = 0>
 __global__ void __launch_bounds__(BX) march_kernel(StencilArgs A, int RY, int gx, int gy) {
   constexpr int R = kRad<M>;
   constexpr int NR = 2 * R + 1;
   constexpr int RING = NR + PF;
-  constexpr int NF = kFields<M>;
+  constexpr int NF = kFields<M, X>;
+  const Field& fa = kClosed<M, X> ? A.b : A.a;
+  const double* const Efa = kClosed<M, X> ? A.Eb : A.Ea;
+  const double* const pw = kClosed<M, X> ? A.a.base : A.p0;
+  constexpr bool kPw = kHasP0<M> && !kInit<M, X>;
   const int64_t nx = A.nx, ny = A.ny;
   const int64_t lb = (int64_t(blockIdx.x) % 8) * (int64_t(gridDim.x) / 8) + blockIdx.x / 8;
   if (lb >= int64_t(gx) * gy) return;
@@ -185,18 +214,26 @@
   double ring[NF][RING][6];
   auto load_row = [&](int slot, int64_t r) {
     r = (r > ny + 1) ? ny + 1 : ((r < -2) ? -2 : r);
-    ld(A.a, A.Ea, r, ring[0][slot]);
+    ld(fa, Efa, r, ring[0][slot]);
     if constexpr (NF == 2) ld(A.b, A.Eb, r, ring[1][slot]);
   };
   auto combine = [&](int slot) {
-    if constexpr (kComb<M>) {
-#pragma unroll
-      for (int q = 0; q < 6; ++q) ring[0][slot][q] = ring[0][slot][q] + alpha * ring[1][slot][q];
+    if constexpr (kInit<M, X>) {
+#pragma unroll
+      for (int q = 0; q < 6; ++q) ring[0][slot][q] = ring[0][slot][q] + alpha * ring[0][slot][q];
+    } else if constexpr (kComb<M> && !kClosed<M, X>) {
+#pragma unroll
+      for (int q = 0; q < 6; ++q)
+        ring[0][slot][q] = ring[0][slot][q] + alpha * ring[NF - 1][slot][q];
     }
   };
   auto ldp = [&](int64_t r) {
     r = (r >= ny) ? ny - 1 : ((r < 0) ? 0 : r);
-    return ld_p0(A, A.p0 + r * nx + cc);
+    return ld_p0(A, pw + r * nx + cc);
+  };
+  auto ldq = [&](int64_t r) {
+    r = (r >= ny) ? ny - 1 : ((r < 0) ? 0 : r);
+    return ld_p0(A, A.q + r * nx + cc);
   };
 
   const int64_t band = A.rev ? int64_t(gy) - 1 - by : by;
@@ -212,9 +249,16 @@
   double2 pq[RING];
 #pragma unroll
   for (int d = 0; d < RING; ++d) pq[d] = make_double2(0.0, 0.0);
-  if constexpr (kHasP0<M>) {
+  if constexpr (kPw) {
 #pragma unroll
     for (int d = 0; d < PF; ++d) pq[d] = ldp(rs + dir * d);
+  }
+  double2 qq[kDots<M, X> ? RING : 1];
+  if constexpr (kDots<M, X>) {
+#pragma unroll
+    for (int d = 0; d < RING; ++d) qq[d] = make_double2(0.0, 0.0);
+#pragma unroll
+    for (int d = 0; d < PF; ++d) qq[d] = ldq(rs + dir * d);
   }
 #pragma unroll
   for (int k = 0; k < NR - 1; ++k) combine(k);
@@ -234,7 +278,8 @@
       const int64_t it = base + u;
       const int64_t r = rs + dir * it;
       load_row((u + RING - 1) % RING, r + dir * (R + PF));
-      if constexpr (kHasP0<M>) pq[(u + PF) % RING] = ldp(r + dir * PF);
+      if constexpr (kPw) pq[(u + PF) % RING] = ldp(r + dir * PF);
+      if constexpr (kDots<M, X>) qq[(u + PF) % RING] = ldq(r + dir * PF);
       combine((u + NR - 1) % RING);
       const double2 pv = pq[u % RING];
       auto W = [&](int m, int q) -> double { return ring[0][(u + m) % RING][q]; };
@@ -260,7 +305,7 @@
           na.dg = 0.0;
           na.a2 = 0.0;
         }
-        res[q] = finish<M>(A, na, nb, q == 0 ? pv.x : pv.y, alpha, sc);
+        res[q] = finish<M, X>(A, na, nb, q == 0 ? pv.x : pv.y, alpha, sc);
       }
       if (active && it < nrows) {
         const int64_t o = r * nx + cc;
@@ -276,8 +321,16 @@
             *reinterpret_cast<double2*>(A.E0 + (b * A.e_ny + er) * 4) = ev;
           }
         }
+        if constexpr (kDots<M, X>) {
+          const double2 qv = qq[u % RING];
+          red[0] += res[0].o0 * qv.x;
+          red[0] += res[1].o0 * qv.y;
+          red[2] += res[0].o0 * res[0].o0;
+          red[2] += res[1].o0 * res[1].o0;
+        }
         if constexpr (M == SMode::TRIAL) {
-          *reinterpret_cast<double2*>(A.out1 + o) = make_double2(res[0].o1, res[1].o1);
+          if constexpr (!kNoG<M, X>)
+            *reinterpret_cast<double2*>(A.out1 + o) = make_double2(res[0].o1, res[1].o1);
           if (A.out2) *reinterpret_cast<double2*>(A.out2 + o) = make_double2(res[0].o2, res[1].o2);
           if (A.PS2[0]) push_row(A.PS2, A.e_row0 + r, make_double2(res[0].o2, res[1].o2));
           if (A.E2) {
@@ -307,6 +360,11 @@
   if (pushed) drain_stores();
   if constexpr (kRed<M>) {
     const double v = block_reduce<3, 1, BX>(red);
+    const int64_t nblk = int64_t(gx) * gy;
+    const int64_t bid = band * gx + bx;
+    if (threadIdx.x < 3) A.partial[threadIdx.x * nblk + bid] = v;
+  } else if constexpr (kDots<M, X>) {
+    const double v = block_reduce<3, 3, BX>(red);
     const int64_t nblk = int64_t(gx) * gy;
     const int64_t bid = band * gx + bx;
     if (threadIdx.x < 3) A.partial[threadIdx.x * nblk + bid] = v;
@@ -358,7 +416,7 @@
     const Res res = finish<M>(A, a, b, pv, alpha, sc);
     A.out0[idx] = res.o0;
     if constexpr (M == SMode::TRIAL) {
-      A.out1[idx] = res.o1;
+      if (A.out1) A.out1[idx] = res.o1;
       if (A.out2) A.out2[idx] = res.o2;
       red[0] = res.o0 * res.o0;
       red[1] = fabs(res.o0);
@@ -440,10 +498,25 @@
          (aligned16(f.base) && (f.lo == nullptr || (aligned16(f.lo) && aligned16(f.hi))));
 }
 
+template <SMode M, int X>
+void march_go(const StencilArgs& B, int pf, dim3 grid, hipStream_t s, int RY, int gx, int gy) {
+  constexpr int BX = 128;
+  if (pf == 2)
+    hipLaunchKernelGGL((march_kernel<M, BX, 2, X>), grid, dim3(BX), 0, s, B, RY, gx, gy);
+  else
+    hipLaunchKernelGGL((march_kernel<M, BX, 1, X>), grid, dim3(BX), 0, s, B, RY, gx, gy);
+}
+
 template <SMode M>
 hipError_t launch_mode(const StencilArgs& A, hipStream_t s, int64_t* nblk) {
   const bool fast = (A.nx % 2 == 0) && A.nx >= 2 && A.ny >= 2 && field_ok(A.a) && field_ok(A.b) &&
-                    aligned16(A.p0) && aligned16(A.out0) && aligned16(A.out1) && aligned16(A.out2);
+                    aligned16(A.p0) && aligned16(A.out0) && aligned16(A.out1) &&
+                    aligned16(A.out2) && aligned16(A.q);
+  const int x = stencil_variant(M, A);
+  if (M == SMode::TRIAL && x == 2 &&
+      !(A.out1 && A.alpha == 0.0 && A.b.base == A.a.base && A.b.lo == A.a.lo))
+    return hipErrorInvalidValue;
+  if (!fast && x != 0 && !(M == SMode::TRIAL && x == 1)) return hipErrorInvalidValue;
   if (fast) {
     StencilArgs B = A;
     for (Field* f : {&B.a, &B.b}) {
@@ -490,10 +563,16 @@
     static const bool nt_p0 = env_int("NKHIP_NT_P0", 1) != 0;
     B.nt_p0 = nt_p0;
     const dim3 grid{unsigned((gx * gy + 7) / 8 * 8), 1u, 1u};
-    if (pf == 2)
-      hipLaunchKernelGGL((march_kernel<M, BX, 2>), grid, dim3(BX), 0, s, B, RY, int(gx), int(gy));
-    else
-      hipLaunchKernelGGL((march_kernel<M, BX, 1>), grid, dim3(BX), 0, s, B, RY, int(gx), int(gy));
+    if constexpr (M == SMode::FDJVP || M == SMode::TRIAL) {
+      if (x == 2)
+        march_go<M, 2>(B, pf, grid, s, RY, int(gx), int(gy));
+      else if (x == 1)
+        march_go<M, 1>(B, pf, grid, s, RY, int(gx), int(gy));
+      else
+        march_go<M, 0>(B, pf, grid, s, RY, int(gx), int(gy));
+    } else {
+      march_go<M, 0>(B, pf, grid, s, RY, int(gx), int(gy));
+    }
   } else {
     if (A.E0 || A.E2 || A.Ea || A.Eb || A.PS0[0] || A.PS2[0])
       return hipErrorInvalidValue;
@@ -528,7 +607,17 @@
   return 3 * (march > point ? march : point) + 3;
 }
 
-double stencil_bytes_per_point(SMode m, bool has_xt) {
+int stencil_variant(SMode m, const StencilArgs& A) {
+  if (m == SMode::FDJVP) return A.p0 ? 0 : ((A.q && A.partial) ? 2 : 1);
+  if (m == SMode::TRIAL) return A.p0 ? (A.out1 ? 0 : 1) : 2;
+  return 0;
+}
+
+double stencil_bytes_per_point(SMode m, bool has_xt, int variant) {
+  if (m == SMode::FDJVP && variant == 1) return 24.0;
+  if (m == SMode::FDJVP && variant == 2) return 32.0;
+  if (m == SMode::TRIAL && variant == 1) return has_xt ? 40.0 : 32.0;
+  if (m == SMode::TRIAL && variant == 2) return has_xt ? 32.0 : 24.0;
   switch (m) {
     case SMode::LAP5: return 16.0;
     case SMode::SH13: return 16.0;
diff --git a/iterative-solvers-summer-2020_amd/nkhip/_lib.py b/iterative-solvers-summer-2020_amd/nkhip/_lib.py
--- a/iterative-solvers-summer-2020_amd/nkhip/_lib.py
+++ b/iterative-solvers-summer-2020_amd/nkhip/_lib.py
@@ -114,6 +114,8 @@
     ("nk_debug_ctl_step", C.c_int, [_I32, _I32, _P, _P, _P, _P, _P, _P, _P, _P, _P, _P, _P, _P]),
     ("nk_debug_stencil", C.c_int, [C.POINTER(nk_stencil_pass), C.POINTER(_D), C.POINTER(_I64),
                                    _P]),
+    ("nk_debug_stencil_callpass", C.c_int, [C.POINTER(nk_stencil_pass), _P, C.POINTER(_D),
+                                            C.POINTER(_I64), _P]),
     ("nk_comm_unique_id_bytes", C.c_int, []),
     ("nk_comm_get_unique_id", C.c_int, [_P]),
     ("nk_comm_create_rccl", C.c_int, [C.POINTER(_P), _P, _I32, _I32]),
diff --git a/iterative-solvers-summer-2020_amd/nkhip/ops.py b/iterative-solvers-summer-2020_amd/nkhip/ops.py
--- a/iterative-solvers-summer-2020_amd/nkhip/ops.py
+++ b/iterative-solvers-summer-2020_amd/nkhip/ops.py
@@ -205,7 +205,7 @@
                  b_halo=None, rows=None, alpha=0.0, sc=1.0, e=0.0, theta=0.0, h=1.0, r=0.0, k=1.0,
                  g=0.0, znorm2=None, omega=0.0, spec=None, spec_thr=0.0, spec_ftol=0.0,
                  spec_rdiff=0.0, spec_zn=1.0, spec_zs=1.0, Ea=None, Eb=None, E0=None, E2=None,
-                 PS0=None, PS2=None, ps_ld=0, rev=-1):
+                 PS0=None, PS2=None, ps_ld=0, rev=-1, q=None, callpass=False):
     from ._lib import nk_stencil_pass
 
     m = STENCIL_MODES.index(mode) if isinstance(mode, str) else int(mode)
@@ -248,8 +248,12 @@
     P.rev = int(rev)
     red = (C.c_double * 3)()
     nblk = C.c_int64(0)
-    check(lib.nk_debug_stencil(C.byref(P), red, C.byref(nblk), _stream()), "nk_debug_stencil")
-    nred = {4: 3, 7: 1}.get(m, 0)
+    if callpass or q is not None:
+        check(lib.nk_debug_stencil_callpass(C.byref(P), dev(q, "q", n), red, C.byref(nblk),
+                                            _stream()), "nk_debug_stencil_callpass")
+    else:
+        check(lib.nk_debug_stencil(C.byref(P), red, C.byref(nblk), _stream()), "nk_debug_stencil")
+    nred = 3 if q is not None else {4: 3, 7: 1}.get(m, 0)
     return [red[i] for i in range(nred)], nblk.value
 
 
```

After: 32.57 (median of 6 runs). No clear change (+1.0%).
